# dbandstra/zang

Hardware: AMD Instinct MI355X
Metric: voice-samples/sec (higher is better)
Workload: dtype f32

## Files before the change

bindings/zang_hip.zig:

```

const std = @import("std");

pub const OK: c_int = 0;
pub const ERR_INVALID: c_int = -1;
pub const ERR_UNSUPPORTED: c_int = -2;
pub const ERR_NO_DEVICE: c_int = -3;
pub const ERR_COMM: c_int = -4;
pub const ERR_RCCL_BASE: c_int = -100;
pub const PAINT_ADD: u32 = 0;
pub const PAINT_ZERO_FIRST: u32 = 1;
pub const PAINT_PARAMS_UNCHANGED: u32 = 4;
pub const PAINT_TOLERANT: u32 = 8;
pub const COB_CONSTANT: u32 = 0;
pub const COB_BUFFER: u32 = 1;
pub const CURVE_INSTANTANEOUS: u32 = 0;
pub const CURVE_LINEAR: u32 = 1;
pub const CURVE_SQUARED: u32 = 2;
pub const CURVE_CUBED: u32 = 3;
pub const CAPTURE_COALESCE: u32 = 1;
pub const MIX_SEQUENTIAL: u32 = 2;
pub const COMM_ID_BYTES: u32 = 128;
pub const AUDIO_SIGNED8: u32 = 0;
pub const AUDIO_SIGNED16_LSB: u32 = 1;
pub const NOISE_WHITE: u32 = 0;
pub const NOISE_PINK: u32 = 1;
pub const ENV_IDLE: u32 = 0;
pub const ENV_ATTACK: u32 = 1;
pub const ENV_DECAY: u32 = 2;
pub const ENV_SUSTAIN: u32 = 3;
pub const ENV_RELEASE: u32 = 4;
pub const FILTER_BYPASS: u32 = 0;
pub const FILTER_LOW_PASS: u32 = 1;
pub const FILTER_BAND_PASS: u32 = 2;
pub const FILTER_HIGH_PASS: u32 = 3;
pub const FILTER_NOTCH: u32 = 4;
pub const FILTER_ALL_PASS: u32 = 5;
pub const SAMPLE_U8: u32 = 0;
pub const SAMPLE_S16_LSB: u32 = 1;
pub const SAMPLE_S24_LSB: u32 = 2;
pub const SAMPLE_S32_LSB: u32 = 3;
pub const DISTORTION_OVERDRIVE: u32 = 0;
pub const DISTORTION_CLIP: u32 = 1;
pub const CURVE_FN_LINEAR: u32 = 0;
pub const CURVE_FN_SMOOTHSTEP: u32 = 1;
pub const MIX_MAX_BATCH: u32 = 16;
pub const FM_MOD_FREQ_MUL: u32 = 0;
pub const FM_MOD_WAVEFORM: u32 = 1;
pub const FM_MOD_VOLUME: u32 = 2;
pub const FM_MOD_ATTACK: u32 = 3;
pub const FM_MOD_DECAY: u32 = 4;
pub const FM_MOD_SUSTAIN: u32 = 5;
pub const FM_MOD_RELEASE: u32 = 6;
pub const FM_MOD_TREMOLO: u32 = 7;
pub const FM_MOD_VIBRATO: u32 = 8;
pub const FM_MOD_FEEDBACK: u32 = 9;
pub const FM_CAR_FREQ_MUL: u32 = 10;
pub const FM_CAR_WAVEFORM: u32 = 11;
pub const FM_CAR_VOLUME: u32 = 12;
pub const FM_CAR_ATTACK: u32 = 13;
pub const FM_CAR_DECAY: u32 = 14;
pub const FM_CAR_SUSTAIN: u32 = 15;
pub const FM_CAR_RELEASE: u32 = 16;
pub const FM_CAR_TREMOLO: u32 = 17;
pub const FM_CAR_VIBRATO: u32 = 18;
pub const FM_TREMOLO_DEPTH: u32 = 19;
pub const FM_VIBRATO_DEPTH: u32 = 20;
pub const FM_ALGORITHM: u32 = 21;
pub const FM_PATCH_VALUES: u32 = 22;
pub const FM_SPLIT_OPERATORS: u32 = 16;
pub const SP_CONSTANT: u32 = 0;
pub const SP_BOOLEAN: u32 = 1;
pub const SP_COB: u32 = 2;
pub const SP_BUFFER: u32 = 3;
pub const SP_ENUM: u32 = 4;
pub const SP_CURVE: u32 = 5;
pub const SINEOSC_SPAN_FREQ: u32 = 0;
pub const SINEOSC_SPAN_PHASE: u32 = 1;
pub const SINEOSC_SPAN_FIELDS: u32 = 2;
pub const PULSEOSC_SPAN_FREQ: u32 = 0;
pub const PULSEOSC_SPAN_COLOR: u32 = 1;
pub const PULSEOSC_SPAN_FIELDS: u32 = 2;
pub const TRISAWOSC_SPAN_FREQ: u32 = 0;
pub const TRISAWOSC_SPAN_COLOR: u32 = 1;
pub const TRISAWOSC_SPAN_FIELDS: u32 = 2;
pub const NOISE_SPAN_COLOR: u32 = 0;
pub const NOISE_SPAN_FIELDS: u32 = 1;
pub const ENVELOPE_SPAN_ATTACK: u32 = 0;
pub const ENVELOPE_SPAN_DECAY: u32 = 1;
pub const ENVELOPE_SPAN_RELEASE: u32 = 2;
pub const ENVELOPE_SPAN_SUSTAIN_VOLUME: u32 = 3;
pub const ENVELOPE_SPAN_NOTE_ON: u32 = 4;
pub const ENVELOPE_SPAN_FIELDS: u32 = 5;
pub const GATE_SPAN_NOTE_ON: u32 = 0;
pub const GATE_SPAN_FIELDS: u32 = 1;
pub const FILTER_SPAN_TYPE: u32 = 0;
pub const FILTER_SPAN_CUTOFF: u32 = 1;
pub const FILTER_SPAN_RES: u32 = 2;
pub const FILTER_SPAN_FIELDS: u32 = 3;
pub const SAMPLER_SPAN_SAMPLE_RATE: u32 = 0;
pub const SAMPLER_SPAN_LOOP: u32 = 1;
pub const SAMPLER_SPAN_FIELDS: u32 = 2;
pub const DECIMATOR_SPAN_FAKE_SAMPLE_RATE: u32 = 0;
pub const DECIMATOR_SPAN_FIELDS: u32 = 1;
pub const DISTORTION_SPAN_TYPE: u32 = 0;
pub const DISTORTION_SPAN_INGAIN: u32 = 1;
pub const DISTORTION_SPAN_OUTGAIN: u32 = 2;
pub const DISTORTION_SPAN_OFFSET: u32 = 3;
pub const DISTORTION_SPAN_FIELDS: u32 = 4;
pub const SAMPLER_KIT_SPAN_SAMPLE_RATE: u32 = 0;
pub const SAMPLER_KIT_SPAN_LOOP: u32 = 1;
pub const SAMPLER_KIT_SPAN_SAMPLE: u32 = 2;
pub const SAMPLER_KIT_SPAN_CHANNEL: u32 = 3;
pub const SAMPLER_KIT_SPAN_FIELDS: u32 = 4;
pub const MAX_IMPULSES: u32 = 32;
pub const MAX_PARAMS_SIZE: u32 = 64;
pub const SCRIPT_MAX_PARAMS: u32 = 16;
pub const ZSCRIPT_FORM_SPANS: u32 = 8;
pub const ZSCRIPT_FORM_ROLES: u32 = 1;
pub const ZSCRIPT_FORM_ROLES_WORTH: u32 = 2;

pub const Ctx = opaque {};
pub const Graph = opaque {};
pub const Event = opaque {};
pub const Comm = opaque {};
pub const SineOscHandle = opaque {};
pub const PulseOscHandle = opaque {};
pub const TriSawOscHandle = opaque {};
pub const NoiseHandle = opaque {};
pub const EnvelopeHandle = opaque {};
pub const GateHandle = opaque {};
pub const FilterHandle = opaque {};
pub const SamplerHandle = opaque {};
pub const SampleKit = opaque {};
pub const DecimatorHandle = opaque {};
pub const DistortionHandle = opaque {};
pub const CurveModuleHandle = opaque {};
pub const CycleHandle = opaque {};
pub const PortamentoHandle = opaque {};
pub const NiceHandle = opaque {};
pub const DelayHandle = opaque {};
pub const FilteredEchoesHandle = opaque {};
pub const StereoEchoesHandle = opaque {};
pub const NoiseFilterHandle = opaque {};
pub const PMOscHandle = opaque {};
pub const Fm = opaque {};
pub const Script = opaque {};
pub const ScriptModule = opaque {};
pub const ZScript = opaque {};
pub const ImpulseQueue = opaque {};
pub const NoteTracker = opaque {};
pub const PolyphonyDispatcher = opaque {};
pub const Trigger = opaque {};
pub const PolyVoice = opaque {};
pub const VoiceBank = opaque {};

pub const Buf = extern struct {
    ptr: ?[*]f32 = null,
    voices: u32 = 0,
    frames: u32 = 0,
    stride: u32 = 0,
    reserved: u32 = 0,
};
pub const F32 = extern struct {
    value: f32 = 0,
    reserved: u32 = 0,
    per_voice: ?[*]const f32 = null,
};
pub const Bool = extern struct {
    value: u32 = 0,
    reserved: u32 = 0,
    per_voice: ?[*]const u8 = null,
};
pub const Cob = extern struct {
    tag: u32 = 0,
    reserved: u32 = 0,
    constant: F32 = std.mem.zeroes(F32),
    buffer: Buf = std.mem.zeroes(Buf),
};
pub const Curve = extern struct {
    tag: u32 = 0,
    reserved: u32 = 0,
    duration: F32 = std.mem.zeroes(F32),
};
pub const SineOscParams = extern struct {
    sample_rate: f32 = 0,
    reserved: u32 = 0,
    freq: Cob = std.mem.zeroes(Cob),
    phase: Cob = std.mem.zeroes(Cob),
};
pub const SineOscState = extern struct {
    t: f32 = 0,
};
pub const PulseOscParams = extern struct {
    sample_rate: f32 = 0,
    reserved: u32 = 0,
    freq: Cob = std.mem.zeroes(Cob),
    color: F32 = std.mem.zeroes(F32),
};
pub const PulseOscState = extern struct {
    cnt: u32 = 0,
};
pub const TriSawOscParams = extern struct {
    sample_rate: f32 = 0,
    reserved: u32 = 0,
    freq: Cob = std.mem.zeroes(Cob),
    color: F32 = std.mem.zeroes(F32),
};
pub const TriSawOscState = extern struct {
    cnt: u32 = 0,
    t: f32 = 0,
};
pub const NoiseParams = extern struct {
    color: u32 = 0,
};
pub const NoiseState = extern struct {
    r: [4]u64 = [_]u64{0} ** 4,
    b: [7]f32 = [_]f32{0} ** 7,
    reserved: u32 = 0,
};
pub const EnvelopeParams = extern struct {
    sample_rate: f32 = 0,
    reserved: u32 = 0,
    attack: Curve = std.mem.zeroes(Curve),
    decay: Curve = std.mem.zeroes(Curve),
    release: Curve = std.mem.zeroes(Curve),
    sustain_volume: F32 = std.mem.zeroes(F32),
    note_on: Bool = std.mem.zeroes(Bool),
};
pub const EnvelopeState = extern struct {
    state: u32 = 0,
    t: f32 = 0,
    last_value: f32 = 0,
    start: f32 = 0,
};
pub const GateParams = extern struct {
    note_on: Bool = std.mem.zeroes(Bool),
};
pub const FilterParams = extern struct {
    input: Buf = std.mem.zeroes(Buf),
    @"type": u32 = 0,
    reserved: u32 = 0,
    cutoff: Cob = std.mem.zeroes(Cob),
    res: Cob = std.mem.zeroes(Cob),
};
pub const FilterState = extern struct {
    l: f32 = 0,
    b: f32 = 0,
};
pub const Sample = extern struct {
    num_channels: u64 = 0,
    sample_rate: u64 = 0,
    format: u32 = 0,
    reserved: u32 = 0,
    data: ?[*]const u8 = null,
    data_len: u64 = 0,
};
pub const SamplerParams = extern struct {
    sample_rate: F32 = std.mem.zeroes(F32),
    sample: Sample = std.mem.zeroes(Sample),
    channel: u64 = 0,
    loop: u32 = 0,
    reserved: u32 = 0,
};
pub const SamplerState = extern struct {
    t: f32 = 0,
};
pub const DecimatorParams = extern struct {
    sample_rate: f32 = 0,
    reserved: u32 = 0,
    input: Buf = std.mem.zeroes(Buf),
    fake_sample_rate: F32 = std.mem.zeroes(F32),
};
// ... 1471 lines not shown
```

include/zang_hip.h:

```cpp
#ifndef ZANG_HIP_H
#define ZANG_HIP_H

#if !defined(__HIPCC_RTC__)
#include <stddef.h>
#include <stdint.h>
#endif

#ifdef __cplusplus
extern "C" {
#endif

#define ZH_API __attribute__((visibility("default")))

enum { ZH_OK = 0, ZH_ERR_INVALID = -1, ZH_ERR_UNSUPPORTED = -2, ZH_ERR_NO_DEVICE = -3,
       ZH_ERR_COMM = -4,
       ZH_ERR_RCCL_BASE = -100     };

enum { ZH_PAINT_ADD = 0,
       ZH_PAINT_ZERO_FIRST = 1,
       ZH_PAINT_PARAMS_UNCHANGED = 4,
       ZH_PAINT_TOLERANT = 8
        };

typedef struct zh_ctx zh_ctx;
// ... 388 lines not shown
typedef struct zh_fm_params { float sample_rate; uint32_t reserved; zh_buf tremolo_input, vibrato_input; zh_f32 freq; zh_bool note_on; } zh_fm_params;
typedef struct zh_fm_op_state { float t, feedback1, feedback2; uint32_t reserved; zh_envelope_state env; } zh_fm_op_state;
typedef struct zh_fm_state { zh_fm_op_state modulator, carrier; } zh_fm_state;
ZH_API int zh_fm_patch_default(zh_fm_patch *patch);
ZH_API int zh_fm_create(zh_ctx *ctx, uint32_t n_voices, uint32_t group, zh_fm **out);
ZH_API int zh_fm_destroy(zh_fm *m);
ZH_API int zh_fm_set_patches(zh_fm *m, const zh_fm_patch *patches, uint32_t n_patches);
ZH_API int zh_fm_get_state(zh_fm *m, zh_fm_state *host);
ZH_API int zh_fm_set_state(zh_fm *m, const zh_fm_state *host);
ZH_API int zh_fm_paint(zh_fm *m, uint32_t span_start, uint32_t span_end, const zh_buf *outputs,
                       const zh_buf *temps ,
                       zh_bool note_id_changed, const zh_fm_params *params, uint32_t flags);
ZH_API int zh_fm_paint_spans(zh_fm *m, uint32_t span_start, uint32_t span_end, const zh_buf *outputs,
                             const zh_buf *temps, float sample_rate, zh_buf tremolo_input, zh_buf vibrato_input,
                             const zh_span_table *table, uint32_t flags);

enum { ZH_SP_CONSTANT = 0,
       ZH_SP_BOOLEAN = 1,
       ZH_SP_COB = 2,
       ZH_SP_BUFFER = 3,
       ZH_SP_ENUM = 4,
       ZH_SP_CURVE = 5 };
typedef struct zh_script_param {
    uint32_t kind, u;
    float f;
    uint32_t is_buffer;
    const float *pf;
    const uint8_t *pb;
    uint32_t stride, reserved;
} zh_script_param;
#define ZH_SCRIPT_MAX_PARAMS 16

typedef struct zh_script zh_script;
typedef struct zh_script_module zh_script_module;
ZH_API int zh_script_compile(const char *hip_source, void **code_out, size_t *code_size_out, char *log, size_t log_cap);
ZH_API void zh_script_free_code(void *code);
ZH_API int zh_script_load(zh_ctx *ctx, const char *hip_source, zh_script **out, char *log, size_t log_cap);
ZH_API int zh_script_load_code(zh_ctx *ctx, const void *code, size_t code_size, zh_script **out);
ZH_API int zh_script_destroy(zh_script *s);
ZH_API int zh_script_module_create(zh_script *s, const char *name, uint32_t n_voices, uint32_t state_words,
                                   uint64_t first_seed, zh_script_module **out);
ZH_API int zh_script_module_destroy(zh_script_module *m);
ZH_API int zh_script_module_ranges_ok(zh_script_module *m);
ZH_API int zh_script_module_get_state(zh_script_module *m, uint32_t *host_words);
ZH_API int zh_script_module_set_state(zh_script_module *m, const uint32_t *host_words);
ZH_API int zh_script_module_paint(zh_script_module *m, uint32_t span_start, uint32_t span_end, const zh_buf *outputs,
                                  zh_bool note_id_changed, const zh_script_param *params, uint32_t n_params, uint32_t flags);
typedef struct zh_script_span_table {
    uint32_t max_spans, reserved;
    const uint32_t *count;
    const uint32_t *start, *end;
    const uint8_t  *note_id_changed;
} zh_script_span_table;
typedef struct zh_script_span_param {
    const float    *f;
    const uint32_t *u;
} zh_script_span_param;
#define ZH_ZSCRIPT_FORM_SPANS 8
ZH_API int zh_script_module_paint_spans(zh_script_module *m, uint32_t span_start, uint32_t span_end, const zh_buf *outputs,
                                        const zh_script_param *params, uint32_t n_params, const zh_script_span_param *span_params,
                                        const zh_script_span_table *table, uint32_t flags);

enum { ZH_SINEOSC_SPAN_FREQ = 0,
       ZH_SINEOSC_SPAN_PHASE,
       ZH_SINEOSC_SPAN_FIELDS };
enum { ZH_PULSEOSC_SPAN_FREQ = 0,
       ZH_PULSEOSC_SPAN_COLOR,
       ZH_PULSEOSC_SPAN_FIELDS };
enum { ZH_TRISAWOSC_SPAN_FREQ = 0,
       ZH_TRISAWOSC_SPAN_COLOR,
       ZH_TRISAWOSC_SPAN_FIELDS };
enum { ZH_NOISE_SPAN_COLOR = 0,
       ZH_NOISE_SPAN_FIELDS };
enum { ZH_ENVELOPE_SPAN_ATTACK = 0,
       ZH_ENVELOPE_SPAN_DECAY,
       ZH_ENVELOPE_SPAN_RELEASE,
       ZH_ENVELOPE_SPAN_SUSTAIN_VOLUME,
       ZH_ENVELOPE_SPAN_NOTE_ON,
       ZH_ENVELOPE_SPAN_FIELDS };
enum { ZH_GATE_SPAN_NOTE_ON = 0,
       ZH_GATE_SPAN_FIELDS };
enum { ZH_FILTER_SPAN_TYPE = 0,
       ZH_FILTER_SPAN_CUTOFF,
       ZH_FILTER_SPAN_RES,
       ZH_FILTER_SPAN_FIELDS };
enum { ZH_SAMPLER_SPAN_SAMPLE_RATE = 0,
       ZH_SAMPLER_SPAN_LOOP,
       ZH_SAMPLER_SPAN_FIELDS };
enum { ZH_DECIMATOR_SPAN_FAKE_SAMPLE_RATE = 0,
       ZH_DECIMATOR_SPAN_FIELDS };
enum { ZH_DISTORTION_SPAN_TYPE = 0,
       ZH_DISTORTION_SPAN_INGAIN,
       ZH_DISTORTION_SPAN_OUTGAIN,
       ZH_DISTORTION_SPAN_OFFSET,
       ZH_DISTORTION_SPAN_FIELDS };
ZH_API int zh_sineosc_paint_spans(zh_sineosc *m, uint32_t span_start, uint32_t span_end, const zh_buf *outputs, const zh_buf *temps,
                                  const zh_sineosc_params *params, const zh_script_span_param *span_params ,
                                  const zh_script_span_table *table, uint32_t flags);
ZH_API int zh_pulseosc_paint_spans(zh_pulseosc *m, uint32_t span_start, uint32_t span_end, const zh_buf *outputs, const zh_buf *temps,
                                   const zh_pulseosc_params *params, const zh_script_span_param *span_params ,
                                   const zh_script_span_table *table, uint32_t flags);
ZH_API int zh_trisawosc_paint_spans(zh_trisawosc *m, uint32_t span_start, uint32_t span_end, const zh_buf *outputs, const zh_buf *temps,
                                    const zh_trisawosc_params *params, const zh_script_span_param *span_params ,
                                    const zh_script_span_table *table, uint32_t flags);
ZH_API int zh_noise_paint_spans(zh_noise *m, uint32_t span_start, uint32_t span_end, const zh_buf *outputs, const zh_buf *temps,
                                const zh_noise_params *params, const zh_script_span_param *span_params ,
                                const zh_script_span_table *table, uint32_t flags);
ZH_API int zh_envelope_paint_spans(zh_envelope *m, uint32_t span_start, uint32_t span_end, const zh_buf *outputs, const zh_buf *temps,
                                   const zh_envelope_params *params, const zh_script_span_param *span_params ,
                                   const zh_script_span_table *table, uint32_t flags);
ZH_API int zh_gate_paint_spans(zh_gate *m, uint32_t span_start, uint32_t span_end, const zh_buf *outputs, const zh_buf *temps,
                               const zh_gate_params *params, const zh_script_span_param *span_params ,
                               const zh_script_span_table *table, uint32_t flags);
ZH_API int zh_filter_paint_spans(zh_filter *m, uint32_t span_start, uint32_t span_end, const zh_buf *outputs, const zh_buf *temps,
                                 const zh_filter_params *params, const zh_script_span_param *span_params ,
                                 const zh_script_span_table *table, uint32_t flags);
ZH_API int zh_sampler_paint_spans(zh_sampler *m, uint32_t span_start, uint32_t span_end, const zh_buf *outputs, const zh_buf *temps,
                                  const zh_sampler_params *params, const zh_script_span_param *span_params ,
                                  const zh_script_span_table *table, uint32_t flags);
ZH_API int zh_decimator_paint_spans(zh_decimator *m, uint32_t span_start, uint32_t span_end, const zh_buf *outputs, const zh_buf *temps,
                                    const zh_decimator_params *params, const zh_script_span_param *span_params ,
                                    const zh_script_span_table *table, uint32_t flags);
ZH_API int zh_distortion_paint_spans(zh_distortion *m, uint32_t span_start, uint32_t span_end, const zh_buf *outputs, const zh_buf *temps,
                                     const zh_distortion_params *params, const zh_script_span_param *span_params ,
                                     const zh_script_span_table *table, uint32_t flags);

typedef struct zh_u32 { uint32_t value; uint32_t reserved; const uint32_t *per_voice; } zh_u32;
typedef struct zh_sampler_kit_params {
    zh_f32 sample_rate;
    zh_bool loop;
    zh_u32 sample;
    zh_u32 channel;
    const zh_sample_kit *kit;
} zh_sampler_kit_params;
enum { ZH_SAMPLER_KIT_SPAN_SAMPLE_RATE = 0,
       ZH_SAMPLER_KIT_SPAN_LOOP,
       ZH_SAMPLER_KIT_SPAN_SAMPLE,
       ZH_SAMPLER_KIT_SPAN_CHANNEL,
       ZH_SAMPLER_KIT_SPAN_FIELDS };
ZH_API int zh_sampler_paint_kit_spans(zh_sampler *m, uint32_t span_start, uint32_t span_end, const zh_buf *outputs, const zh_buf *temps,
                                      const zh_sampler_kit_params *params, const zh_script_span_param *span_params ,
                                      const zh_script_span_table *table, uint32_t flags);
ZH_API int zh_sampler_paint_kit(zh_sampler *m, uint32_t span_start, uint32_t span_end, const zh_buf *outputs, const zh_buf *temps,
                                zh_bool note_id_changed, const zh_sampler_kit_params *params, uint32_t flags);

typedef struct zh_zscript zh_zscript;
ZH_API int zh_zscript_compile(const char *text, const char *filename, uint32_t packages, zh_zscript **out, char *err, size_t err_cap);
ZH_API int zh_zscript_destroy(zh_zscript *z);
ZH_API void zh_zscript_free_text(char *text);
ZH_API int zh_zscript_generate_zig(zh_zscript *z, char **text_out);
ZH_API int zh_zscript_generate_hip(zh_zscript *z, const char *only_csv, int unroll, char **text_out);
#define ZH_ZSCRIPT_FORM_ROLES 1
#define ZH_ZSCRIPT_FORM_ROLES_WORTH 2
ZH_API int zh_zscript_generate_hip_forms(zh_zscript *z, const char *only_csv, int unroll, uint32_t forms, char **text_out);
ZH_API uint32_t zh_zscript_module_count(zh_zscript *z);
ZH_API int zh_zscript_module_info(zh_zscript *z, uint32_t i, char *name, size_t name_cap, uint32_t *state_words, uint32_t *noise_fields,
                                  uint32_t *n_params, char *error , size_t error_cap);
ZH_API int zh_zscript_module_num_temps(zh_zscript *z, uint32_t i, uint32_t *num_temps);
ZH_API int zh_zscript_module_param(zh_zscript *z, uint32_t i, uint32_t p, char *name, size_t name_cap, char *kind, size_t kind_cap,
                                   char *enum_name, size_t enum_cap);

typedef struct zh_impulse { uint64_t frame, note_id, event_id; } zh_impulse;
typedef struct zh_iap { const zh_impulse *impulses; const void *paramses; uint64_t len; } zh_iap;
enum { ZH_MAX_IMPULSES = 32, ZH_MAX_PARAMS_SIZE = 64 };

typedef struct zh_impulse_queue zh_impulse_queue;
ZH_API int zh_impulse_queue_create(uint32_t params_size, zh_impulse_queue **out);
ZH_API int zh_impulse_queue_destroy(zh_impulse_queue *q);
ZH_API int zh_impulse_queue_push(zh_impulse_queue *q, uint64_t impulse_frame, uint64_t note_id, const void *params);
ZH_API int zh_impulse_queue_consume(zh_impulse_queue *q, zh_iap *out);

typedef struct zh_note_tracker zh_note_tracker;
ZH_API int zh_note_tracker_create(uint32_t params_size, uint64_t n_events, const void *paramses, const float *t,
                                  const uint64_t *note_ids, zh_note_tracker **out);
ZH_API int zh_note_tracker_destroy(zh_note_tracker *nt);
ZH_API int zh_note_tracker_reset(zh_note_tracker *nt);
ZH_API int zh_note_tracker_consume(zh_note_tracker *nt, float sample_rate, uint64_t span_start, uint64_t span_end, zh_iap *out);

typedef struct zh_polyphony_dispatcher zh_polyphony_dispatcher;
ZH_API int zh_polyphony_dispatcher_create(uint32_t polyphony, uint32_t params_size, uint32_t note_on_offset,
                                          zh_polyphony_dispatcher **out);
ZH_API int zh_polyphony_dispatcher_destroy(zh_polyphony_dispatcher *pd);
ZH_API int zh_polyphony_dispatcher_reset(zh_polyphony_dispatcher *pd);
ZH_API int zh_polyphony_dispatcher_dispatch(zh_polyphony_dispatcher *pd, zh_iap iap, zh_iap *out );

typedef struct zh_trigger zh_trigger;
typedef struct zh_paint_span {
    uint64_t start, end; uint32_t note_id_changed; uint32_t reserved; uint8_t params[64];
} zh_paint_span;
ZH_API int zh_trigger_create(uint32_t params_size, zh_trigger **out);
ZH_API int zh_trigger_destroy(zh_trigger *t);
ZH_API int zh_trigger_reset(zh_trigger *t);
ZH_API int zh_trigger_counter(zh_trigger *t, uint64_t span_start, uint64_t span_end, zh_iap iap);
ZH_API int zh_trigger_next(zh_trigger *t, zh_paint_span *out);

typedef struct zh_poly_voice zh_poly_voice;
ZH_API int zh_poly_voice_create(uint32_t polyphony, uint32_t params_size, uint32_t note_on_offset, uint64_t n_events,
                                const void *paramses, const float *t, const uint64_t *note_ids, zh_poly_voice **out);
ZH_API int zh_poly_voice_destroy(zh_poly_voice *pv);
ZH_API int zh_poly_voice_reset(zh_poly_voice *pv);
ZH_API int zh_poly_voice_schedule(zh_poly_voice *pv, float sample_rate, const uint32_t *frames, uint32_t n_buffers,
                                  uint32_t max_spans, uint32_t *counts, uint32_t *start, uint32_t *end, void *params,
                                  uint8_t *note_id_changed);

typedef struct zh_voice_bank zh_voice_bank;
typedef struct zh_voice_bank_instrument_state { uint64_t next_event; float t; uint32_t reserved; } zh_voice_bank_instrument_state;
typedef struct zh_voice_bank_voice_state {
    uint32_t used, note_on; uint64_t note_id, event_id;
    uint32_t has_note, reserved; uint64_t trigger_note_id;
    uint64_t trigger_event;
} zh_voice_bank_voice_state;
ZH_API int zh_voice_bank_create(zh_ctx *ctx, uint32_t n_instruments, uint32_t polyphony, uint32_t params_size, uint32_t note_on_offset,
                                const uint64_t *event_offsets, const void *paramses, const float *t, const uint64_t *note_ids,
                                zh_voice_bank **out);
ZH_API int zh_voice_bank_destroy(zh_voice_bank *bank);
ZH_API int zh_voice_bank_reset(zh_voice_bank *bank);
ZH_API int zh_voice_bank_reserve(zh_voice_bank *bank, uint32_t max_rows);
ZH_API int zh_voice_bank_schedule(zh_voice_bank *bank, float sample_rate, const uint32_t *frames, uint32_t n_buffers, uint32_t max_spans);
ZH_API int zh_voice_bank_script_table(const zh_voice_bank *bank, uint32_t max_spans, zh_script_span_table *out);
ZH_API int zh_voice_bank_span_param(const zh_voice_bank *bank, uint32_t word, zh_script_span_param *out);
ZH_API int zh_voice_bank_span_table(const zh_voice_bank *bank, uint32_t max_spans, uint32_t freq_word, zh_span_table *out);
ZH_API int zh_voice_bank_overflows(zh_voice_bank *bank, uint64_t *out);
ZH_API int zh_voice_bank_get_state(zh_voice_bank *bank, zh_voice_bank_instrument_state *instruments ,
                                   zh_voice_bank_voice_state *voices );
ZH_API int zh_voice_bank_set_state(zh_voice_bank *bank, const zh_voice_bank_instrument_state *instruments,
                                   const zh_voice_bank_voice_state *voices);

typedef struct zh_bank_impulses {
    uint32_t n; const uint32_t *instrument, *frame; const uint64_t *note_id; const void *paramses;
} zh_bank_impulses;
typedef struct zh_voice_bank_live_voice_state {
    uint32_t used, note_on; uint64_t note_id, event_id;
    uint32_t has_note, reserved; uint64_t trigger_note_id;
    uint32_t carried[16];
} zh_voice_bank_live_voice_state;
ZH_API int zh_voice_bank_create_live(zh_ctx *ctx, uint32_t n_instruments, uint32_t polyphony, uint32_t params_size, uint32_t note_on_offset,
                                     uint32_t max_impulses_per_call, zh_voice_bank **out);
ZH_API int zh_voice_bank_schedule_live(zh_voice_bank *bank, uint32_t out_len, uint32_t max_spans, const zh_bank_impulses *batch);
ZH_API int zh_voice_bank_live_get_state(zh_voice_bank *bank, uint64_t *next_event_id ,
                                        zh_voice_bank_live_voice_state *voices );
ZH_API int zh_voice_bank_live_set_state(zh_voice_bank *bank, const uint64_t *next_event_id, const zh_voice_bank_live_voice_state *voices);

typedef struct zh_hcob { uint32_t tag; float constant; const float *buffer; } zh_hcob;
typedef struct zh_hcurve { uint32_t tag; float duration; } zh_hcurve;

typedef struct zh_sineosc_host_params { float sample_rate; zh_hcob freq, phase; } zh_sineosc_host_params;
typedef struct zh_pulseosc_host_params { float sample_rate; zh_hcob freq; float color; } zh_pulseosc_host_params;
typedef zh_pulseosc_host_params zh_trisawosc_host_params;
typedef struct zh_noise_host_params { uint32_t color; } zh_noise_host_params;
typedef struct zh_envelope_host_params { float sample_rate; zh_hcurve attack, decay, release; float sustain_volume; uint32_t note_on; } zh_envelope_host_params;
typedef struct zh_gate_host_params { uint32_t note_on; } zh_gate_host_params;
typedef struct zh_filter_host_params { const float *input; uint32_t type; zh_hcob cutoff, res; } zh_filter_host_params;
typedef struct zh_sampler_host_params {
    float sample_rate; uint64_t num_channels, sample_rate_in; uint32_t format; const uint8_t *data; uint64_t data_len;
    uint64_t channel; uint32_t loop;
} zh_sampler_host_params;
typedef struct zh_decimator_host_params { float sample_rate; const float *input; float fake_sample_rate; } zh_decimator_host_params;
typedef struct zh_distortion_host_params { const float *input; uint32_t type; float ingain, outgain, offset; } zh_distortion_host_params;

ZH_API int zh_noise_state_init(zh_noise_state *state, uint64_t seed);
ZH_API int zh_decimator_state_init(zh_decimator_state *state);

ZH_API int zh_sineosc_paint_host(zh_ctx *ctx, zh_sineosc_state *state, uint32_t span_start, uint32_t span_end, float *const *outputs, float *const *temps, uint32_t note_id_changed, const zh_sineosc_host_params *params);
ZH_API int zh_pulseosc_paint_host(zh_ctx *ctx, zh_pulseosc_state *state, uint32_t span_start, uint32_t span_end, float *const *outputs, float *const *temps, uint32_t note_id_changed, const zh_pulseosc_host_params *params);
ZH_API int zh_trisawosc_paint_host(zh_ctx *ctx, zh_trisawosc_state *state, uint32_t span_start, uint32_t span_end, float *const *outputs, float *const *temps, uint32_t note_id_changed, const zh_trisawosc_host_params *params);
ZH_API int zh_noise_paint_host(zh_ctx *ctx, zh_noise_state *state, uint32_t span_start, uint32_t span_end, float *const *outputs, float *const *temps, uint32_t note_id_changed, const zh_noise_host_params *params);
ZH_API int zh_envelope_paint_host(zh_ctx *ctx, zh_envelope_state *state, uint32_t span_start, uint32_t span_end, float *const *outputs, float *const *temps, uint32_t note_id_changed, const zh_envelope_host_params *params);
ZH_API int zh_gate_paint_host(zh_ctx *ctx, void *state_unused, uint32_t span_start, uint32_t span_end, float *const *outputs, float *const *temps, uint32_t note_id_changed, const zh_gate_host_params *params);
ZH_API int zh_filter_paint_host(zh_ctx *ctx, zh_filter_state *state, uint32_t span_start, uint32_t span_end, float *const *outputs, float *const *temps, uint32_t note_id_changed, const zh_filter_host_params *params);
ZH_API int zh_sampler_paint_host(zh_ctx *ctx, zh_sampler_state *state, uint32_t span_start, uint32_t span_end, float *const *outputs, float *const *temps, uint32_t note_id_changed, const zh_sampler_host_params *params);
ZH_API int zh_decimator_paint_host(zh_ctx *ctx, zh_decimator_state *state, uint32_t span_start, uint32_t span_end, float *const *outputs, float *const *temps, uint32_t note_id_changed, const zh_decimator_host_params *params);
ZH_API int zh_distortion_paint_host(zh_ctx *ctx, void *state_unused, uint32_t span_start, uint32_t span_end, float *const *outputs, float *const *temps, uint32_t note_id_changed, const zh_distortion_host_params *params);

#ifdef __cplusplus
}
#endif
#endif
```

zang_amd/csrc/common.hip.h:

```cpp
#pragma once
#if defined(__HIPCC_RTC__)
#define ZH_DEVICE_ONLY 1
#endif
#include <hip/hip_runtime.h>
#if !defined(ZH_DEVICE_ONLY)
#include <stdint.h>
#include <stddef.h>
#include <new>
#endif
#include "rtc_types.hip.h"
#include "../../include/zang_hip.h"

#if !defined(ZH_DEVICE_ONLY)
#include <utility>
#include <vector>
#include <functional>
#include <memory>
#include <string>
struct zh_flipper {
    uint64_t id;
    zh_ctx *ctx;
    uint32_t n;
    uint32_t *cnt[2];
    int cur;
    uint32_t words = 1;
};
struct zh_flip_use {
    uint64_t id;
    zh_flipper *f;
    int first_cur;
    uint32_t flips;
};

struct zh_flipper;
struct zh_co_batch {
    bool active = false;
    const void *owner = nullptr;
    uint32_t start = 0, end = 0, stride = 0, key = 0, max = 0;
    bool flips = false;
    std::vector<float *> imgs;
    std::shared_ptr<void> items;
    std::function<void(hipStream_t, float *const *, uint32_t)> launch;
    const char *kernel = nullptr;
};
struct zh_direct_item {
    std::function<void(hipStream_t, float *const *, uint32_t)> launch;
    std::vector<float *> imgs;
    const char *kernel;
};

struct zh_ctx {
    int device;
    hipStream_t stream;
    bool own_stream;
    uint32_t capture_flags;
    bool epoch_open;
    zh_co_batch co;
    uint32_t co_paints, co_launches;
    std::string last_form;
    bool form_fresh;
    float *mix_partials;
    size_t mix_partials_floats;
    std::vector<float *> mix_retired;
    uint32_t graphs_live;
    std::vector<struct zh_graph *> graphs;
    bool capturing;
    uint32_t capture_serial;
    std::vector<zh_flip_use> capture_log;
    std::vector<std::pair<std::string, uint32_t>> capture_kernels;
    int deferred_error = 0;
    std::vector<zh_direct_item> co_plan;
    bool co_plan_ok = true;
    uint32_t capture_launches = 0, co_plan_launches = 0;
    void *noise_jump;
};

struct zh_graph {
    zh_ctx *ctx;
    hipGraph_t graph;
    hipGraphExec_t exec;
    std::vector<zh_flip_use> flips;
    uint32_t nodes = 0;
    uint32_t co_paints = 0, co_launches = 0;
    std::vector<std::pair<std::string, uint32_t>> kernels;
    std::vector<zh_direct_item> plan;
    std::vector<std::pair<std::string, uint32_t>> plan_kernels;
};

struct ZhDeviceGuard {
    int prev, want;
    explicit ZhDeviceGuard(int device) : prev(-1), want(device) {
        if (want < 0) return;
        if (hipGetDevice(&prev) != hipSuccess) { prev = -1; return; }
        if (prev != want) (void)hipSetDevice(want);
    }
    ~ZhDeviceGuard() { if (want >= 0 && prev >= 0 && prev != want) (void)hipSetDevice(prev); }
    ZhDeviceGuard(const ZhDeviceGuard &) = delete;
    ZhDeviceGuard &operator=(const ZhDeviceGuard &) = delete;
};
void zh_epoch_barrier(zh_ctx *ctx);
extern thread_local zh_ctx *zh_tls_ctx;
struct ZhFormScope {
    zh_ctx *prev;
    explicit ZhFormScope(const zh_ctx *c) : prev(zh_tls_ctx) {
        if (!prev) { zh_tls_ctx = const_cast<zh_ctx *>(c); if (zh_tls_ctx) zh_tls_ctx->form_fresh = true; }
    }
    ~ZhFormScope() { zh_tls_ctx = prev; }
};
#define ZH_GUARD_EPOCH(ctxptr) const zh_ctx *_zh_gctx = (ctxptr); ZhDeviceGuard _zh_guard(_zh_gctx ? _zh_gctx->device : -1); ZhFormScope _zh_fscope(_zh_gctx)
#define ZH_LAUNCH(kernel, ...) do { zh_note_launch(zh_tls_ctx, #kernel); hipLaunchKernelGGL(kernel, __VA_ARGS__); } while (0)
#define ZH_GUARD(ctxptr) ZH_GUARD_EPOCH(ctxptr); do { if (_zh_gctx && _zh_gctx->epoch_open) zh_epoch_barrier(const_cast<zh_ctx *>(_zh_gctx)); } while (0)
void zh_epoch_flush_batch(zh_ctx *ctx, bool last);

void zh_flipper_register(zh_flipper *f);
void zh_flipper_unregister(zh_flipper *f);
void zh_flipper_used(zh_flipper *f);
void zh_flipper_painted(zh_flipper *f);

enum { ZF_SINE_RANGES, ZF_NOISE_RANGES, ZF_ENVELOPE_RANGES, ZF_SAMPLER_RANGES, ZF_DECIMATOR_RANGES, ZF_CURVE_RANGES, ZF_CYCLE_RANGES,
       ZF_PORTAMENTO_RANGES, ZF_PULSE_CTRL_RANGES, ZF_PULSE_CTRL_SUMS, ZF_TRISAW_CTRL_RANGES, ZF_TRISAW_CTRL_QUOT, ZF_PMOSC_RANGES,
       ZF_SCRIPT_RANGES, ZF_SCRIPT_RANGES_MAXV, ZF_OSC_FC, ZF_NICE_PC_MAX, ZF_NICE_PC4_MAX, ZF_NICE_WAVE_MAX, ZF_PMOSC_WAVE_MAX,
       ZF_NICE_MIX_ROLL, ZF_NICE_MIX_WG_MIN, ZF_NF_PC_MAX, ZF_NF_RING_MAX, ZF_FILTER_PC_MAX, ZF_FILTER_PC16_MAX, ZF_FILTER_PC_CTL_MAX,
       ZF_PINK_PIPE_MAX, ZF_PINK_TAPS, ZF_ECHOES_PC_MAX, ZF_DELAY_FRAMES_MAX, ZF_FILTER_TP_MAX, ZF_NF_TP_MAX, ZF_NICE_TP_MAX,
       ZF_PINK_TP_MAX, ZF_ECHOES_TP_MAX, ZF_NICE_MIX_FMA, ZF_BASICS_ROWS_MIN, ZF_SCRIPT_PC, ZF_SCRIPT_PC_MAXV, ZF_NF_TP_PIPE_FRAMES, ZF_DISTORTION_ROWS_MIN, ZF_DISTORTION_RC, ZF_GRAPH_DIRECT,
       ZF_STEREO_ECHOES_PC_MAX, ZF_COUNT };
long zh_form(int id);
bool zh_form_is_set(int id);
uint32_t zh_range_frames(uint32_t V, uint32_t n, int form, uint32_t target_waves, uint32_t max_voices);
void zh_note_launch(zh_ctx *ctx, const char *kernel);
extern thread_local const char *zh_tls_launch_detail;

constexpr int kMixGroupFrames = 8;

struct zh_event {
    hipEvent_t ev;
};
#endif

#define ZH_INLINE_LAMBDA __attribute__((always_inline))

#if !defined(ZH_DEVICE_ONLY)
#define ZH_TRY(expr)                                   \
    do {                                               \
        hipError_t _e = (expr);                        \
        if (_e != hipSuccess) return (int)_e;          \
    } while (0)

static inline int zh_launch_status() {
    hipError_t e = hipGetLastError();
    return e == hipSuccess ? ZH_OK : (int)e;
}
#endif

struct Img {
    float *p;
    uint32_t stride;
    __device__ __forceinline__ float *at(uint32_t f, uint32_t v) const { return p + (size_t)f * stride + v; }
};
struct CImg {
    const float *p;
    uint32_t stride;
    __device__ __forceinline__ const float *at(uint32_t f, uint32_t v) const { return p + (size_t)f * stride + v; }
};
struct F32P {
    float value;
    const float *pv;
    __device__ __forceinline__ float get(uint32_t v) const { return pv ? pv[v] : value; }
};
struct BoolP {
    uint32_t value;
    const uint8_t *pv;
    __device__ __forceinline__ bool get(uint32_t v) const { return pv ? pv[v] != 0 : value != 0; }
};
struct CobP {
    uint32_t is_buffer;
    F32P c;
    CImg b;
};

#if !defined(ZH_DEVICE_ONLY)
static inline Img mk_img(const zh_buf &b) { return Img{b.ptr, b.stride}; }
static inline CImg mk_cimg(const zh_buf &b) { return CImg{b.ptr, b.stride}; }
static inline F32P mk_f32(const zh_f32 &f) { return F32P{f.value, f.per_voice}; }
static inline BoolP mk_bool(const zh_bool &b) { return BoolP{b.value, b.per_voice}; }
static inline CobP mk_cob(const zh_cob &c) {
    return CobP{c.tag == ZH_COB_BUFFER ? 1u : 0u, mk_f32(c.constant), mk_cimg(c.buffer)};
}

constexpr uint32_t kMaxRowStride = 1u << 26;
static inline bool buf_covers(const zh_buf &b, uint32_t n_voices, uint32_t span_end) {
    return b.ptr != nullptr && b.voices >= n_voices && b.frames >= span_end && b.stride >= n_voices && b.stride <= kMaxRowStride;
}
static inline bool bufs_alias(const zh_buf &a, const zh_buf &b) {
    if (!a.ptr || !b.ptr) return false;
    const float *ae = a.ptr + (size_t)a.frames * a.stride, *be = b.ptr + (size_t)b.frames * b.stride;
    return a.ptr < be && b.ptr < ae;
}
static inline bool cob_aliases(const zh_cob &c, const zh_buf &b) { return c.tag == ZH_COB_BUFFER && bufs_alias(c.buffer, b); }
static inline int zh_zero_first_aliased(zh_ctx *ctx, uint32_t start, uint32_t end, const zh_buf &out, uint32_t n_voices, bool aliased, uint32_t &flags) {
    if (!aliased || !(flags & ZH_PAINT_ZERO_FIRST)) return ZH_OK;
    flags &= ~(uint32_t)ZH_PAINT_ZERO_FIRST;
    zh_buf o = out;
    o.voices = n_voices;
    return end > start ? zh_zero(ctx, start, end, o) : ZH_OK;
}
static inline bool cob_ok(const zh_cob &c, uint32_t n_voices, uint32_t span_end) {
    if (c.tag == ZH_COB_CONSTANT) return true;
    if (c.tag == ZH_COB_BUFFER) return buf_covers(c.buffer, n_voices, span_end);
    return false;
}

#ifndef ZH_SEQ_BLOCK
#define ZH_SEQ_BLOCK 64
#endif
constexpr int kSeqBlock = ZH_SEQ_BLOCK;
static inline dim3 seq_grid(uint32_t n) { return dim3((n + kSeqBlock - 1) / kSeqBlock); }

template <typename T> static inline int dev_alloc(T **p, size_t count) {
    *p = nullptr;
    if (count == 0) return ZH_OK;
    hipError_t e = hipMalloc((void **)p, count * sizeof(T));
    return e == hipSuccess ? ZH_OK : (int)e;
}

#endif

enum StoreMode { ST_PLAIN = 0, ST_NT = 1, ST_SC1 = 2, ST_SC0SC1 = 3 };

typedef float zv4f __attribute__((ext_vector_type(4)));
typedef unsigned int zv4u __attribute__((ext_vector_type(4)));

#if defined(__HIP_DEVICE_COMPILE__)
typedef __amdgpu_buffer_rsrc_t zh_rsrc_t;
__device__ __forceinline__ zh_rsrc_t make_rsrc(const void *base, uint32_t bytes) {
    return __builtin_amdgcn_make_buffer_rsrc(const_cast<void *>(base), 0, bytes, 0x00020000);
}
template <int SM>
__device__ __forceinline__ void store4(float *p, zh_rsrc_t rsrc, uint32_t byte_off, zv4f v) {
    if constexpr (SM == ST_PLAIN) *reinterpret_cast<zv4f *>(p) = v;
    else if constexpr (SM == ST_NT) __builtin_nontemporal_store(v, reinterpret_cast<zv4f *>(p));
    else if constexpr (SM == ST_SC1) __builtin_amdgcn_raw_buffer_store_b128(__builtin_bit_cast(zv4u, v), rsrc, byte_off, 0, 16);
    else __builtin_amdgcn_raw_buffer_store_b128(__builtin_bit_cast(zv4u, v), rsrc, byte_off, 0, 17);
}
template <int SM>
__device__ __forceinline__ void store1(float *p, zh_rsrc_t rsrc, uint32_t byte_off, float v) {
    if constexpr (SM == ST_PLAIN) *p = v;
    else if constexpr (SM == ST_NT) __builtin_nontemporal_store(v, p);
    else if constexpr (SM == ST_SC1) __builtin_amdgcn_raw_buffer_store_b32(__builtin_bit_cast(unsigned int, v), rsrc, byte_off, 0, 16);
    else __builtin_amdgcn_raw_buffer_store_b32(__builtin_bit_cast(unsigned int, v), rsrc, byte_off, 0, 17);
}
__device__ __forceinline__ void store_row(float *p, float v) { __builtin_nontemporal_store(v, p); }
__device__ __forceinline__ void store4_sc1(float *p, zv4f v) { asm volatile("global_store_dwordx4 %0, %1, off sc1\n\ts_nop 1" ::"v"(p), "v"(v) : "memory"); }
#else
typedef int zh_rsrc_t;
__device__ inline void store4_sc1(float *, zv4f) {}
__device__ inline void store_row(float *, float) {}
__device__ inline zh_rsrc_t make_rsrc(const void *, uint32_t) { return 0; }
template <int SM> __device__ inline void store4(float *, zh_rsrc_t, uint32_t, zv4f) {}
template <int SM> __device__ inline void store1(float *, zh_rsrc_t, uint32_t, float) {}
#endif

#if !defined(ZH_DEVICE_ONLY)
int zh_store_mode();
int zh_store_mode_env();
constexpr uint32_t kRowPadVoices = 1024;
#endif
```

zang_amd/csrc/dispatch.hip:

```cpp
#include "common.hip.h"
#include <mutex>
#include <stdlib.h>
#include <string.h>
#include <string>

namespace {
struct FormRow { const char *name; long def; const char *doc; };
const FormRow kForms[ZF_COUNT] = {
     {"sine_ranges", -1, "SineOsc: frame ranges of the span at once, each replaying the phase walk before it (k_sineosc_ranges); auto: ~4,096 waves up to 1 Mi voices, ~2,048 up to 65,536 with a control image"},
     {"noise_ranges", -1, "Noise: frame ranges from jumped generator states (noise_jump.hip); auto: by voice count up to 65,536"},
     {"envelope_ranges", -1, "Envelope: frame ranges, each replaying the clock (k_envelope_ranges); auto: ~2,048 waves up to 40,960 voices"},
     {"sampler_ranges", -1, "Sampler: frame ranges (positions are a product, no replay); auto: ~16,384 waves up to 1 Mi voices"},
     {"decimator_ranges", -1, "Decimator: frame ranges replaying the hold counter; auto: ~1,024-2,048 waves up to 65,536 voices"},
     {"curve_ranges", -1, "Curve: frame ranges; auto: ~2,048 waves up to 40,960 voices"},
     {"cycle_ranges", -1, "Cycle: frame ranges (constant speed); auto: ~1,024 waves up to 16,384 voices"},
     {"portamento_ranges", -1, "Portamento: frame ranges; auto: ~2,048 waves up to 32,768 voices"},
     {"pulse_ctrl_ranges", -1, "PulseOsc with a frequency image: frame ranges over the summed phase advances; auto: ~2,048 waves up to 40,960 voices"},
     {"pulse_ctrl_sums", 1, "... 1: a first kernel sums each range's own advances (k_pulseosc_ctrl_sums), 0: every range replays the frames before it"},
     {"trisaw_ctrl_ranges", -1, "TriSawOsc with a frequency image: frame ranges; auto: ~1,024 waves up to 16,384 voices"},
     {"trisaw_ctrl_quot", 1, "... 1: freq / sample_rate painted once into a module-owned image first (k_div_image), 0: divided in every replay"},
     {"pmosc_ranges", -1, "PMOscInstrument: frame ranges (k_pmosc_ranges); auto: ~2,048-4,096 waves up to 131,072 voices"},
     {"script_ranges", -1, "generated script kernels: frame ranges for modules without a delay ring; auto: by voice count"},
     {"script_ranges_maxv", 131072, "... the largest voice count that takes them"},
     {"osc_fc", 0, "constant-frequency PulseOsc / TriSawOsc: frames per lane of the chunked kernel; 0 = PulseOsc 4, from 16,384 voices 3 with non-temporal stores (profiles/r05/osc_large_voice_counts.txt); TriSawOsc 8-64 by voice count (tools/sweep_osc_fc.sh), PulseOsc's when the paint is a sawtooth for every voice (one color <= 0)"},
     {"nice_pc_max", 65536, "NiceInstrument: up to here the oscillator, envelope and filter chains run in three waves side by side (k_nice_pc: 72 vs 146 us at 4,096 voices, 107 vs 168 at 65,536; slower at 131,072)"},
     {"nice_pc4_max", 32768, "... and up to here in four (k_nice_pc4: 44 / 47 / 53.5 us at 4,096 / 16,384 / 32,768 voices against 60.5 / 62.5 / 63)"},
     {"nice_wave_max", 64, "zh_nice_paint_spans: up to here one WAVE per voice, lanes = frames (k_nice_spans_wave)"},
     {"pmosc_wave_max", 64, "zh_pmosc_paint_spans: the same (k_pmosc_spans_wave)"},
     {"nice_mix_roll", 1, "fused mixdown: the oscillator's half-period bit carried as a lane mask (1) or recomputed (0): 148.2 vs 149.6 us at 131,072 voices"},
     {"nice_mix_wg_min", 65536, "fused mixdown: from here one partial row per 256-voice workgroup instead of per wave (a quarter of the partial traffic; 4,096 voices: 99 -> 105 us with it, 131,072: level)"},
     {"nf_pc_max", 65536, "Noise -> Filter voice: up to here noise and filter in two waves side by side (k_noise_filter_pc: 75 vs 110 us at 4,096 voices, 111 vs 133 at 65,536)"},
     {"nf_ring_max", 16384, "... white noise: up to here three producer waves, a filter wave and a writer wave per 64 voices (k_noise_filter_ring)"},
     {"filter_pc_max", 32768, "Filter, constant cutoff / resonance: up to here the three-wave pipeline over 32-frame tiles (k_filter_pc: 41-51 us against 54-76 in one wave); 0 = never (the 16-frame form too unless filter_pc16_max is given), 1 = the 16-frame form only"},
     {"filter_pc16_max", 65536, "... 16-frame tiles above filter_pc_max up to here (36,864 / 65,536 voices: 72 / 104 us against 97 / 116)"},
     {"filter_pc_ctl_max", 32768, "... with control images (k_filter_pc_ctl: 47-98 us against 96-140 up to 32,768 voices)"},
     {"pink_pipe_max", 32768, "pink Noise: up to here white frame ranges + the taps as a second kernel (k_pink_taps / k_pink_pipe) instead of one loop"},
     {"pink_taps", 1, "... 1: four-wave tap kernel (32-frame tiles up to 16,384 voices, 16 above), 16: the 16-frame tiles always, 0: the seven-stage chain k_pink_pipe"},
     {"echoes_pc_max", 65536, "FilteredEchoes: up to here ring reader / filter / writer as waves side by side (k_filtered_echoes_pc)"},
     {"delay_frames_max", 4294967295, "Delay: up to here the frames of a delay length at once instead of the walk (57 -> 13 us at 4,096 voices, 423 -> 271 at 131,072: every voice count)"},
     {"filter_tp_max", 16384, "ZH_PAINT_TOLERANT Filter: the largest voice count painted as chunks at once (filter_tp.hip.h)"},
     {"nf_tp_max", 16384, "... Noise -> Filter voice"},
     {"nice_tp_max", 16384, "... NiceInstrument and its fused mixdown"},
     {"pink_tp_max", 16384, "... pink Noise"},
     {"echoes_tp_max", 6144, "... FilteredEchoes (six image streams: level with the exact form at 8,192 voices)"},
     {"nice_mix_fma", 1, "ZH_PAINT_TOLERANT fused mixdown above nice_tp_max voices: 1 = the kernel compiled with multiply-adds fused (nice_mix_fma.hip), 0 = the exact kernel"},
     {"basics_rows_min", 32768, "basics.zig operations (zero, set, copy, add ..., multiply ...): from here three consecutive rows of a 256-voice column per wave (k_elementwise_chunks) instead of the row-striding loop: 131,072 voices 12-23 % faster"},
     {"script_pc", -1, "generated script kernels: the role-wave form (zs_paint_pc_<name>: the body's builtin calls as producer / recurrence / writer waves over LDS tiles); auto: where the emitter found the lane form unable to take frame ranges and the longest role well below the whole body; 0 = never, 1 = every module that has the form"},
     {"script_pc_maxv", 65536, "... the largest voice count that takes it -- half of it for a module whose role form does more than 1.25 x the body's work or needs more than 9 waves (FilteredSawtooth: 53 / 57 / 66 / 110 us at 4,096 / 16,384 / 32,768 / 65,536 voices against 172-181 in one wave per 64 voices; slower at 131,072)"},
     {"nf_tp_pipe_frames", 0, "ZH_PAINT_TOLERANT Noise -> Filter voice recorded pipelined (ZH_CAPTURE_COALESCE, k_nf_tp_ba): frames per chunk, a multiple of 32; 0 = as outside a pipeline (32 at 4,096 voices)"},
     {"distortion_rows_min", 32768, "Distortion clip: from here four voices per lane, three consecutive rows of a 256-voice column per wave, the per-voice constants once per workgroup through LDS (k_distortion_chunks: 224 -> 178 us at 131,072 voices); the overdrive too when this row is set by hand (no faster: 239 against 244-250 us)"},
     {"distortion_rc", 0, "... rows per wave of that form: 3 (0), 6 or 8"},
     {"graph_direct", 1, "zh_graph_launch of a ZH_CAPTURE_COALESCE capture that recorded nothing but held-back oscillator batches: 1 = their launches enqueued directly, one per batch of up to 32 buffers (20 paints: one launch of 20), 0 = the recorded hipGraph (20 paints: two launches of 10)"},
     {"stereo_echoes_pc_max", 32768, "StereoEchoes: up to here loader / filter / writer waves (k_stereo_echoes_pc); StereoEchoes(15000), 1,024 frames, role waves against the walk: 253 / 318 us at 32,768 voices, 518 / 454 at 65,536 (profiles/r10)"},
};

struct Overrides { bool set[ZF_COUNT]; long val[ZF_COUNT]; };
Overrides parse_forms() {
    Overrides o;
    memset(&o, 0, sizeof o);
    const char *e = getenv("ZH_FORMS");
    if (!e) return o;
    std::string s(e);
    size_t i = 0;
    while (i < s.size()) {
        size_t j = s.find(',', i);
        if (j == std::string::npos) j = s.size();
        const std::string item = s.substr(i, j - i);
        const size_t eq = item.find('=');
        if (eq != std::string::npos) {
            const std::string name = item.substr(0, eq);
            for (int k = 0; k < ZF_COUNT; k++)
                if (name == kForms[k].name) { o.set[k] = true; o.val[k] = strtol(item.c_str() + eq + 1, nullptr, 10); }
        }
        i = j + 1;
    }
    return o;
}
}

bool zh_form_is_set(int id) {
    if (id < 0 || id >= ZF_COUNT) return false;
    return parse_forms().set[id];
}

long zh_form(int id) {
    if (id < 0 || id >= ZF_COUNT) return 0;
    static const bool live = [] { const char *e = getenv("ZH_ENV_LIVE"); return e && e[0] == '1'; }();
    if (live) {
        const Overrides o = parse_forms();
        return o.set[id] ? o.val[id] : kForms[id].def;
    }
    static const Overrides once = parse_forms();
    return once.set[id] ? once.val[id] : kForms[id].def;
}

uint32_t zh_range_frames(uint32_t V, uint32_t n, int form, uint32_t target_waves, uint32_t max_voices) {
    const long forced = zh_form(form);
    if (forced == 0 || V == 0 || n < 128 || V > max_voices) return 0;
    const uint32_t waves = (V + 63) / 64;
    uint32_t want = forced > 0 ? (uint32_t)forced : target_waves / waves;
    if (want < 2) return 0;
    if (want > 64) want = 64;
    const uint32_t ch = ((n + want - 1) / want + 7) / 8 * 8;
    return (n + ch - 1) / ch >= 2 ? ch : 0;
}

thread_local const char *zh_tls_launch_detail = nullptr;

void zh_note_launch(zh_ctx *ctx, const char *kernel) {
    const char *detail = zh_tls_launch_detail;
    zh_tls_launch_detail = nullptr;
    if (!ctx) return;
    if (ctx->capturing) {
        ctx->capture_launches++;
        const char *b0 = kernel;
        while (*b0 == '(' || *b0 == ' ') b0++;
        size_t n0 = 0;
        while (b0[n0] && b0[n0] != '<' && b0[n0] != ')' && b0[n0] != ' ') n0++;
        std::string key(b0, n0);
        if (detail) { key += '['; key += detail; key += ']'; }
        bool found = false;
        for (auto &kv : ctx->capture_kernels) if (kv.first == key) { kv.second++; found = true; break; }
        if (!found && ctx->capture_kernels.size() < 64) ctx->capture_kernels.emplace_back(key, 1u);
    }
    std::string &f = ctx->last_form;
    if (ctx->form_fresh) { f.clear(); ctx->form_fresh = false; }
    if (f.size() > 480) return;
    const char *b = kernel;
    while (*b == '(' || *b == ' ') b++;
    size_t n = 0;
    while (b[n] && b[n] != '<' && b[n] != ')' && b[n] != ' ') n++;
    if (!f.empty()) {
        const size_t last = f.rfind(',');
        const std::string prev = last == std::string::npos ? f : f.substr(last + 1);
        if (prev.compare(0, std::string::npos, b, n) == 0) return;
        f += ',';
    }
    f.append(b, n);
}

extern "C" {

int zh_form_count(void) { return ZF_COUNT; }

int zh_form_info(int index, const char **name, long *default_value, long *current_value, const char **doc) {
    if (index < 0 || index >= ZF_COUNT) return ZH_ERR_INVALID;
    if (name) *name = kForms[index].name;
    if (default_value) *default_value = kForms[index].def;
    if (current_value) *current_value = zh_form(index);
    if (doc) *doc = kForms[index].doc;
    return ZH_OK;
}

int zh_last_form(zh_ctx *ctx, char *out, size_t n) {
    if (!ctx || !out || n == 0) return ZH_ERR_INVALID;
    const std::string &f = ctx->last_form;
    const size_t k = f.size() < n - 1 ? f.size() : n - 1;
    memcpy(out, f.data(), k);
    out[k] = 0;
    return ZH_OK;
}

}
```

zang_amd/csrc/voices.hip.h:

```cpp
#pragma once
#include "common.hip.h"
#include "zmath.hip.h"
#include "dsp.hip.h"
#include "envelope.hip.h"

template <int SINMODE = 1>
__device__ __forceinline__ float sine_osc_sin(float t) {
    const float x = t * 3.14159265358979323846f * 2.0f;
    if constexpr (SINMODE == 2) return zsinf_tol(x);
    else return zsinf<SINMODE != 0>(x);
}
constexpr float kSineOscSmallT = 6.0e7f;

struct SineOscLane {
    float t;
    float t_step, inv_sr;
    __device__ __forceinline__ void begin(float sample_rate, float freq_const) {
        t_step = freq_const / sample_rate;
        inv_sr = 1.0f / sample_rate;
    }
    template <bool FB, int SINMODE = 1, bool SELF = false> __device__ __forceinline__ float frame(float freq_i, float phase_i) {
        const float val = sine_osc_sin<SINMODE>(t + phase_i);
        if (FB) t += (SELF ? freq_i + val : freq_i) * inv_sr; else t += t_step;
        return val;
// ... 21 lines not shown
    __device__ __forceinline__ bool frame_const(float &val) {
        if (bad) return false;
        val = pulse_sample(k, cnt);
        cnt += k.ifreq;
        return true;
    }
    __device__ __forceinline__ void begin_ctrl(float sample_rate, float color) {
        srf = 4294967296.0f / sample_rate;
        sr8 = sample_rate / 8.0f;
        pulse_setup_color(k, color);
    }
    __device__ __forceinline__ bool frame_ctrl(float s_freq, float &val) {
        if (s_freq < 0 || s_freq > sr8) return false;
        pulse_setup_freq(k, srf, s_freq);
        val = pulse_sample(k, cnt);
        cnt += k.ifreq;
        return true;
    }
};

struct TriSawK {
    uint32_t ifreq, brpt;
    float f, omf, rcpf, col, c1, c2;
};

__device__ __forceinline__ void trisaw_setup(TriSawK &k, float srf, float freq, float color) {
    const float gain = 0.7f;
    k.ifreq = zf32_to_u32(srf * freq);
    k.brpt = zftou32(zclamp01(color));
    k.f = zutof23(k.ifreq);
    k.omf = 1.0f - k.f;
    k.rcpf = 1.0f / k.f;
    k.col = zutof23(k.brpt);
    k.c1 = gain / k.col;
    k.c2 = -gain / (1.0f - k.col);
}
__device__ __forceinline__ float trisaw_sample(const TriSawK &k, uint32_t cnt) {
    const float gain = 0.7f;
    const float p = zutof23(cnt) - k.col;
    const bool b0 = cnt < k.brpt;
    const bool b1 = (uint32_t)(cnt - k.ifreq) < k.brpt;
    const bool b2 = cnt < k.ifreq;
    const float cx = b0 ? k.c1 : k.c2;
    const float flat_nowrap = cx * (p + p - k.f);
    const float flat_wrap = -k.rcpf * (gain + cx * k.omf * (p + p + k.omf));
    const float ramp2 = k.rcpf * (k.c2 * (p * p) - k.c1 * ((p - k.f) * (p - k.f)));
    const float ramp5 = -k.rcpf * (gain + k.c2 * ((p + k.omf) * (p + k.omf)) - k.c1 * (p * p));
    const float flat = b2 ? flat_wrap : flat_nowrap;
    const float ramp = b2 ? ramp5 : ramp2;
    const float v = (b0 == b1) ? flat : ramp;
    return gain + v;
}
__device__ __forceinline__ bool trisaw_all_saw(const TriSawK &k) { return __builtin_amdgcn_ballot_w64(k.brpt != 0u) == 0; }
__device__ __forceinline__ float trisaw_sample_saw(const TriSawK &k, uint32_t cnt) {
    const float gain = 0.7f;
    const float p = zutof23(cnt) - k.col;
    const bool b2 = cnt < k.ifreq;
    const float flat_nowrap = k.c2 * (p + p - k.f);
    const float flat_wrap = -k.rcpf * (gain + k.c2 * k.omf * (p + p + k.omf));
    return gain + (b2 ? flat_wrap : flat_nowrap);
}
__device__ __forceinline__ float trisaw_naive(float t, bool saw) {
    const float fr = t - floorf(t);
    const float sawv = fr * 2.0f - 1.0f;
    const float up = fr * 4.0f;
    const float down = 1.0f - (fr - 0.25f) * 4.0f;
    const float up2 = (fr - 0.75f) * 4.0f - 1.0f;
    const float tri = zsel_hard(fr < 0.25f, up, zsel_hard(fr < 0.75f, down, up2));
    return 0.7f * zsel_hard(saw, sawv, tri);
}

struct TriSawOscLane {
    uint32_t cnt;
    float t;
    TriSawK k;
    float sample_rate;
    bool bad, saw;
    bool all_saw;
    __device__ __forceinline__ void begin_const(float sr, float freq, float color) {
        bad = freq < 0 || freq > sr / 8.0f;
        trisaw_setup(k, 4294967296.0f / sr, freq, color);
        all_saw = trisaw_all_saw(k);
    }
    __device__ __forceinline__ bool frame_const(float &val) {
        if (bad) return false;
        val = all_saw ? trisaw_sample_saw(k, cnt) : trisaw_sample(k, cnt);
        cnt += k.ifreq;
        return true;
    }
    __device__ __forceinline__ void begin_ctrl(float sr, float color) {
        sample_rate = sr;
        saw = color < 0.25f || color > 0.75f;
    }
    template <bool SELF = false> __device__ __forceinline__ float frame_ctrl(float s_freq) {
        const float val = trisaw_naive(t, saw);
        t += (SELF ? s_freq + val : s_freq) / sample_rate;
        return val;
    }
    __device__ __forceinline__ float frame_ctrl_q(float q) {
        const float val = trisaw_naive(t, saw);
        t += q;
        return val;
    }
    __device__ __forceinline__ void end_ctrl() { t = t - truncf(t); }
};

struct NoiseLane {
    ZXoshiro r;
    float b[7];
    __device__ __forceinline__ void begin() {
#pragma unroll
        for (int j = 0; j < 7; j++) b[j] = 0.0f;
    }
    template <bool PINK> __device__ __forceinline__ float frame() {
        const float white = zrandom_float32(r) * 2.0f - 1.0f;
        return PINK ? pink_step(b, white) : white;
    }
    __device__ __forceinline__ float frame_sel(bool pink) {
        const float white = zrandom_float32(r) * 2.0f - 1.0f;
        const float p = pink_step(b, white);
        return pink ? p : white;
    }
};

struct FilterLane {
    float l, b;
    float cut, res, l_mul, b_mul, h_mul;
    bool bypass;
    __device__ __forceinline__ void begin(uint32_t type, float cutoff_const, float res_const) {
        bypass = type == ZH_FILTER_BYPASS;
        l_mul = (type == ZH_FILTER_LOW_PASS || type == ZH_FILTER_NOTCH || type == ZH_FILTER_ALL_PASS) ? 1.0f : 0.0f;
        b_mul = (type == ZH_FILTER_BAND_PASS || type == ZH_FILTER_ALL_PASS) ? 1.0f : 0.0f;
        h_mul = (type == ZH_FILTER_HIGH_PASS || type == ZH_FILTER_NOTCH || type == ZH_FILTER_ALL_PASS) ? 1.0f : 0.0f;
        cut = zclampf(cutoff_const, 0.0f, 1.0f);
        res = 1.0f - zclampf(res_const, 0.0f, 1.0f);
    }
    template <bool CB, bool RB> __device__ __forceinline__ float frame(float x, float cutoff_i, float res_i) {
        if (bypass) return x;
        if (CB) cut = zclampf(cutoff_i, 0.0f, 1.0f);
        if (RB) res = 1.0f - zclampf(res_i, 0.0f, 1.0f);
        const SvfOut s = svf_step(l, b, x, cut, res);
        return s.l * l_mul + s.b * b_mul + s.h * h_mul;
    }
    __device__ __forceinline__ float pre(float x) const { return x + kSvfDcOffset; }
    template <bool CB, bool RB> __device__ __forceinline__ SvfOut core(float in, float cutoff_i, float res_i) {
        if (bypass) return SvfOut{0.0f, 0.0f, 0.0f};
        if (CB) cut = zclampf(cutoff_i, 0.0f, 1.0f);
        if (RB) res = 1.0f - zclampf(res_i, 0.0f, 1.0f);
        return svf_core(l, b, in, cut, res);
    }
    __device__ __forceinline__ float mix(float sl, float sb, float sh) const { return sl * l_mul + sb * b_mul + sh * h_mul; }
    __device__ __forceinline__ float post(float x, float sl, float sb, float sh) const { return bypass ? x : mix(sl, sb, sh); }

};

struct DecimatorLane {
    float dval, dcount;
    int mode;
    float ratio;
    __device__ __forceinline__ void begin(float sample_rate, float fake) {
        mode = fake >= sample_rate ? 0 : (fake > 0.0f ? 1 : 2);
        ratio = fake / sample_rate;
    }
    __device__ __forceinline__ bool frame(float x, float &val) {
        const float dc = dcount + ratio;
        const bool trig = dc >= 1.0f;
        const float dcn = trig ? dc - 1.0f : dc;
        const bool run = mode == 1;
        dval = (run && trig) ? x : dval;
        dcount = run ? dcn : dcount;
        val = mode == 0 ? x : dval;
        return mode != 2;
    }
    __device__ __forceinline__ void step(uint32_t i, uint32_t &last) {
        const float dc = dcount + ratio;
        const bool trig = dc >= 1.0f;
        dcount = trig ? dc - 1.0f : dc;
        last = trig ? i : last;
    }
    __device__ __forceinline__ bool walk_is_plain() const { return mode != 1 || (dcount >= 0.0f && dcount <= 1.0f && ratio > 0.0f && ratio < 1.0f); }
    __device__ __forceinline__ void step_plain(uint32_t &idx, uint32_t &last) {
        const float dc = dcount + ratio;
        last = dc >= 1.0f ? idx : last;
        dcount = __builtin_amdgcn_fractf(dc);
        idx += 1;
    }
    __device__ __forceinline__ void end() {
        if (mode == 0) { dval = 0.0f; dcount = 1.0f; }
    }
};

struct DistortionLane {
    float gain1, offs, gain2;
    bool overdrive;
    __device__ __forceinline__ void begin(uint32_t type, float ingain, float outgain, float offset) {
        overdrive = type == ZH_DISTORTION_OVERDRIVE;
        gain1 = zpowf_pos(2.0f, ingain * 8.0f - 2.0f);
        offs = gain1 * offset;
        gain2 = overdrive ? outgain / zatanf(gain1) : outgain;
    }
    __device__ __forceinline__ float frame(float x) {
        const float a0 = x * gain1 + offs;
        if (overdrive) return gain2 * zatanf(a0);
        return gain2 * (a0 < -1.0f ? -1.0f : (a0 > 1.0f ? 1.0f : a0));
    }
};

struct SampleP {
    const uint8_t *data;
    uint64_t data_len;
    uint32_t num_channels, sample_rate_in, format, channel, loop, whole;
    int32_t num_samples;
    double inv_num_samples;
};

template <int N> struct zint { static constexpr int value = N; };
constexpr int kSampleEmpty = -1;
template <int FMT>
__device__ __forceinline__ float sampler_decode(const uint8_t *data, size_t i, bool whole) {
    if constexpr (FMT == kSampleEmpty) return 0.0f;
    else if constexpr (FMT == ZH_SAMPLE_U8) return ((float)data[i] - 127.5f) / 127.5f;
    else {
        constexpr int byte_count = FMT + 1;
        const uint8_t *p = data + i * byte_count;
        int32_t sval;
        if constexpr (byte_count == 2) sval = whole ? (int16_t)*reinterpret_cast<const uint16_t *>(p) : (int16_t)((uint16_t)p[0] | ((uint16_t)p[1] << 8));
        else if constexpr (byte_count == 3) {
            const uint32_t u = (uint32_t)p[0] | ((uint32_t)p[1] << 8) | ((uint32_t)p[2] << 16);
            sval = (int32_t)(u << 8) >> 8;
        } else sval = whole ? (int32_t)*reinterpret_cast<const uint32_t *>(p)
                            : (int32_t)((uint32_t)p[0] | ((uint32_t)p[1] << 8) | ((uint32_t)p[2] << 16) | ((uint32_t)p[3] << 24));
        const float inv_max = 1.0f / (float)(1u << (byte_count * 8 - 1));
        return (float)sval * inv_max;
    }
}

__device__ __forceinline__ int32_t sampler_mod(int32_t index, int32_t n, double inv_n) {
    const int32_t q = (int32_t)floor((double)index * inv_n);
    int32_t r = (int32_t)((uint32_t)index - (uint32_t)q * (uint32_t)n);
    r = r < 0 ? r + n : r;
    r = r >= n ? r - n : r;
    return r;
}

template <int FMT>
__device__ __forceinline__ float sampler_at(const SampleP &s, int32_t index) {
    if constexpr (FMT == kSampleEmpty) return 0.0f;
    const bool in = index >= 0 && index < s.num_samples;
    const size_t i = (size_t)(in ? index : 0) * s.num_channels + s.channel;
    const float val = sampler_decode<FMT>(s.data, i, s.whole != 0);
    return in ? val : 0.0f;
}
template <int FMT, bool LOOP>
__device__ __forceinline__ float sampler_get_sample(const SampleP &s, int32_t index1) {
    if constexpr (FMT == kSampleEmpty) return 0.0f;
    return sampler_at<FMT>(s, LOOP ? sampler_mod(index1, s.num_samples, s.inv_num_samples) : index1);
}

struct SamplerLane {
    float t;
    float ratio;
    int32_t t0;
    uint32_t n;
    bool loop, silent, plain;
    __device__ __forceinline__ void begin(const SampleP &s, float out_rate, bool loop_, bool note_id_changed) {
        if (note_id_changed) t = 0.0f;
        loop = loop_;
        ratio = (float)s.sample_rate_in / out_rate;
        silent = ratio < 0.0f && !loop;
        plain = ratio > 0.9999f && ratio < 1.0001f;
        t0 = zf32_to_i32(roundf(t));
        n = 0;
    }
    template <int FMT> __device__ __forceinline__ float at(const SampleP &s, int32_t index1) const {
        if constexpr (FMT == kSampleEmpty) return 0.0f;
        else return sampler_at<FMT>(s, loop ? sampler_mod(index1, s.num_samples, s.inv_num_samples) : index1);
    }
    template <int FMT> __device__ __forceinline__ bool frame(const SampleP &s, float &val) {
        if (silent) return false;
        if (plain) {
            val = at<FMT>(s, (int32_t)((uint32_t)t0 + n));
            n++;
            return true;
        }
        const int32_t i0 = zf32_to_i32(floorf(t));
        const int32_t i1 = (int32_t)((uint32_t)i0 + 1u);
        const float tfrac = (float)i1 - t;
        const float s0 = at<FMT>(s, i0);
        const float s1 = at<FMT>(s, i1);
        val = s0 * (1.0f - tfrac) + s1 * tfrac;
        t += ratio;
        return true;
    }
    __device__ __forceinline__ void end(const SampleP &s) {
        if (silent) return;
        if (plain) t += (float)n;
        if (t >= (float)s.data_len && loop) t -= (float)s.data_len;
    }
};

struct CycleLane {
    float t;
    float step, isr;
    __device__ __forceinline__ void begin(float sample_rate, float speed_const) {
        step = speed_const / sample_rate;
        isr = 1.0f / sample_rate;
// ... 228 lines not shown
```

zang_amd/csrc/zscript_emit.hip:

```cpp
#include <math.h>
#include <stdarg.h>
#include <stdio.h>
#include <stdlib.h>
#include <string.h>

#include "../../include/zang_hip.h"
#include "zscript.hpp"
#include <algorithm>
#include <regex>

namespace zs {
namespace {

std::string strf(const char *fmt, ...) {
    va_list ap, ap2;
    va_start(ap, fmt);
    va_copy(ap2, ap);
    const int n = vsnprintf(nullptr, 0, fmt, ap);
    va_end(ap);
    std::string s((size_t)n + 1, '\0');
    vsnprintf(&s[0], s.size(), fmt, ap2);
    va_end(ap2);
    s.resize((size_t)n);
    return s;
// ... 253 lines not shown
            o.p(strf("pub const num_outputs = %zu;\n", mr.num_outputs));
            o.p(strf("pub const num_temps = %zu;\n", mr.num_temps));
            o.p("pub const Params = struct {\n");
            param_decls(module->params, false);
            o.p("};\n");
            o.p("pub const NoteParams = struct {\n");
            param_decls(module->params, true);
            o.p("};\n");
            o.p("\n");
            for (size_t j = 0; j < mr.fields.size(); j++) o.p(strf("field%zu: ", j) + module_name(mr.fields[j]) + ",\n");
            for (size_t j = 0; j < mr.delays.size(); j++) o.p(strf("delay%zu: zang.Delay(%zu),\n", j, mr.delays[j]));
            for (size_t j = 0; j < mr.note_trackers.size(); j++) o.p(strf("tracker%zu: zang.Notes(_track%zu.Params).NoteTracker,\n", j, mr.note_trackers[j]));
            for (size_t j = 0; j < mr.triggers.size(); j++) o.p(strf("trigger%zu: zang.Trigger(_track%zu.Params),\n", j, mr.triggers[j]));
            o.p("\n");
            o.p(strf("pub fn init() _module%zu {\n", mi));
            o.p("return .{\n");
            for (size_t j = 0; j < mr.fields.size(); j++) o.p(strf(".field%zu = ", j) + module_name(mr.fields[j]) + ".init(),\n");
            for (size_t j = 0; j < mr.delays.size(); j++) o.p(strf(".delay%zu = zang.Delay(%zu).init(),\n", j, mr.delays[j]));
            for (size_t j = 0; j < mr.note_trackers.size(); j++)
                o.p(strf(".tracker%zu = zang.Notes(_track%zu.Params).NoteTracker.init(&_track%zu.notes),\n", j, mr.note_trackers[j], mr.note_trackers[j]));
            for (size_t j = 0; j < mr.triggers.size(); j++) o.p(strf(".trigger%zu = zang.Trigger(_track%zu.Params).init(),\n", j, mr.triggers[j]));
            o.p("};\n");
            o.p("}\n");
            o.p("\n");
            o.p(strf("pub fn paint(self: *_module%zu, span: zang.Span, outputs: [num_outputs][]f32, temps: [num_temps][]f32, note_id_changed: bool, params: Params) void {\n", mi));
            for (const Instr &ins : mr.instructions) instruction(mr, ins, "span", "note_id_changed");
            o.p("}\n");
            o.p("};\n");
        }
        return o.text;
    }
};

struct HipBackendError { std::string message; };

std::string f32_literal(float xf) {
    const double x = (double)xf;
    if (x != x) return "__builtin_nanf(\"\")";
    if (isinf(x)) return x < 0 ? "-__builtin_inff()" : "__builtin_inff()";
    const char *sign = signbit(x) ? "-" : "";
    if (x == 0.0) return std::string(sign) + "0x0.0p+0f";
    int e;
    const double m = frexp(fabs(x), &e);
    const uint64_t frac = (uint64_t)ldexp(m * 2.0 - 1.0, 52);
    return strf("%s0x1.%013llxp%+df", sign, (unsigned long long)frac, e - 1);
}

struct Val {
    enum Kind { buf, flt, boolean, en, curve } kind = flt;
    std::string expr;
    std::string tag;
    bool tag_literal = false;
    std::shared_ptr<Val> payload;
    std::string count;
    bool computed = false;
    std::string cob_b, cob_c;
    uint64_t sines = 0;
};

const uint64_t kAllSines = ~0ull;
const size_t kMaxSines = 63;
static bool linear_input(const std::string &module, const std::string &param) {
    return (module == "Filter" || module == "Decimator") && param == "input";
}

size_t state_words(const std::string &name) {
    static const std::map<std::string, size_t> w = {{"SineOsc", 1}, {"PulseOsc", 1}, {"TriSawOsc", 2}, {"Noise", 8}, {"Envelope", 4}, {"Gate", 0},
                                                    {"Filter", 2}, {"Decimator", 2}, {"Distortion", 0}, {"Cycle", 1}, {"Portamento", 3}, {"Curve", 4}};
    auto it = w.find(name);
    if (it == w.end()) throw HipBackendError{"builtin module " + name + " is not supported by the HIP backend"};
    return it->second;
}
const size_t kTrackWords = 3;

struct InitItem { bool noise; size_t word; size_t k; float value; };

struct Part {
    Lines lines;
    int cost = 1, walk = 0;
    bool stateful = false;
    bool owner = false;
};
struct Unit {
    Lines text;
    std::vector<Part> parts;
    std::vector<std::string> ztemps;
    bool opaque = false;
    bool stateful = false;
    int cost = 1;
    int walk = 0;
    std::vector<size_t> ends, stores, quiets;
};
struct Mark { size_t ends, stores, quiets, units, frame; };

struct Kernel {
    std::string name;
    std::vector<HipParam> params;
    Lines pro, frame, epi_ends, epi_stores;
    std::set<size_t> pro_begin;
    std::map<size_t, std::pair<std::string, std::string>> pro_split;
    std::vector<Unit> units;
    Mark mark() const { return Mark{epi_ends.size(), epi_stores.size(), quiet_terms.size(), units.size(), frame.size()}; }
    void unit_done(const Mark &m, Unit u) {
        for (size_t i = m.ends; i < epi_ends.size(); i++) u.ends.push_back(i);
        for (size_t i = m.stores; i < epi_stores.size(); i++) u.stores.push_back(i);
        for (size_t i = m.quiets; i < quiet_terms.size(); i++) u.quiets.push_back(i);
        units.push_back(std::move(u));
    }
    void collapse(const Mark &m) {
        Unit u;
        u.opaque = u.stateful = true;
        u.cost = 4;
        for (size_t i = m.units; i < units.size(); i++) u.cost += units[i].cost;
        u.walk = u.cost;
        units.resize(m.units);
        u.text.assign(frame.begin() + (long)m.frame, frame.end());
        unit_done(m, std::move(u));
    }
    std::vector<InitItem> init;
    std::set<size_t> tracks;
    Lines temps;
    std::vector<size_t> rows;
    size_t words = 0, noise_fields = 0, uid = 0;
    bool rings = false;
    bool walk_reads_computed = false;
    Lines quiet_terms;
    size_t nsines = 0;
    uint64_t exact_sines = 0;
    std::string fresh(const std::string &stem) { uid++; return stem + std::to_string(uid); }
    size_t zuid = 0;
    std::string zfresh(const std::string &stem) { zuid++; return stem + std::to_string(zuid); }
    size_t alloc(size_t n) { const size_t w = words; words += n; return w; }
    long sine_source(uint64_t &bit) {
        if (nsines >= kMaxSines) { bit = 0; return -1; }
        bit = 1ull << nsines;
        return (long)nsines++;
    }
    void sink(const Val &v) { if (v.kind == Val::buf) exact_sines |= v.sines; }
};

struct ModuleCtx {
    Kernel &k;
    size_t module_index;
    std::vector<Val> env;
    std::string outvar, nic, prefix;
    std::map<size_t, std::string> tnames;
    std::map<size_t, bool> heavy;
    std::map<size_t, std::pair<std::string, std::string>> cobsrc;
    std::map<size_t, uint64_t> srcs;
    uint64_t outsines = 0;
    Lines *begin_sink, *end_sink;
    std::string rel = "(i - L.start)", length = "SPAN_LEN";
    const std::map<size_t, Val> *track = nullptr;
    ModuleCtx(Kernel &k_, size_t mi, std::vector<Val> env_, std::string outvar_, std::string nic_, std::string prefix_, const ModuleCtx *parent)
        : k(k_), module_index(mi), env(std::move(env_)), outvar(std::move(outvar_)), nic(std::move(nic_)), prefix(std::move(prefix_)) {
        begin_sink = parent ? parent->begin_sink : &k.pro;
        end_sink = parent ? parent->end_sink : &k.epi_ends;
        if (parent) { rel = parent->rel; length = parent->length; }
    }
    std::string tname(size_t i) {
        auto it = tnames.find(i);
        if (it != tnames.end()) return it->second;
        const std::string n = prefix + "t" + std::to_string(i);
        tnames[i] = n;
        k.temps.push_back(n);
        return n;
    }
    std::string fname(size_t i) const { return prefix + "f" + std::to_string(i); }
};

struct BeginSink {
    ModuleCtx &mc;
    void push_back(const std::string &l) const {
        if (mc.begin_sink == &mc.k.pro) mc.k.pro_begin.insert(mc.k.pro.size());
        mc.begin_sink->push_back(l);
    }
};

static std::string resolve_sines(const std::string &line, uint64_t tolerant) {
    std::string out;
    size_t at = 0;
    for (;;) {
        const size_t b = line.find('\x01', at);
        if (b == std::string::npos) { out += line.substr(at); return out; }
        const size_t bar = line.find('|', b), e = line.find('\x02', b);
        out += line.substr(at, b - at);
        const char kind = line[b + 1];
        const unsigned long sid = strtoul(line.substr(b + 2, bar - b - 2).c_str(), nullptr, 10);
        const std::string payload = line.substr(bar + 1, e - bar - 1);
        const bool tol = (tolerant >> sid) & 1;
        if (kind == 'O') {
            if (payload == "1") out += tol ? ", (ZS_T ? 2 : 1)" : "";
            else out += tol ? ", (ZS_T ? 2 : (int)!ZS_Q)" : ", !ZS_Q";
        } else {
            out += tol ? "(ZS_T ? zsinf_tol(" + payload + ") : zsinf(" + payload + "))" : "zsinf(" + payload + ")";
        }
        at = e + 1;
    }
}

class HipEmitter {
public:
    const CompiledScript &s;
    explicit HipEmitter(const CompiledScript &cs) : s(cs) {}

    Val val(ModuleCtx &mc, const Res &r) {
        Val v;
        switch (r.kind) {
        case RK::temp_buffer: {
            v.kind = Val::buf; v.expr = mc.tname(r.index);
            auto it = mc.heavy.find(r.index);
            v.computed = it == mc.heavy.end() ? true : it->second;
            auto ss = mc.srcs.find(r.index);
            v.sines = ss == mc.srcs.end() ? kAllSines : ss->second;
            auto cs = mc.cobsrc.find(r.index);
            if (cs != mc.cobsrc.end()) { v.cob_b = cs->second.first; v.cob_c = cs->second.second; }
            return v;
        }
        case RK::temp_float: v.kind = Val::flt; v.expr = mc.fname(r.index); return v;
        case RK::literal_number: v.kind = Val::flt; v.expr = f32_literal(r.num.value); return v;
        case RK::literal_boolean: v.kind = Val::boolean; v.expr = r.bval ? "true" : "false"; return v;
        case RK::literal_enum_value:
            v.kind = Val::en; v.tag = r.label; v.tag_literal = true;
            if (r.payload) v.payload = std::make_shared<Val>(val(mc, *r.payload));
            return v;
        case RK::literal_curve: v.kind = Val::curve; v.expr = strf("zs_curve%zu", r.index); v.count = std::to_string(s.pr.curves[r.index].points.size()); return v;
        case RK::self_param: return mc.env[r.index];
        case RK::track_param: return mc.track->at(r.index);
        default: throw HipBackendError{"internal: value kind"};
        }
    }
    static std::string enum_tag(const Val &v, const BuiltinEnum &en) {
        if (v.tag_literal) {
            for (size_t i = 0; i < en.values.size(); i++) if (en.values[i].label == v.tag) return std::to_string(i);
            throw HipBackendError{"internal: enum label"};
        }
        return v.tag;
    }
    static std::string enum_payload(const Val &v) { return v.payload ? v.payload->expr : "0.0f"; }
    static Lines put_lines(ModuleCtx &mc, const Dest &d, const std::string &expr, bool zero_first, bool heavy, uint64_t sines) {
        if (!d.output) {
            mc.heavy[d.index] = heavy;
            mc.srcs[d.index] = sines;
            mc.cobsrc.erase(d.index);
            const std::string t = mc.tname(d.index);
            if (zero_first) return {t + " = 0.0f;", t + " = " + t + " + (" + expr + ");"};
            return {t + " = " + expr + ";"};
        }
        mc.outsines |= sines;
        return {mc.outvar + " = " + mc.outvar + " + (" + expr + ");"};
    }
    static void put(ModuleCtx &mc, const Dest &d, const std::string &expr, bool zero_first, bool heavy = false, uint64_t sines = 0, int cost = 1) {
        Kernel &k = mc.k;
        const Mark mk = k.mark();
        Unit u;
        u.text = put_lines(mc, d, expr, zero_first, heavy, sines);
        u.cost = cost + (zero_first ? 1 : 0);
        if (d.output && mc.outvar == "o") {
            const std::string zo = k.zfresh("zo");
            u.ztemps.push_back(zo);
            Part a, w;
            a.lines = {zo + " = " + expr + ";"};
            a.cost = u.cost; a.owner = true;
            w.lines = {"o = o + (" + zo + ");"};
            u.parts = {a, w};
        }
        append(k.frame, u.text);
        k.unit_done(mk, std::move(u));
    }
    static int op_cost(const std::string &op) {
        if (op == "sin" || op == "cos") return 36;
        if (op == "pow") return 90;
        if (op == "div") return 10;
        if (op == "sqrt") return 8;
        if (op == "max" || op == "min") return 2;
        return 1;
    }
    static std::string un(const std::string &op, const std::string &a) {
        if (op == "abs") return "fabsf(" + a + ")";
        if (op == "cos") return "zcosf(" + a + ")";
        if (op == "neg") return "-(" + a + ")";
        if (op == "sin") return "zsinf(" + a + ")";
        return "sqrtf(" + a + ")";
    }
    static std::string bin(const std::string &op, const std::string &a, const std::string &b) {
        if (op == "add") return "(" + a + ") + (" + b + ")";
        if (op == "sub") return "(" + a + ") - (" + b + ")";
        if (op == "mul") return "(" + a + ") * (" + b + ")";
        if (op == "div") return "(" + a + ") / (" + b + ")";
        if (op == "pow") return "zpowf(" + a + ", " + b + ")";
        if (op == "max") return "zs_max(" + a + ", " + b + ")";
        return "zs_min(" + a + ", " + b + ")";
    }

    void call_builtin(ModuleCtx &mc, const Instr &ins, const Module &callee, const std::vector<Res> &args) {
        Kernel &k = mc.k;
        const Mark mk = k.mark();
        const std::string &name = callee.builtin_name;
        std::map<std::string, Val> a;
        for (size_t i = 0; i < callee.params.size(); i++) a[callee.params[i].name] = val(mc, args[i]);
        {
            static const std::map<std::string, std::vector<std::string>> state_inputs = {
                {"SineOsc", {"freq"}}, {"PulseOsc", {"freq"}}, {"TriSawOsc", {"freq"}}, {"Cycle", {"speed"}},
                {"Filter", {"input", "cutoff", "res"}}, {"Decimator", {"input"}}};
            auto si = state_inputs.find(name);
            if (si != state_inputs.end())
                for (const std::string &pn : si->second) {
                    auto it = a.find(pn);
                    if (it != a.end() && it->second.kind == Val::buf && it->second.computed) k.walk_reads_computed = true;
                }
        }
        uint64_t out_sines = 0;
        for (const auto &pv : a) {
            if (linear_input(name, pv.first)) out_sines |= pv.second.kind == Val::buf ? pv.second.sines : 0;
            else k.sink(pv.second);
        }
        const std::string o = k.fresh("m");
        const size_t w = k.alloc(state_words(name));
        Lines &decl = k.pro, &ends = *mc.end_sink, &epi = k.epi_stores;
        const BeginSink pro{mc};
        Lines frame;
        std::string painted, value;
        const char *oc = o.c_str();
        auto ld_f = [&](const char *field, size_t word) {
            decl.push_back(strf("%s.%s = zs_ld_f(L.state, %zu, V, v);", oc, field, word));
            epi.push_back(strf("zs_st_f(L.state, %zu, V, v, %s.%s);", word, oc, field));
        };
        auto ld_u = [&](const char *field, size_t word, const char *cast) {
            decl.push_back(strf("%s.%s = %szs_ld_u(L.state, %zu, V, v);", oc, field, cast, word));
            epi.push_back(strf("zs_st_u(L.state, %zu, V, v, (uint32_t)%s.%s);", word, oc, field));
        };
        struct Cob { bool is_buf; std::string c, i; };
        auto cob = [](const Val &v) { return v.kind == Val::buf ? Cob{true, "0.0f", v.expr} : Cob{false, v.expr, v.expr}; };
        auto tf = [](bool b) { return b ? "true" : "false"; };
        auto painted_pair = [&]() {
            const std::string cv = k.fresh("cv"), cp = k.fresh("cp");
            return std::make_pair(cv, cp);
        };
        const std::string sr = a.count("sample_rate") ? a["sample_rate"].expr : "";

        if (name == "SineOsc") {
            const Cob f = cob(a["freq"]), ph = cob(a["phase"]);
            decl.push_back("SineOscLane " + o + ";");
            ld_f("t", w);
            pro.push_back(o + ".begin(" + sr + ", " + f.c + ");");
            const Val &fv = a["freq"];
            const bool quiet = !ph.is_buf && mc.begin_sink == &k.pro && (!f.is_buf || !fv.cob_b.empty());
            if (quiet && !f.is_buf) k.quiet_terms.push_back(o + ".small_args(" + ph.c + ", (float)zs_n)");
            if (quiet && f.is_buf) k.quiet_terms.push_back("(!" + fv.cob_b + " && " + o + ".small_args_step(" + fv.cob_c + " * " + o + ".inv_sr, " + ph.c + ", (float)zs_n))");
            uint64_t bit = 0;
            const long sid = k.sine_source(bit);
            out_sines |= bit;
            const std::string mode = sid < 0 ? std::string(quiet ? ", !ZS_Q" : "") : strf("\x01" "O%ld|%s\x02", sid, quiet ? "!ZS_Q" : "1");
            value = o + ".frame<" + tf(f.is_buf) + mode + ">(" + (f.is_buf ? f.i : "0.0f") + ", " + ph.i + ")";
            ends.push_back(o + ".end();");
        } else if (name == "Cycle") {
            const Cob sp = cob(a["speed"]);
            decl.push_back("CycleLane " + o + ";");
            ld_f("t", w);
            pro.push_back(o + ".begin(" + sr + ", " + sp.c + ");");
            value = o + ".frame<" + tf(sp.is_buf) + ">(" + (sp.is_buf ? sp.i : "0.0f") + ")";
        } else if (name == "PulseOsc" || name == "TriSawOsc") {
            const Cob f = cob(a["freq"]);
            decl.push_back(name + "Lane " + o + ";");
            ld_u("cnt", w, "");
            if (name == "TriSawOsc") ld_f("t", w + 1);
            if (f.is_buf) {
                pro.push_back(o + ".begin_ctrl(" + sr + ", " + a["color"].expr + ");");
                if (name == "PulseOsc") {
                    auto pp = painted_pair();
                    frame.push_back("float " + pp.first + " = 0.0f;");
                    frame.push_back("const bool " + pp.second + " = " + o + ".frame_ctrl(" + f.i + ", " + pp.first + ");");
                    painted = pp.second; value = pp.first;
                } else {
                    value = o + ".frame_ctrl(" + f.i + ")";
                    ends.push_back(o + ".end_ctrl();");
                }
            } else {
                pro.push_back(o + ".begin_const(" + sr + ", " + f.c + ", " + a["color"].expr + ");");
                auto pp = painted_pair();
                frame.push_back("float " + pp.first + " = 0.0f;");
                frame.push_back("const bool " + pp.second + " = " + o + ".frame_const(" + pp.first + ");");
                painted = pp.second; value = pp.first;
            }
        } else if (name == "Noise") {
            decl.push_back("NoiseLane " + o + ";");
            for (size_t j = 0; j < 4; j++) {
                decl.push_back(strf("%s.r.s%zu = zs_ld_u64(L.state, %zu, V, v);", oc, j, w + 2 * j));
                epi.push_back(strf("zs_st_u64(L.state, %zu, V, v, %s.r.s%zu);", w + 2 * j, oc, j));
            }
            pro.push_back(o + ".begin();");
            k.init.push_back(InitItem{true, w, k.noise_fields, 0.0f});
            k.noise_fields++;
            const std::string tag = enum_tag(a["color"], *callee.params[0].type.en);
            if (tag == "0" || tag == "1") value = o + ".frame<" + tf(tag == "1") + ">()";
            else value = "((" + tag + ") == 1u ? " + o + ".frame<true>() : " + o + ".frame<false>())";
        } else if (name == "Envelope") {
            const std::string t0 = enum_tag(a["attack"], *callee.params[1].type.en), t1 = enum_tag(a["decay"], *callee.params[2].type.en),
                              t2 = enum_tag(a["release"], *callee.params[3].type.en);
            const bool one_tag = a["attack"].tag_literal && a["decay"].tag_literal && a["release"].tag_literal && t0 == t1 && t1 == t2 && t0 != "0";
            decl.push_back(one_tag ? "EnvLaneT<1, " + t0 + "> " + o + ";" : "EnvLane " + o + ";");
            ld_u("state", w, "");
            ld_f("t", w + 1);
            ld_f("last_value", w + 2);
            ld_f("start", w + 3);
            pro.push_back(o + ".sample_rate = " + sr + "; " + o + ".sustain_volume = " + a["sustain_volume"].expr + "; " + o + ".note_on = " + a["note_on"].expr + ";");
            const char *stages[3] = {"attack", "decay", "release"};
            for (int i = 0; i < 3; i++)
                pro.push_back(o + "." + stages[i] + " = CurveP{(uint32_t)(" + enum_tag(a[stages[i]], *callee.params[1 + i].type.en) + "), " + enum_payload(a[stages[i]]) + "};");
            pro.push_back(o + ".begin(" + mc.nic + ");");
            auto pp = painted_pair();
            frame.push_back("float " + pp.first + " = 0.0f;");
            const std::string step = mc.begin_sink == &k.pro ? "frame_sq<ZS_Q>(" + pp.first + ", zs_walk)" : "frame(" + pp.first + ")";
            if (mc.begin_sink == &k.pro) k.quiet_terms.push_back(o + ".quiet(zs_n)");
            frame.push_back("const bool " + pp.second + " = " + o + "." + step + ";");
            painted = pp.second; value = pp.first;
        } else if (name == "Gate") {
            painted = a["note_on"].expr; value = "1.0f";
        } else if (name == "Filter") {
            const Cob c = cob(a["cutoff"]), r = cob(a["res"]);
            decl.push_back("FilterLane " + o + ";");
            ld_f("l", w);
            ld_f("b", w + 1);
            pro.push_back(o + ".begin((uint32_t)(" + enum_tag(a["type"], *callee.params[1].type.en) + "), " + c.c + ", " + r.c + ");");
            value = o + ".frame<" + tf(c.is_buf) + ", " + tf(r.is_buf) + ">(" + a["input"].expr + ", " + (c.is_buf ? c.i : "0.0f") + ", " + (r.is_buf ? r.i : "0.0f") + ")";
        } else if (name == "Decimator") {
            decl.push_back("DecimatorLane " + o + ";");
            ld_f("dval", w);
            ld_f("dcount", w + 1);
            k.init.push_back(InitItem{false, w + 1, 0, 1.0f});
            pro.push_back(o + ".begin(" + sr + ", " + a["fake_sample_rate"].expr + ");");
            auto pp = painted_pair();
            frame.push_back("float " + pp.first + " = 0.0f;");
            frame.push_back("const bool " + pp.second + " = " + o + ".frame(" + a["input"].expr + ", " + pp.first + ");");
            painted = pp.second; value = pp.first;
            ends.push_back(o + ".end();");
        } else if (name == "Distortion") {
            decl.push_back("DistortionLane " + o + ";");
            pro.push_back(o + ".begin((uint32_t)(" + enum_tag(a["type"], *callee.params[1].type.en) + "), " + a["ingain"].expr + ", " + a["outgain"].expr + ", " + a["offset"].expr + ");");
            value = o + ".frame(" + a["input"].expr + ")";
        } else if (name == "Portamento") {
            decl.push_back("PortamentoLane " + o + ";");
            ld_f("t", w);
            ld_f("last", w + 1);
            ld_f("st", w + 2);
            pro.push_back(o + ".begin(" + sr + ", (uint32_t)(" + enum_tag(a["curve"], *callee.params[1].type.en) + "), " + enum_payload(a["curve"]) + ", " + a["goal"].expr + ", " +
                          a["note_on"].expr + ", " + a["prev_note_on"].expr + ", " + mc.nic + ");");
            value = o + ".frame()";
        } else if (name == "Curve") {
            decl.push_back("CurveLane " + o + ";");
            decl.push_back("CurveTable " + o + "_tb;");
            ld_f("t", w);
            ld_u("cur", w + 1, "");
            ld_u("off", w + 2, "(int32_t)");
            ld_u("next", w + 3, "");
            pro.push_back(o + ".begin(" + o + "_tb, " + sr + ", (uint32_t)(" + enum_tag(a["function"], *callee.params[1].type.en) + "), " + a["curve"].expr + ", " + a["curve"].count + ", " +
                          mc.length + ", " + mc.nic + ");");
            auto pp = painted_pair();
            frame.push_back("float " + pp.first + " = 0.0f;");
            frame.push_back("const bool " + pp.second + " = " + o + ".frame(" + o + "_tb, " + mc.rel + ", " + pp.first + ");");
            painted = pp.second; value = pp.first;
        } else {
            throw HipBackendError{"builtin module " + name + " is not supported by the HIP backend"};
        }
        std::string target;
        if (!ins.out.output) {
            mc.heavy[ins.out.index] = true;
            mc.srcs[ins.out.index] = out_sines;
            mc.cobsrc.erase(ins.out.index);
            target = mc.tname(ins.out.index);
            frame.insert(frame.begin(), target + " = 0.0f;");
        } else {
            mc.outsines |= out_sines;
            target = mc.outvar;
        }
        const std::string addl = target + " = " + target + " + (" + value + ");";
        Unit u;
        u.stateful = state_words(name) > 0;
        u.cost = builtin_cost(name, a, u.walk);
        auto writer_add = [&](const std::string &val, const std::string &flag) {
            const std::string zo = k.zfresh("zo");
            u.ztemps.push_back(zo);
            Lines give = {zo + " = " + val + ";"};
            Part w;
            w.lines = {"o = o + (" + zo + ");"};
            if (!flag.empty()) {
                const std::string zp = k.zfresh("zp");
                u.ztemps.push_back(zp);
                give.push_back(zp + " = (" + flag + ") ? 1.0f : 0.0f;");
                w.lines = {"if (" + zp + " != 0.0f) o = o + (" + zo + ");"};
            }
            return std::make_pair(give, w);
        };
        if (name == "Filter") {
            const Cob c = cob(a["cutoff"]), r = cob(a["res"]);
            const std::string fi = k.zfresh("zfi"), fl = k.zfresh("zfl"), fb = k.zfresh("zfb"), fh = k.zfresh("zfh");
            for (const std::string &t : {fi, fl, fb, fh}) u.ztemps.push_back(t);
            Part pa, pb, pc;
            pa.lines = {fi + " = " + o + ".pre(" + a["input"].expr + ");"};
            pa.cost = 1;
            pb.lines = {"{", "    const SvfOut zs_s = " + o + ".core<" + tf(c.is_buf) + ", " + tf(r.is_buf) + ">(" + fi + ", " + (c.is_buf ? c.i : "0.0f") + ", " + (r.is_buf ? r.i : "0.0f") + ");",
                        "    " + fl + " = zs_s.l;", "    " + fb + " = zs_s.b;", "    " + fh + " = zs_s.h;", "}"};
            pb.cost = pb.walk = u.cost - 6; pb.stateful = pb.owner = true;
            const bool never_bypass = a["type"].tag_literal && a["type"].tag != "bypass";
            const std::string mix = never_bypass ? o + ".mix(" + fl + ", " + fb + ", " + fh + ")" : o + ".post(" + a["input"].expr + ", " + fl + ", " + fb + ", " + fh + ")";
            pc.cost = 5;
            if (target == "o") {
                auto gw = writer_add(mix, "");
                pc.lines = gw.first;
                u.parts = {pa, pb, pc, gw.second};
            } else {
                if (!ins.out.output) pc.lines.push_back(target + " = 0.0f;");
                pc.lines.push_back(target + " = " + target + " + (" + mix + ");");
                u.parts = {pa, pb, pc};
            }
        } else if (target == "o") {
            auto gw = writer_add(value, painted);
            Lines body = frame;
            append(body, gw.first);
            Part pa;
            pa.lines.push_back("{");
            append(pa.lines, indent(body));
            pa.lines.push_back("}");
            pa.cost = u.cost; pa.walk = u.walk; pa.stateful = u.stateful; pa.owner = true;
            u.parts = {pa, gw.second};
        }
        frame.push_back(painted.empty() ? addl : "if (" + painted + ") " + addl);
        u.text.push_back("{");
        append(u.text, indent(frame));
        u.text.push_back("}");
        append(k.frame, u.text);
        k.unit_done(mk, std::move(u));
    }
    static int builtin_cost(const std::string &name, std::map<std::string, Val> &a, int &walk) {
        auto is_buf = [&](const char *p) { auto it = a.find(p); return it != a.end() && it->second.kind == Val::buf; };
        auto ret = [&](int cost, int w) { walk = w; return cost; };
        if (name == "SineOsc") return is_buf("freq") ? ret(42, 3) : ret(40, 2);
        if (name == "PulseOsc") return is_buf("freq") ? ret(34, 34) : ret(16, 2);
        if (name == "TriSawOsc") {
            if (is_buf("freq")) return ret(24, 12);
            const std::string &c = a["color"].expr;
            return c == "0x0.0p+0f" || c == "-0x0.0p+0f" ? ret(17, 2) : ret(42, 2);
        }
        if (name == "Noise") return a["color"].tag_literal && a["color"].tag == "white" ? ret(24, 20) : ret(44, 20);
        if (name == "Envelope") return ret(16, 5);
        if (name == "Filter") { const int c = 21 + (is_buf("cutoff") ? 3 : 0) + (is_buf("res") ? 4 : 0); return ret(c, c); }
        if (name == "Decimator") return ret(8, 8);
        if (name == "Distortion") return a["type"].tag_literal && a["type"].tag == "clip" ? ret(6, 0) : ret(40, 0);
        if (name == "Portamento") return ret(14, 9);
        if (name == "Curve") return ret(10, 4);
        if (name == "Cycle") return ret(5, 5);
        return ret(2, 0);
    }

    void instruction(ModuleCtx &mc, const ModuleResult &mr, const Instr &ins) {
        Kernel &k = mc.k;
        switch (ins.kind) {
        case IK::copy_buffer: {
            const Val src = val(mc, ins.src);
            put(mc, ins.out, src.expr, false, src.computed, src.sines);
            if (!ins.out.output && !src.cob_b.empty()) mc.cobsrc[ins.out.index] = {src.cob_b, src.cob_c};
            break;
        }
        case IK::float_to_buffer: put(mc, ins.out, val(mc, ins.src).expr, false); break;
        case IK::cob_to_buffer: {
            const Val &src = mc.env[ins.in_self_param];
            put(mc, ins.out, src.expr, false, src.computed, src.sines);
            if (!ins.out.output && !src.cob_b.empty()) mc.cobsrc[ins.out.index] = {src.cob_b, src.cob_c};
            break;
        }
        case IK::arith_float: case IK::arith_float_float: {
            const std::string expr = ins.kind == IK::arith_float ? un(ins.op, val(mc, ins.a).expr) : bin(ins.op, val(mc, ins.a).expr, val(mc, ins.b).expr);
            if (mc.begin_sink == &k.pro) {
                k.pro_split[k.pro.size()] = {"float " + mc.fname(ins.out_float) + " = 0.0f;", mc.fname(ins.out_float) + " = " + expr + ";"};
                k.pro.push_back("const float " + mc.fname(ins.out_float) + " = " + expr + ";");
            } else {
                k.pro.push_back("float " + mc.fname(ins.out_float) + " = 0.0f;");
                mc.begin_sink->push_back(mc.fname(ins.out_float) + " = " + expr + ";");
            }
            break;
        }
        case IK::arith_buffer: {
            const Val va = val(mc, ins.a);
            std::string expr = un(ins.op, va.expr);
            uint64_t sines = va.sines;
            if (ins.op == "sin" || ins.op == "cos" || ins.op == "sqrt") {
                k.sink(va);
                sines = 0;
                if (ins.op == "sin") {
                    const long sid = k.sine_source(sines);
                    if (sid >= 0) expr = strf("\x01" "F%ld|", sid) + va.expr + "\x02";
                }
            }
            put(mc, ins.out, expr, false, va.computed || ins.op == "sin" || ins.op == "cos", sines, op_cost(ins.op));
            break;
        }
        case IK::arith_float_buffer: case IK::arith_buffer_float: case IK::arith_buffer_buffer: {
            const Val va = val(mc, ins.a), vb = val(mc, ins.b);
            std::string a = va.expr, b = vb.expr;
            const bool heavy = va.computed || vb.computed || ins.op == "pow";
            const uint64_t sa = va.kind == Val::buf ? va.sines : 0, sb = vb.kind == Val::buf ? vb.sines : 0;
            uint64_t sines = sa | sb;
            if (ins.op == "pow") { k.sink(va); k.sink(vb); sines = 0; }
            else if (ins.op == "div") { k.sink(vb); sines = sa; }
            if (ins.op == "add" || ins.op == "mul") {
                if (ins.kind == IK::arith_float_buffer) std::swap(a, b);
                put(mc, ins.out, bin(ins.op, a, b), true, heavy, sines, op_cost(ins.op));
            } else {
                put(mc, ins.out, bin(ins.op, a, b), false, heavy, sines, op_cost(ins.op));
            }
            break;
        }
        case IK::call: {
            const size_t callee_index = mr.fields[ins.field_index];
            const Module &callee = s.pr.modules[callee_index];
            if (callee.builtin) { call_builtin(mc, ins, callee, ins.args); break; }
            std::vector<Val> env;
            for (const Res &r : ins.args) env.push_back(val(mc, r));
            std::string outvar;
            if (!ins.out.output) {
                mc.heavy[ins.out.index] = true; mc.cobsrc.erase(ins.out.index); outvar = mc.tname(ins.out.index);
                const Mark mk = k.mark();
                Unit u;
                u.text = {outvar + " = 0.0f;"};
                append(k.frame, u.text);
                k.unit_done(mk, std::move(u));
            } else outvar = mc.outvar;
            ModuleCtx sub(k, callee_index, env, outvar, mc.nic, k.fresh(mc.prefix + "c") + "_", &mc);
            module_body(sub);
            if (!ins.out.output) mc.srcs[ins.out.index] = sub.outsines;
            else mc.outsines |= sub.outsines;
            break;
        }
        case IK::track_call: track_call(mc, mr, ins); break;
        case IK::delay: delay(mc, mr, ins); break;
        }
    }

    void delay(ModuleCtx &mc, const ModuleResult &mr, const Instr &ins) {
        Kernel &k = mc.k;
        const Mark mk = k.mark();
        const size_t n = mr.delays[ins.delay_index];
        if (n < 1) throw HipBackendError{"delay of 0 samples"};
        const size_t w_idx = k.alloc(1), w_ring = k.alloc(n);
        const std::string d = k.fresh("d");
        k.pro.push_back(strf("uint32_t %s_idx = zs_ld_u(L.state, %zu, V, v);", d.c_str(), w_idx));
        k.epi_stores.push_back(strf("zs_st_u(L.state, %zu, V, v, %s_idx);", w_idx, d.c_str()));
        if (!ins.out.output) k.frame.push_back(mc.tname(ins.out.index) + " = 0.0f;");
        const std::string fb = mc.tname(ins.feedback_temp), fbout = mc.tname(ins.feedback_out_temp);
        mc.srcs[ins.feedback_temp] = kAllSines;
        Lines begins, ends, body;
        Lines *sb = mc.begin_sink, *se = mc.end_sink;
        const std::string srel = mc.rel, slen = mc.length;
        const std::string rel = d + "_rel", length = d + "_len";
        const Lines head = {"const uint32_t " + rel + " = " + srel + strf(" %% %zuu;", n),
                            "const uint32_t " + length + strf(" = min(%zuu, ", n) + slen + " - (" + srel + " - " + rel + "));"};
        Lines saved_frame;
        saved_frame.swap(k.frame);
        mc.begin_sink = &begins; mc.end_sink = &ends; mc.rel = rel; mc.length = length;
        try {
            for (const Instr &sub : ins.instructions) instruction(mc, mr, sub);
        } catch (...) {
            mc.begin_sink = sb; mc.end_sink = se; mc.rel = srel; mc.length = slen;
            throw;
        }
        body.swap(k.frame);
        k.frame.swap(saved_frame);
        mc.begin_sink = sb; mc.end_sink = se; mc.rel = srel; mc.length = slen;
        k.rings = true;
        const std::string slot = strf("L.state[(size_t)(%zuu + %s_idx) * V + v]", w_ring, d.c_str());
        append(k.frame, head);
        if (!begins.empty()) { k.frame.push_back("if (" + rel + " == 0u) {"); append(k.frame, indent(begins)); k.frame.push_back("}"); }
        k.frame.push_back(fbout + " = 0.0f;");
        k.frame.push_back(fb + " = 0.0f;");
        if (n >= 2) {
            const char *dc = d.c_str();
            k.pro.push_back(strf("float %s_pre = zu2f(L.state[(size_t)(%zuu + %s_idx) * V + v]);", dc, w_ring, dc));
            k.frame.push_back(strf("const float %s_cur = %s_pre;", dc, dc));
            k.frame.push_back(strf("%s_pre = zu2f(L.state[(size_t)(%zuu + (%s_idx + 1u == %zuu ? 0u : %s_idx + 1u)) * V + v]);", dc, w_ring, dc, n, dc));
            k.frame.push_back(fb + " = " + fb + " + " + d + "_cur;");
        } else {
            k.frame.push_back(fb + " = " + fb + " + zu2f(" + slot + ");");
        }
        append(k.frame, body);
        k.frame.push_back(slot + " = zf2u(" + fbout + ");");
        k.frame.push_back(strf("%s_idx = %s_idx + 1u == %zuu ? 0u : %s_idx + 1u;", d.c_str(), d.c_str(), n, d.c_str()));
        if (!ends.empty()) { k.frame.push_back("if (" + rel + " + 1u == " + length + ") {"); append(k.frame, indent(ends)); k.frame.push_back("}"); }
        k.collapse(mk);
    }

    void track_call(ModuleCtx &mc, const ModuleResult &mr, const Instr &ins) {
        Kernel &k = mc.k;
        const Mark mk = k.mark();
        const size_t ti = ins.track_index;
        const Track &track = s.pr.tracks[ti];
        const Module &module = s.pr.modules[mc.module_index];
        const size_t w = k.alloc(kTrackWords);
        const std::string t = k.fresh("trk");
        const char *tc = t.c_str();
        k.tracks.insert(ti);
        std::map<size_t, Val> env;
        Lines loads;
        for (size_t pi = 0; pi < track.params.size(); pi++) {
            const ModuleParam &p = track.params[pi];
            Val v;
            if (p.type.kind == PK::constant) {
                k.pro.push_back(strf("float %s_p%zu = 0.0f;", tc, pi));
                loads.push_back(strf("%s_p%zu = zs_track%zu_p%zu[%s_note];", tc, pi, ti, pi, tc));
                v.kind = Val::flt; v.expr = strf("%s_p%zu", tc, pi);
            } else if (p.type.kind == PK::boolean) {
                k.pro.push_back(strf("bool %s_p%zu = false;", tc, pi));
                loads.push_back(strf("%s_p%zu = zs_track%zu_p%zu[%s_note] != 0;", tc, pi, ti, pi, tc));
                v.kind = Val::boolean; v.expr = strf("%s_p%zu", tc, pi);
            } else if (p.type.kind == PK::one_of) {
                k.pro.push_back(strf("uint32_t %s_p%zu = 0u; float %s_q%zu = 0.0f;", tc, pi, tc, pi));
                loads.push_back(strf("%s_p%zu = zs_track%zu_p%zu[%s_note]; %s_q%zu = zs_track%zu_q%zu[%s_note];", tc, pi, ti, pi, tc, tc, pi, ti, pi, tc));
                v.kind = Val::en; v.tag = strf("%s_p%zu", tc, pi);
                v.payload = std::make_shared<Val>();
                v.payload->kind = Val::flt; v.payload->expr = strf("%s_q%zu", tc, pi);
            } else if (p.type.kind == PK::curve) {
                k.pro.push_back(strf("const zh_curve_node *%s_p%zu = nullptr; uint32_t %s_q%zu = 0u;", tc, pi, tc, pi));
                loads.push_back(strf("%s_p%zu = zs_track%zu_p%zu[%s_note]; %s_q%zu = zs_track%zu_q%zu[%s_note];", tc, pi, ti, pi, tc, tc, pi, ti, pi, tc));
                v.kind = Val::curve; v.expr = strf("%s_p%zu", tc, pi); v.count = strf("%s_q%zu", tc, pi);
            } else {
                const char *kn = p.type.kind == PK::buffer ? "buffer" : "constant_or_buffer";
                throw HipBackendError{"track param `" + p.name + "`: type " + kn + " is not supported by the HIP backend"};
            }
            env[pi] = v;
        }
        std::string reset = mc.nic;
        for (size_t i = 0; i < module.params.size(); i++)
            if (module.params[i].name == "note_on") { reset = "(" + mc.env[i].expr + " && " + mc.nic + ")"; break; }
        k.pro.push_back("TrackLane " + t + ";");
        k.pro.push_back(strf("%s.next = zs_ld_u(L.state, %zu, V, v); %s.t = zs_ld_f(L.state, %zu, V, v); %s.cur = zs_ld_u(L.state, %zu, V, v);", tc, w, tc, w + 1, tc, w + 2));
        k.pro.push_back(strf("uint32_t %s_k = 0u, %s_note = 0u; bool %s_new = false;", tc, tc, tc));
        k.epi_stores.push_back(strf("zs_st_u(L.state, %zu, V, v, %s.next); zs_st_f(L.state, %zu, V, v, %s.t); zs_st_u(L.state, %zu, V, v, %s.cur);", w, tc, w + 1, tc, w + 2, tc));
        BeginSink{mc}.push_back(t + strf(".begin(zs_track%zu_t, %zuu, (", ti, track.notes.size()) + mc.env[0].expr + ") / (" + val(mc, ins.speed).expr + "), " + mc.length + ", " + reset + ");");
        BeginSink{mc}.push_back(t + "_k = 0u;");
        Lines begins, ends, body;
        Lines *sb = mc.begin_sink, *se = mc.end_sink;
        const std::string srel = mc.rel, slen = mc.length, snic = mc.nic;
        const std::map<size_t, Val> *strack = mc.track;
        Lines saved_frame;
        saved_frame.swap(k.frame);
        mc.begin_sink = &begins; mc.end_sink = &ends;
        mc.rel = strf("(%s_rel - %s.s_start[%s_k])", tc, tc, tc);
        mc.length = strf("(%s.s_end[%s_k] - %s.s_start[%s_k])", tc, tc, tc, tc);
        mc.nic = t + "_new"; mc.track = &env;
        auto restore = [&]() { mc.begin_sink = sb; mc.end_sink = se; mc.rel = srel; mc.length = slen; mc.nic = snic; mc.track = strack; };
        try {
            for (const Instr &sub : ins.instructions) instruction(mc, mr, sub);
        } catch (...) { restore(); throw; }
        body.swap(k.frame);
        k.frame.swap(saved_frame);
        restore();
        const std::string I = "    ";
        k.frame.push_back(strf("const uint32_t %s_rel = ", tc) + srel + ";");
        k.frame.push_back(strf("if (%s_k < %s.n && %s_rel == %s.s_start[%s_k]) {", tc, tc, tc, tc, tc));
        k.frame.push_back(I + strf("%s_note = %s.s_note[%s_k];", tc, tc, tc));
        k.frame.push_back(I + t + "_new = " + reset + strf(" || %s.s_new[%s_k];", tc, tc));
        append(k.frame, indent(loads));
        append(k.frame, indent(begins));
        k.frame.push_back("}");
        k.frame.push_back(strf("const bool %s_on = %s_k < %s.n && %s_rel >= %s.s_start[%s_k];", tc, tc, tc, tc, tc, tc));
        k.frame.push_back(strf("if (%s_on) {", tc));
        append(k.frame, indent(body));
        k.frame.push_back("}");
        k.frame.push_back(strf("if (%s_on && %s_rel + 1u == %s.s_end[%s_k]) {", tc, tc, tc, tc));
        append(k.frame, indent(ends));
        k.frame.push_back(I + t + "_k++;");
        k.frame.push_back("}");
        k.collapse(mk);
    }

    Lines track_tables(size_t ti) {
        const Track &track = s.pr.tracks[ti];
        const auto &notes = s.track_results[ti];
        const size_t n = track.notes.empty() ? 1 : track.notes.size();
        auto join = [](const Lines &parts, const char *empty) {
            std::string o;
            for (size_t i = 0; i < parts.size(); i++) o += (i ? ", " : "") + parts[i];
            return o.empty() ? std::string(empty) : o;
        };
        Lines out, parts;
        for (const TrackNote &x : track.notes) parts.push_back(f32_literal(x.t.value));
        out.push_back(strf("__device__ const float zs_track%zu_t[%zu] = {", ti, n) + join(parts, "0.0f") + "};");
        for (size_t pi = 0; pi < track.params.size(); pi++) {
            const ModuleParam &p = track.params[pi];
            Lines a, b;
            if (p.type.kind == PK::constant) {
                for (size_t ni = 0; ni < track.notes.size(); ni++) a.push_back(f32_literal(notes[ni][pi].num.value));
                out.push_back(strf("__device__ const float zs_track%zu_p%zu[%zu] = {", ti, pi, n) + join(a, "0.0f") + "};");
            } else if (p.type.kind == PK::boolean) {
                for (size_t ni = 0; ni < track.notes.size(); ni++) a.push_back(notes[ni][pi].bval ? "1" : "0");
                out.push_back(strf("__device__ const unsigned char zs_track%zu_p%zu[%zu] = {", ti, pi, n) + join(a, "0") + "};");
            } else if (p.type.kind == PK::one_of) {
                for (size_t ni = 0; ni < track.notes.size(); ni++) {
                    const Res &r = notes[ni][pi];
                    size_t idx = 0;
                    while (p.type.en->values[idx].label != r.label) idx++;
                    a.push_back(std::to_string(idx));
                    b.push_back(r.payload ? f32_literal(r.payload->num.value) : "0.0f");
                }
                out.push_back(strf("__device__ const unsigned int zs_track%zu_p%zu[%zu] = {", ti, pi, n) + join(a, "0") + "};");
                out.push_back(strf("__device__ const float zs_track%zu_q%zu[%zu] = {", ti, pi, n) + join(b, "0.0f") + "};");
            } else if (p.type.kind == PK::curve) {
                for (size_t ni = 0; ni < track.notes.size(); ni++) {
                    a.push_back(strf("zs_curve%zu", notes[ni][pi].index));
                    b.push_back(std::to_string(s.pr.curves[notes[ni][pi].index].points.size()));
                }
                out.push_back(strf("__device__ const zh_curve_node *const zs_track%zu_p%zu[%zu] = {", ti, pi, n) + join(a, "nullptr") + "};");
                out.push_back(strf("__device__ const unsigned int zs_track%zu_q%zu[%zu] = {", ti, pi, n) + join(b, "0") + "};");
            }
        }
        return out;
    }

    void module_body(ModuleCtx &mc) {
        const ModuleResult &mr = s.module_results[mc.module_index];
        for (const Instr &ins : mr.instructions) instruction(mc, mr, ins);
    }

    void kernel(Kernel &k, size_t module_index) {
        const Module &module = s.pr.modules[module_index];
        if (module.params.size() > ZH_SCRIPT_MAX_PARAMS)
            throw HipBackendError{strf("module has %zu params; the loader passes at most 16", module.params.size())};
        std::vector<Val> env;
        for (size_t i = 0; i < module.params.size(); i++) {
            const ModuleParam &p = module.params[i];
            Val v;
            const char *kind = "";
            switch (p.type.kind) {
            case PK::constant:
                kind = "constant";
                k.pro_split[k.pro.size()] = {strf("float P%zu = 0.0f;", i), strf("P%zu = zs_span_f(L.p[%zu], S.p[%zu], zs_kv, v);", i, i, i)};
                k.pro.push_back(strf("const float P%zu = zs_const(L.p[%zu], v);", i, i));
                v.kind = Val::flt; v.expr = strf("P%zu", i);
                break;
            case PK::boolean:
                kind = "boolean";
                k.pro_split[k.pro.size()] = {strf("bool P%zu = false;", i), strf("P%zu = zs_span_b(L.p[%zu], S.p[%zu], zs_kv, v);", i, i, i)};
                k.pro.push_back(strf("const bool P%zu = zs_bool(L.p[%zu], v);", i, i));
                v.kind = Val::boolean; v.expr = strf("P%zu", i);
                break;
            case PK::buffer: {
                kind = "buffer";
                const size_t j = k.rows.size();
                k.rows.push_back(i);
                v.kind = Val::buf; v.expr = strf("x[%zu]", j);
                break;
            }
            case PK::constant_or_buffer: {
                kind = "constant_or_buffer";
                const size_t j = k.rows.size();
                k.rows.push_back(i);
                k.pro_split[k.pro.size()] = {strf("const bool P%zu_b = L.p[%zu].is_buffer != 0; float P%zu_c = 0.0f;", i, i, i),
                                             strf("P%zu_c = zs_span_f(L.p[%zu], S.p[%zu], zs_kv, v);", i, i, i)};
                k.pro.push_back(strf("const bool P%zu_b = L.p[%zu].is_buffer != 0; const float P%zu_c = zs_const(L.p[%zu], v);", i, i, i, i));
                v.kind = Val::buf; v.expr = strf("(P%zu_b ? x[%zu] : P%zu_c)", i, j, i);
                v.cob_b = strf("P%zu_b", i); v.cob_c = strf("P%zu_c", i);
                break;
            }
            case PK::curve:
                kind = "curve";
                v.kind = Val::curve; v.expr = strf("reinterpret_cast<const zh_curve_node *>(L.p[%zu].pf)", i); v.count = strf("L.p[%zu].u", i);
                break;
            case PK::one_of:
                kind = "one_of";
                k.pro_split[k.pro.size()] = {strf("uint32_t P%zu_tag = 0u; float P%zu_f = 0.0f;", i, i),
                                             strf("P%zu_tag = zs_span_tag(L.p[%zu], S.p[%zu], zs_kv); P%zu_f = zs_span_payload(L.p[%zu], S.p[%zu], zs_kv);", i, i, i, i, i, i)};
                k.pro.push_back(strf("const uint32_t P%zu_tag = L.p[%zu].u; const float P%zu_f = L.p[%zu].f;", i, i, i, i));
                v.kind = Val::en; v.tag = strf("P%zu_tag", i);
                v.payload = std::make_shared<Val>();
                v.payload->kind = Val::flt; v.payload->expr = strf("P%zu_f", i);
                break;
            }
            env.push_back(v);
            k.params.push_back(HipParam{p.name, kind, p.type.en ? p.type.en->name : ""});
        }
        ModuleCtx mc(k, module_index, env, "o", "NIC", "", nullptr);
        module_body(mc);
    }

    struct RUnit {
        Lines lines;
        std::set<std::string> reads, writes;
        std::set<size_t> rows;
        bool touches_o = false, stateful = false, opaque = false, floating = false;
        int cost = 1, walk = 0, role = -1;
        std::vector<size_t> ends, stores, quiets;
    };
    struct Role {
        std::vector<size_t> items;
        std::set<int> preds;
        int cost = 0, lag = 0;
        int walk = 0, rep = 1;
        int walk_sum = 0;
        std::vector<size_t> tin, tout;
    };
    struct Transfer {
        long def;
        std::string var;
        int from = 0;
        std::set<int> to;
        int depth = 2, src_lag = 0;
        size_t off = 0;
    };
    static constexpr long kOIn = -1000000;
    static constexpr int kMaxProducers = 5;

    template <class CB> static void scan_idents(const std::string &l, size_t from, size_t to, CB &&cb) {
        size_t i = from;
        while (i < to) {
            const char c = l[i];
            if ((c >= '0' && c <= '9')) {
                size_t j = i + 1;
                while (j < to && (isalnum((unsigned char)l[j]) || l[j] == '.' || ((l[j] == '+' || l[j] == '-') && (l[j - 1] == 'p' || l[j - 1] == 'P' || l[j - 1] == 'e' || l[j - 1] == 'E')))) j++;
                i = j;
            } else if (isalpha((unsigned char)c) || c == '_') {
                size_t j = i + 1;
                while (j < to && (isalnum((unsigned char)l[j]) || l[j] == '_')) j++;
                const bool member = i > 0 && l[i - 1] == '.';
                if (!member) cb(l.substr(i, j - i), i, j);
                i = j;
            } else {
                i++;
            }
        }
    }
    static void analyze(RUnit &u, const std::set<std::string> &temps) {
        std::set<std::string> written;
        auto read = [&](const std::string &id, size_t, size_t e, const std::string &l) {
            if (id == "o") { u.touches_o = true; return; }
            if (id == "x" && e < l.size() && l[e] == '[') { u.rows.insert((size_t)strtoul(l.c_str() + e + 1, nullptr, 10)); return; }
            if (!temps.count(id)) return;
            if (u.opaque) { u.reads.insert(id); u.writes.insert(id); return; }
            if (!written.count(id)) u.reads.insert(id);
        };
        for (const std::string &l : u.lines) {
            size_t p = l.find_first_not_of(' ');
            if (p == std::string::npos) continue;
            size_t cond0 = 0, cond1 = 0;
            bool conditional = false;
            if (!u.opaque && l.compare(p, 4, "if (") == 0) {
                int depth = 0;
                size_t q = p + 3;
                for (; q < l.size(); q++) { if (l[q] == '(') depth++; else if (l[q] == ')' && --depth == 0) break; }
                cond0 = p + 4; cond1 = q; conditional = true;
                p = l.find_first_not_of(' ', q + 1);
                if (p == std::string::npos) p = l.size();
            }
            std::string target;
            size_t rhs = p;
            if (!u.opaque) {
                size_t j = p;
                while (j < l.size() && (isalnum((unsigned char)l[j]) || l[j] == '_')) j++;
                const std::string id = l.substr(p, j - p);
                if (l.compare(j, 3, " = ") == 0 && (temps.count(id) || id == "o")) { target = id; rhs = j + 3; }
            }
            scan_idents(l, cond0, cond1, [&](const std::string &id, size_t b, size_t e) { read(id, b, e, l); });
            scan_idents(l, rhs, l.size(), [&](const std::string &id, size_t b, size_t e) { read(id, b, e, l); });
            if (target == "o") u.touches_o = true;
            else if (!target.empty()) {
                if (conditional && !written.count(target)) u.reads.insert(target);
                written.insert(target);
                u.writes.insert(target);
            }
        }
    }

    Lines role_kernel(const Kernel &k, size_t nin, size_t ni, const Lines &preamble, size_t lds_budget, bool &worth) {
        std::set<std::string> temps(k.temps.begin(), k.temps.end());
        std::vector<RUnit> us;
        for (const Unit &u : k.units) {
            temps.insert(u.ztemps.begin(), u.ztemps.end());
            if (u.parts.empty()) {
                RUnit r;
                r.stateful = u.stateful; r.opaque = u.opaque; r.cost = u.cost; r.walk = u.walk;
                r.ends = u.ends; r.stores = u.stores; r.quiets = u.quiets;
                r.lines = u.text;
                us.push_back(std::move(r));
                continue;
            }
            for (const Part &p : u.parts) {
                RUnit r;
                r.stateful = p.stateful; r.cost = p.cost; r.walk = p.walk;
                if (p.owner) { r.ends = u.ends; r.stores = u.stores; r.quiets = u.quiets; }
                r.lines = p.lines;
                us.push_back(std::move(r));
            }
        }
        for (RUnit &u : us) analyze(u, temps);
        const size_t n = us.size();
        std::vector<std::vector<std::pair<size_t, std::string>>> deps(n);
        {
            std::map<std::string, size_t> last;
            for (size_t i = 0; i < n; i++) {
                for (const std::string &t : us[i].reads) { auto it = last.find(t); if (it != last.end()) deps[i].push_back({it->second, t}); }
                for (const std::string &t : us[i].writes) last[t] = i;
            }
        }
        std::vector<Role> roles(1);
        auto reaches = [&](int a, int b) {
            std::vector<int> stack = {b};
            std::set<int> seen;
            while (!stack.empty()) {
                const int r = stack.back(); stack.pop_back();
                if (r == a) return true;
                if (!seen.insert(r).second) continue;
                for (int p : roles[(size_t)r].preds) stack.push_back(p);
            }
            return false;
        };
        for (size_t i = 0; i < n; i++) {
            RUnit &u = us[i];
            std::set<int> P;
            {
                std::vector<size_t> stack = {i};
                std::set<size_t> seen;
                while (!stack.empty()) {
                    const size_t x = stack.back(); stack.pop_back();
                    for (const auto &d : deps[x]) {
                        if (!us[d.first].floating) P.insert(us[d.first].role);
                        else if (seen.insert(d.first).second) stack.push_back(d.first);
                    }
                }
            }
            auto recurrence = [&](int r) { return r > 0 && roles[(size_t)r].cost > 0 && roles[(size_t)r].walk_sum == roles[(size_t)r].cost; };
            bool floats = !u.stateful && !u.opaque && !u.touches_o && u.cost < 8 && !P.count(0);
            if (floats && !P.empty()) {
                floats = false;
                std::vector<int> sinks;
                for (int r : P) {
// ... 64 lines not shown
                if (state[(size_t)r]) continue;
                state[(size_t)r] = 1;
                stack.push_back({r, true});
                for (int p : roles[(size_t)r].preds) if (!state[(size_t)p]) stack.push_back({p, false});
            }
            for (int r : order) {
                int lag = (!role_rows[(size_t)r].empty() || r == 0) ? 1 : 0;
                for (int p : roles[(size_t)r].preds) lag = std::max(lag, roles[(size_t)p].lag + 1);
                roles[(size_t)r].lag = lag;
            }
            for (auto it = order.rbegin(); it != order.rend(); ++it) {
                const int r = *it;
                int latest = -1;
                for (int s = 0; s < NR; s++) if (roles[(size_t)s].preds.count(r)) latest = latest < 0 ? roles[(size_t)s].lag - 1 : std::min(latest, roles[(size_t)s].lag - 1);
                if (latest > roles[(size_t)r].lag) roles[(size_t)r].lag = latest;
            }
        }
        const int max_lag = roles[0].lag;
        std::vector<Transfer> tr;
        auto transfer = [&](long def, const std::string &var, int from, int to) -> size_t {
            for (size_t t = 0; t < tr.size(); t++) if (tr[t].def == def && tr[t].var == var) { tr[t].to.insert(to); return t; }
            Transfer x; x.def = def; x.var = var; x.from = from; x.to.insert(to);
            tr.push_back(x);
            return tr.size() - 1;
        };
        for (int r = 0; r < NR; r++) {
            for (size_t j : role_rows[(size_t)r]) transfer(-1 - (long)j, strf("x[%zu]", j), -1, r);
            for (size_t i : roles[(size_t)r].items)
                for (const auto &d : deps[i])
                    if (!us[d.first].floating && us[d.first].role != r) transfer((long)d.first, d.second, us[d.first].role, r);
        }
        const size_t oin = transfer(kOIn, "o", -1, 0);
        size_t bufs_no_oin = 0, bufs = 0;
        for (size_t t = 0; t < tr.size(); t++) {
            Transfer &x = tr[t];
            int first = 1 << 30, last = 0;
            for (int r : x.to) { first = std::min(first, roles[(size_t)r].lag); last = std::max(last, roles[(size_t)r].lag); }
            x.src_lag = x.from < 0 ? first - 1 : roles[(size_t)x.from].lag;
            x.depth = last - x.src_lag + 1;
            x.off = bufs;
            bufs += (size_t)x.depth;
            if (t != oin) bufs_no_oin = bufs;
        }
        int ch = 32;
        while (ch > 4 && bufs * (size_t)ch * 256 > lds_budget) ch /= 2;
        if (bufs * (size_t)ch * 256 > lds_budget) return {};
        const size_t tile = (size_t)ch / 4 * 64;
        for (int r = 0; r < NR; r++) {
            Role &R = roles[(size_t)r];
            for (size_t t = 0; t < tr.size(); t++) {
                if (t != oin && tr[t].to.count(r)) R.tin.push_back(t);
                if (tr[t].from == r) R.tout.push_back(t);
            }
            if (r == 0) R.tin.push_back(oin);
        }
        std::vector<std::vector<size_t>> loaders;
        for (size_t t = 0; t < tr.size(); t++) {
            if (tr[t].from >= 0) continue;
            if (loaders.empty() || loaders.back().size() == 4) loaders.emplace_back();
            loaders.back().push_back(t);
        }
        size_t nwaves = loaders.size() + (size_t)NR;
        {
            int pace = 14;
            std::vector<bool> can((size_t)NR, false);
            for (int r = 0; r < NR; r++) {
                Role &R = roles[(size_t)r];
                bool ok = r != 0;
                for (size_t i : R.items) { R.walk += us[i].walk; if (us[i].opaque) ok = false; }
                can[(size_t)r] = ok && R.walk * 2 <= R.cost;
                pace = std::max(pace, can[(size_t)r] ? R.walk : R.cost);
            }
            for (int r = 1; r < NR; r++) {
                Role &R = roles[(size_t)r];
                if (!can[(size_t)r]) continue;
                while (R.rep < 4 && R.rep * 2 <= ch / 4 && nwaves + (size_t)R.rep <= 16 && R.walk + (R.cost - R.walk) / R.rep > pace + pace / 8) { nwaves += (size_t)R.rep; R.rep *= 2; }
            }
        }
        int total = 0, longest = 0;
        for (int r = 0; r < NR; r++) { total += roles[(size_t)r].cost; longest = std::max(longest, roles[(size_t)r].walk + (roles[(size_t)r].cost - roles[(size_t)r].walk) / roles[(size_t)r].rep); }
        const bool hint = (k.rings || k.walk_reads_computed) && longest * 10 <= total * 7;
        worth = hint;
        int work = 0;
        for (int r = 0; r < NR; r++) work += roles[(size_t)r].rep * roles[(size_t)r].walk + (roles[(size_t)r].cost - roles[(size_t)r].walk);
        const bool hint_many = hint && work * 4 <= total * 5 && nwaves <= 9 && longest * 7 <= total * 2;

        const std::string I = "    ";
        const char *nc = k.name.c_str();
        Lines out;
        out.push_back(strf("// role-wave form: %zu waves (%zu loader, %d roles, the last the writer), %d frames per tile, %zu tile buffers", nwaves, loaders.size(), NR, ch, bufs));
        out.push_back(strf("extern \"C\" __device__ const uint32_t zs_pc_info_%s[4] = {%zuu, %zuu, %zuu, %uu};", nc, nwaves * 64, bufs * (size_t)ch * 256,
                           bufs_no_oin * (size_t)ch * 256, (hint ? 1u : 0u) | (hint_many ? 2u : 0u)));
        out.push_back(strf("extern \"C\" __global__ void __launch_bounds__(%zu) zs_paint_pc_%s(const ZsLaunch L) {", nwaves * 64, nc));
        out.push_back(I + "extern __shared__ float4 zs_lds[];");
        out.push_back(I + "const uint32_t zs_lane = threadIdx.x & 63u, zs_role = (uint32_t)__builtin_amdgcn_readfirstlane((int)(threadIdx.x >> 6));");
        out.push_back(I + "const uint32_t V = L.V;");
        out.push_back(I + "const uint32_t zs_v0 = blockIdx.x * 64 + zs_lane;");
        out.push_back(I + "const bool zs_live = zs_v0 < V;");
        out.push_back(I + "const uint32_t v = zs_live ? zs_v0 : V - 1;      // a lane past the last voice runs voice V - 1 again");
        append(out, preamble);
        out.push_back(I + "const bool zs_walk = false; (void)zs_walk;");
        out.push_back(I + "const uint32_t zs_nfr = L.end - L.start;");
        out.push_back(I + strf("const uint32_t zs_steps = (zs_nfr + %du) / %du + %du;", ch - 1, ch, max_lag));
        out.push_back(I + "const bool zs_zf = (L.flags & ZH_PAINT_ZERO_FIRST) != 0;");
        auto tile_list = [&](const std::vector<size_t> &ts) {
            std::string s;
            for (size_t t : ts) s += (s.empty() ? "" : ", ") + strf("{%zuu, %du}", tr[t].off * tile, tr[t].depth);
            return s.empty() ? std::string("{0u, 1u}") : s;
        };
        size_t wave = 0;
        for (const auto &ld : loaders) {
            out.push_back(I + (wave ? "} else if" : "if") + strf(" (zs_role == %zuu) {", wave));
            std::string src, str, vof, lag;
            for (size_t t : ld) {
                const bool o = tr[t].def == kOIn;
                const size_t j = o ? 0 : (size_t)(-1 - tr[t].def);
                src += (src.empty() ? "" : ", ") + (o ? std::string("L.out") : strf("ins[%zu]", j));
                str += (str.empty() ? "" : ", ") + (o ? std::string("zs_zf ? (size_t)0 : (size_t)L.ostride") : strf("istr[%zu]", j));
                vof += (vof.empty() ? "" : ", ") + (o ? std::string("v * 4u") : strf("ivo[%zu]", j));
                lag += (lag.empty() ? "" : ", ") + strf("%du", tr[t].src_lag);
            }
            out.push_back(I + I + strf("const ZsTileRef zs_to[%zu] = {", ld.size()) + tile_list(ld) + "};");
            out.push_back(I + I + strf("const float *zs_src[%zu] = {", ld.size()) + src + "};");
            out.push_back(I + I + strf("const size_t zs_str[%zu] = {", ld.size()) + str + "};");
            out.push_back(I + I + strf("const uint32_t zs_vof[%zu] = {", ld.size()) + vof + "};");
            out.push_back(I + I + strf("const uint32_t zs_lag[%zu] = {", ld.size()) + lag + "};");
            out.push_back(I + I + strf("zs_loader_run<%d, %zu>(zs_lds, zs_lane, zs_steps, L.start, zs_nfr, zs_to, zs_src, zs_str, zs_vof, zs_lag);", ch, ld.size()));
            wave++;
        }
        std::vector<int> seq;
        for (int r = 1; r < NR; r++) seq.push_back(r);
        seq.push_back(0);
        for (int r : seq) {
            const Role &R = roles[(size_t)r];
            if (R.rep == 1) out.push_back(I + (wave ? "} else if" : "if") + strf(" (zs_role == %zuu) {", wave) + strf("      // lag %d, ~%d instructions per frame", R.lag, R.cost));
            else out.push_back(I + (wave ? "} else if" : "if") + strf(" (zs_role >= %zuu && zs_role < %zuu) {", wave, wave + (size_t)R.rep) +
                               strf("      // lag %d, ~%d instructions per frame, ~%d of them state: %d waves, each computes every %s group of four frames", R.lag, R.cost, R.walk, R.rep,
                                    R.rep == 2 ? "second" : R.rep == 3 ? "third" : "fourth"));
            out.push_back(I + I + strf("const uint32_t zs_rep = zs_role - %zuu; (void)zs_rep;", wave));
            wave += (size_t)R.rep;
            const size_t NIN = R.tin.size(), NOUT = R.tout.size();
            out.push_back(I + I + strf("const ZsTileRef zs_ti[%zu] = {", NIN ? NIN : 1) + tile_list(R.tin) + "};");
            out.push_back(I + I + strf("const ZsTileRef zs_to[%zu] = {", NOUT ? NOUT : 1) + tile_list(R.tout) + "};");
            Lines quiet;
            for (size_t i : R.items) for (size_t q : us[i].quiets) quiet.push_back(k.quiet_terms[q]);
            std::string all;
            for (const std::string &t : quiet) all += (all.empty() ? "" : " && ") + t;
            const bool two = !quiet.empty();
            if (two) out.push_back(I + I + "auto zs_quiet = [&](int zs_n) ZH_INLINE_LAMBDA -> bool { return " + all + "; };");
            else out.push_back(I + I + "auto zs_quiet = [](int) ZH_INLINE_LAMBDA -> bool { return false; };");
            out.push_back(I + I + strf("auto zs_body = [&](auto zs_q, uint32_t i, const float (&zs_in)[%zu], float (&zs_out)[%zu], float &o) ZH_INLINE_LAMBDA {", NIN ? NIN : 1, NOUT ? NOUT : 1));
            const std::string B = I + I + I;
            out.push_back(B + "constexpr bool ZS_Q = decltype(zs_q)::value; (void)ZS_Q;");
            out.push_back(B + "(void)i; (void)zs_in; (void)zs_out; (void)o;");
            out.push_back(B + strf("float x[%zu]; (void)x;", ni));
            {
                std::string decl;
                for (const std::string &t : temps) decl += (decl.empty() ? "float " : ", ") + t + " = 0.0f";
                if (!decl.empty()) out.push_back(B + decl + ";");
                std::string use;
                for (const std::string &t : temps) use += "(void)" + t + "; ";
                if (!use.empty()) out.push_back(B + use);
            }
            std::set<size_t> loaded;
            for (size_t a = 0; a < NIN; a++) if (tr[R.tin[a]].def < 0 && tr[R.tin[a]].def != kOIn) { out.push_back(B + tr[R.tin[a]].var + strf(" = zs_in[%zu];", a)); loaded.insert(R.tin[a]); }
            for (size_t i : R.items) {
                for (const auto &d : deps[i]) {
                    if (us[d.first].floating || us[d.first].role == r) continue;
                    for (size_t a = 0; a < NIN; a++) {
                        const Transfer &x = tr[R.tin[a]];
                        if (x.def == (long)d.first && x.var == d.second && loaded.insert(R.tin[a]).second) out.push_back(B + x.var + strf(" = zs_in[%zu];", a));
                    }
                }
                for (const std::string &l : us[i].lines) out.push_back(B + resolve_sines(l, 0));
                for (size_t b = 0; b < NOUT; b++) if (tr[R.tout[b]].def == (long)i) out.push_back(B + strf("zs_out[%zu] = ", b) + tr[R.tout[b]].var + ";");
            }
            out.push_back(I + I + "};");
            size_t body_lines = 0;
            for (size_t i : R.items) body_lines += us[i].lines.size();
            const int uq = body_lines <= 12 ? ch / 4 : body_lines <= 40 ? 2 : 1;
            const std::string lam = strf("[&](uint32_t i, const float (&a)[%zu], float (&b)[%zu], float &o) ZH_INLINE_LAMBDA ", NIN ? NIN : 1, NOUT ? NOUT : 1);
            out.push_back(I + I + strf("zs_role_run<%d, %zu, %zu, %d, %s, %d>(zs_lds, zs_lane, %du, zs_rep, zs_steps, L.start, zs_nfr, zs_ti, zs_to, L.out, L.ostride, v * 4u, zs_zf,", ch, NIN, NOUT,
                                       R.rep > 1 ? std::max(uq / R.rep * R.rep, R.rep) : uq, r == 0 ? "true" : "false", R.rep, R.lag));
            out.push_back(I + I + I + lam + "{ zs_body(zs_tag<false>{}, i, a, b, o); }, zs_quiet,");
            out.push_back(I + I + I + lam + strf("{ zs_body(zs_tag<%s>{}, i, a, b, o); });", two ? "true" : "false"));
            Lines fin;
            for (size_t i : R.items) for (size_t e : us[i].ends) fin.push_back(k.epi_ends[e]);
            for (size_t i : R.items) for (size_t e : us[i].stores) fin.push_back(k.epi_stores[e]);
            if (!fin.empty()) {
                out.push_back(I + I + (R.rep > 1 ? "if (zs_live && zs_rep == 0u) {" : "if (zs_live) {"));
                for (const std::string &l : fin) out.push_back(I + I + I + l);
                out.push_back(I + I + "}");
            }
        }
        out.push_back(I + "}");
        out.push_back("}");
        return out;
    }

    Lines spans_kernel(const Kernel &k, size_t nin, size_t ni, int unroll) {
        const std::string I = "    ", II = I + I;
        auto rel = [](std::string l) {
            const std::string from = "(i - L.start)", to = "(i - zs_s0)";
            for (size_t at = l.find(from); at != std::string::npos; at = l.find(from, at + to.size())) l.replace(at, from.size(), to);
            return l;
        };
        Lines out, once, begin, ends, frame;
        for (size_t j = 0; j < k.pro.size(); j++) {
            auto sp = k.pro_split.find(j);
            if (sp != k.pro_split.end()) { once.push_back(sp->second.first); begin.push_back(sp->second.second); }
            else if (k.pro_begin.count(j)) begin.push_back(rel(k.pro[j]));
            else once.push_back(k.pro[j]);
        }
        for (const std::string &l : k.epi_ends) ends.push_back(rel(l));
        for (const std::string &l : k.frame) frame.push_back(rel(resolve_sines(l, 0)));
        out.push_back(strf("extern \"C\" __global__ void __launch_bounds__(64) zs_paint_spans_%s(const ZsLaunch L, const ZsSpans S) {", k.name.c_str()));
        out.push_back(I + "const uint32_t V = L.V;");
        out.push_back(I + "const bool zs_live = blockIdx.x * 64 + threadIdx.x < V;");
        out.push_back(I + "const uint32_t v = zs_live ? blockIdx.x * 64 + threadIdx.x : V - 1;   // (past the last voice: its loads, no sub-spans, no stores)");
        out.push_back(I + "bool NIC = false;");
        out.push_back(I + "uint32_t SPAN_LEN = 0u, zs_s0 = 0u;");
        out.push_back(I + "(void)NIC; (void)SPAN_LEN; (void)zs_s0;");
        std::string nulls, zeros;
        for (size_t j = 0; j < ni; j++) { nulls += j ? ", nullptr" : "nullptr"; zeros += j ? ", 0" : "0"; }
        out.push_back(I + strf("const float *ins[%zu] = {", ni) + nulls + "};");
        out.push_back(I + strf("size_t istr[%zu] = {", ni) + zeros + "};");
        out.push_back(I + strf("uint32_t ivo[%zu] = {", ni) + zeros + "};");
        for (size_t j = 0; j < k.rows.size(); j++) out.push_back(I + strf("ins[%zu] = zs_row(L.p[%zu], v, istr[%zu], ivo[%zu]);", j, k.rows[j], j, j));
        append(out, indent(once));
        out.push_back(I + "bool zs_walk = false;");
        out.push_back(I + "auto zs_begin = [&](const size_t zs_kv) ZH_INLINE_LAMBDA {");
        out.push_back(II + "NIC = S.t.note_id_changed[zs_kv] != 0;");
        out.push_back(II + "zs_s0 = S.t.start[zs_kv];");
        out.push_back(II + "SPAN_LEN = S.t.end[zs_kv] - zs_s0;");
        append(out, indent(indent(begin)));
        out.push_back(I + "};");
        out.push_back(I + "auto zs_end = [&]() ZH_INLINE_LAMBDA {");
        append(out, indent(indent(ends)));
        out.push_back(I + "};");
        std::string all;
        for (const std::string &t : k.quiet_terms) all += (all.empty() ? "" : " && ") + t;
        out.push_back(I + strf("auto zs_body = [&](auto zs_q, uint32_t i, const float (&x)[%zu], float &o) ZH_INLINE_LAMBDA {", ni));
        out.push_back(II + "constexpr bool ZS_Q = decltype(zs_q)::value; (void)ZS_Q;");
        out.push_back(II + "(void)i; (void)x;");
        if (!k.temps.empty()) {
            std::string decl = "float ";
            for (size_t j = 0; j < k.temps.size(); j++) decl += (j ? ", " : "") + k.temps[j] + " = 0.0f";
            out.push_back(II + decl + ";");
        }
        append(out, indent(indent(frame)));
        out.push_back(I + "};");
        out.push_back(I + strf("auto zs_f = [&](uint32_t i, const float (&x)[%zu], float &o) ZH_INLINE_LAMBDA { zs_body(zs_tag<false>{}, i, x, o); };", ni));
        if (all.empty()) {
            out.push_back(I + strf("zs_span_walk<%d, %zu>(L, S, v, zs_live, ins, istr, ivo, zs_walk, zs_begin, zs_end, zs_f, [](int) { return false; }, zs_f);", unroll, nin));
        } else {
            out.push_back(I + "auto zs_quiet = [&](int zs_n) ZH_INLINE_LAMBDA -> bool { return " + all + "; };");
            out.push_back(I + strf("auto zs_fq = [&](uint32_t i, const float (&x)[%zu], float &o) ZH_INLINE_LAMBDA { zs_body(zs_tag<true>{}, i, x, o); };", ni));
            out.push_back(I + strf("zs_span_walk<%d, %zu>(L, S, v, zs_live, ins, istr, ivo, zs_walk, zs_begin, zs_end, zs_f, zs_quiet, zs_fq);", unroll, nin));
        }
        out.push_back(I + "if (!zs_live) return;");
        append(out, indent(k.epi_stores));
        out.push_back("}");
        return out;
    }

    std::string generate(const std::set<std::string> *only, std::vector<HipModuleMeta> &meta, int unroll_override, unsigned forms) {
        Lines out = {"// generated by zang_amd.zangscript (HIP backend) -- compile with zh_script_load / zh_script_compile",
                     "#include \"script_rt.hip.h\"", ""};
        for (size_t ci = 0; ci < s.pr.curves.size(); ci++) {
            std::string pts;
            for (size_t i = 0; i < s.pr.curves[ci].points.size(); i++) {
                const auto &p = s.pr.curves[ci].points[i];
                pts += (i ? ", " : "") + ("{" + f32_literal(p.second.value) + ", " + f32_literal(p.first.value) + "}");
            }
            out.push_back(strf("__device__ const zh_curve_node zs_curve%zu[] = {", ci) + (pts.empty() ? "{0.0f, 0.0f}" : pts) + "};");
        }
        std::set<size_t> used_tracks;
        const size_t table_at = out.size();
        for (const auto &em : s.exported_modules) {
            const std::string &name = em.first;
            if (only && !only->count(name)) continue;
            Kernel k;
            k.name = name;
            HipModuleMeta m;
            m.name = name;
            m.num_temps = s.module_results[em.second].num_temps;
            try {
                kernel(k, em.second);
            } catch (const HipBackendError &e) {
                m.error = e.message;
                meta.push_back(m);
                out.push_back("");
                out.push_back("// " + name + ": " + e.message);
                continue;
            }
            m.state_words = k.words; m.noise_fields = k.noise_fields; m.params = k.params;
            meta.push_back(m);
            used_tracks.insert(k.tracks.begin(), k.tracks.end());
            const size_t nin = k.rows.size(), ni = nin ? nin : 1;
            const int unroll = unroll_override ? unroll_override : (k.frame.size() <= 40 ? 8 : k.frame.size() <= 100 ? 4 : 2);
            const std::string I = "    ";
            const char *nc = name.c_str();
            out.push_back("");
            out.push_back(strf("extern \"C\" __device__ const uint32_t zs_ranges_ok_%s = %uu;", nc, (k.rings || k.walk_reads_computed) ? 0u : 1u));
            {
                std::vector<bool> stored(k.words, false);
                static const std::regex re("zs_st_(f|u|u64)\\(L\\.state, ([0-9]+), V, v,");
                auto scan = [&](const Lines &ls) {
                    for (const std::string &ln : ls)
                        for (std::sregex_iterator it(ln.begin(), ln.end(), re), end; it != end; ++it) {
                            const size_t w = (size_t)std::stoul((*it)[2].str());
                            if (w < stored.size()) stored[w] = true;
                            if ((*it)[1].str() == "u64" && w + 1 < stored.size()) stored[w + 1] = true;
                        }
                };
                scan(k.epi_ends); scan(k.epi_stores);
                size_t n_stored = 0;
                for (bool b : stored) n_stored += b ? 1 : 0;
                out.push_back(strf("extern \"C\" __device__ const uint32_t zs_state_words_stored_%s = %zuu;", nc, n_stored));
            }
            out.push_back(strf("extern \"C\" __global__ void zs_init_%s(uint32_t *__restrict__ st, uint32_t V, uint64_t first_seed) {", nc));
            out.push_back(I + "const uint32_t v = blockIdx.x * 64 + threadIdx.x;");
            out.push_back(I + "if (v >= V) return;");
            out.push_back(I + strf("for (uint32_t w = 0; w < %zuu; w++) st[(size_t)w * V + v] = 0u;", k.words));
            for (const InitItem &it : k.init) {
                if (!it.noise) {
                    out.push_back(I + strf("zs_st_f(st, %zu, V, v, ", it.word) + f32_literal(it.value) + ");");
                } else {
                    out.push_back(I + strf("{ ZXoshiro r; zxoshiro_seed(r, first_seed + (uint64_t)v * %zuu + %zuu);", k.noise_fields, it.k));
                    out.push_back(I + strf("  zs_st_u64(st, %zu, V, v, r.s0); zs_st_u64(st, %zu, V, v, r.s1); zs_st_u64(st, %zu, V, v, r.s2); zs_st_u64(st, %zu, V, v, r.s3); }",
                                           it.word, it.word + 2, it.word + 4, it.word + 6));
                }
            }
            out.push_back("}");
            out.push_back("");
            out.push_back(strf("extern \"C\" __global__ void __launch_bounds__(64) zs_paint_%s(const ZsLaunch L) {", nc));
            out.push_back(I + "const uint32_t v = blockIdx.x * 64 + threadIdx.x;");
            out.push_back(I + "const uint32_t V = L.V;");
            out.push_back(I + "if (v >= V) return;");
            Lines preamble;
            preamble.push_back(I + "const bool NIC = L.nic.get(v);");
            preamble.push_back(I + "const uint32_t SPAN_LEN = L.end - L.start;");
            preamble.push_back(I + "(void)NIC; (void)SPAN_LEN;");
            std::string nulls, zeros;
            for (size_t j = 0; j < ni; j++) { nulls += j ? ", nullptr" : "nullptr"; zeros += j ? ", 0" : "0"; }
            preamble.push_back(I + strf("const float *ins[%zu] = {", ni) + nulls + "};");
            preamble.push_back(I + strf("size_t istr[%zu] = {", ni) + zeros + "};");
            preamble.push_back(I + strf("uint32_t ivo[%zu] = {", ni) + zeros + "};");
            for (size_t j = 0; j < k.rows.size(); j++) preamble.push_back(I + strf("ins[%zu] = zs_row(L.p[%zu], v, istr[%zu], ivo[%zu]);", j, k.rows[j], j, j));
            append(preamble, indent(k.pro));
            append(out, preamble);
            out.push_back(I + "bool zs_walk = false; (void)zs_walk;");
            const bool two_bodies = !k.quiet_terms.empty();
            const std::string loop_call = I +
                strf("zs_frame_loop<%d, %zu>(L.out, v, L.ostride, ins, istr, ivo, L.start, L.end, (L.flags & ZH_PAINT_ZERO_FIRST) != 0, zs_walk,", unroll, nin);
            uint64_t tolerant = 0;
            for (size_t i = 0; i < k.nsines; i++) if (!((k.exact_sines >> i) & 1)) tolerant |= 1ull << i;
            Lines frame_lines;
            for (const std::string &l : k.frame) frame_lines.push_back(resolve_sines(l, tolerant));
            const std::string lam = I + strf("                     [&](uint32_t i, const float (&x)[%zu], float &o) ZH_INLINE_LAMBDA ", ni);
            std::string all;
            for (const std::string &t : k.quiet_terms) all += (all.empty() ? "" : " && ") + t;
            if (tolerant) {
                if (two_bodies) out.push_back(I + "auto zs_quiet = [&](int zs_n) ZH_INLINE_LAMBDA -> bool { return " + all + "; };");
                out.push_back(I + strf("auto zs_body = [&](auto zs_q, auto zs_t, uint32_t i, const float (&x)[%zu], float &o) ZH_INLINE_LAMBDA {", ni));
                out.push_back(I + I + "constexpr bool ZS_Q = decltype(zs_q)::value; (void)ZS_Q;");
                out.push_back(I + I + "constexpr bool ZS_T = decltype(zs_t)::value; (void)ZS_T;");
            } else if (two_bodies) {
                out.push_back(I + "auto zs_quiet = [&](int zs_n) ZH_INLINE_LAMBDA -> bool { return " + all + "; };");
                out.push_back(I + strf("auto zs_body = [&](auto zs_q, uint32_t i, const float (&x)[%zu], float &o) ZH_INLINE_LAMBDA {", ni));
                out.push_back(I + I + "constexpr bool ZS_Q = decltype(zs_q)::value; (void)ZS_Q;");
            } else {
                out.push_back(loop_call);
                out.push_back(lam + "{");
            }
            out.push_back(I + I + "(void)i; (void)x;");
            if (!k.temps.empty()) {
                std::string decl = "float ";
                for (size_t j = 0; j < k.temps.size(); j++) decl += (j ? ", " : "") + k.temps[j] + " = 0.0f";
                out.push_back(I + I + decl + ";");
            }
            append(out, indent(indent(frame_lines)));
            if (tolerant) {
                out.push_back(I + "};");
                for (const char *t : {"true", "false"}) {
                    out.push_back(I + (std::string(t) == "true" ? "if (L.flags & ZH_PAINT_TOLERANT) {" : "} else {"));
                    out.push_back(loop_call);
                    if (two_bodies) {
                        out.push_back(lam + strf("{ zs_body(zs_tag<false>{}, zs_tag<%s>{}, i, x, o); }, zs_quiet,", t));
                        out.push_back(lam + strf("{ zs_body(zs_tag<true>{}, zs_tag<%s>{}, i, x, o); });", t));
                    } else {
                        out.push_back(lam + strf("{ zs_body(zs_tag<false>{}, zs_tag<%s>{}, i, x, o); });", t));
                    }
                }
                out.push_back(I + "}");
            } else if (two_bodies) {
                out.push_back(I + "};");
                out.push_back(loop_call);
                out.push_back(lam + "{ zs_body(zs_tag<false>{}, i, x, o); }, zs_quiet,");
                out.push_back(lam + "{ zs_body(zs_tag<true>{}, i, x, o); });");
            } else {
                out.push_back(I + "});");
            }
            append(out, indent(k.epi_ends));
            append(out, indent(k.epi_stores));
            out.push_back("}");
            if (forms & ZH_ZSCRIPT_FORM_SPANS) { out.push_back(""); append(out, spans_kernel(k, nin, ni, unroll)); }
            if (forms & (ZH_ZSCRIPT_FORM_ROLES | ZH_ZSCRIPT_FORM_ROLES_WORTH)) {
                bool worth = false;
                const Lines pc = role_kernel(k, nin, ni, preamble, (forms & 4u) ? 131072 : 65536, worth);
                if (!pc.empty() && ((forms & ZH_ZSCRIPT_FORM_ROLES) || worth)) { out.push_back(""); append(out, pc); }
            }
        }
        Lines tables;
        for (size_t ti : used_tracks) append(tables, track_tables(ti));
        out.insert(out.begin() + (long)table_at, tables.begin(), tables.end());
        std::string text;
        for (const std::string &l : out) text += l + "\n";
        return text;
    }
};

}

std::string generate_zig(const CompiledScript &cs) { return ZigEmitter(cs).generate(); }
std::string generate_hip(const CompiledScript &cs, const std::set<std::string> *only, std::vector<HipModuleMeta> &meta, int unroll_override, unsigned forms) {
    return HipEmitter(cs).generate(only, meta, unroll_override, forms);
}

}

struct zh_zscript {
    std::unique_ptr<zs::CompiledScript> cs;
    std::vector<zs::HipModuleMeta> meta;
};

static void put_text(char *dst, size_t cap, const std::string &text) {
    if (!dst || cap == 0) return;
    const size_t n = text.size() < cap - 1 ? text.size() : cap - 1;
    memcpy(dst, text.data(), n);
    dst[n] = 0;
}
static char *dup_text(const std::string &s) {
    char *p = (char *)malloc(s.size() + 1);
    if (p) memcpy(p, s.c_str(), s.size() + 1);
    return p;
}

extern "C" {

int zh_zscript_compile(const char *text, const char *filename, uint32_t packages, zh_zscript **out, char *err, size_t err_cap) {
    if (!text || !out) return ZH_ERR_INVALID;
    *out = nullptr;
    std::vector<const zs::Package *> pk;
    if (packages & 1u) pk.push_back(&zs::zang_builtin_package());
    if (packages & 2u) pk.push_back(&zs::modules_builtin_package());
    try {
        zh_zscript *z = new zh_zscript();
        try {
            z->cs = zs::compile(text, filename ? filename : "script.txt", pk);
        } catch (...) { delete z; throw; }
        *out = z;
        return ZH_OK;
    } catch (const zs::ScriptError &e) {
        put_text(err, err_cap, e.rendered);
        return ZH_ERR_INVALID;
    } catch (const std::exception &e) {
        put_text(err, err_cap, e.what());
        return ZH_ERR_INVALID;
    }
}
int zh_zscript_destroy(zh_zscript *z) { delete z; return ZH_OK; }
void zh_zscript_free_text(char *text) { free(text); }

int zh_zscript_generate_zig(zh_zscript *z, char **text_out) {
    if (!z || !text_out) return ZH_ERR_INVALID;
    *text_out = dup_text(zs::generate_zig(*z->cs));
    return *text_out ? ZH_OK : ZH_ERR_INVALID;
}
int zh_zscript_generate_hip(zh_zscript *z, const char *only_csv, int unroll, char **text_out) {
    return zh_zscript_generate_hip_forms(z, only_csv, unroll, 0u, text_out);
}
int zh_zscript_generate_hip_forms(zh_zscript *z, const char *only_csv, int unroll, uint32_t forms, char **text_out) {
    if (!z || !text_out) return ZH_ERR_INVALID;
    std::set<std::string> only;
    if (only_csv) {
        std::string cur;
        for (const char *p = only_csv;; p++) {
            if (*p == ',' || *p == 0) { if (!cur.empty()) only.insert(cur); cur.clear(); if (!*p) break; }
            else cur += *p;
        }
    }
    z->meta.clear();
    *text_out = dup_text(zs::generate_hip(*z->cs, only_csv ? &only : nullptr, z->meta, unroll, forms));
    return *text_out ? ZH_OK : ZH_ERR_INVALID;
}
uint32_t zh_zscript_module_count(zh_zscript *z) { return z ? (uint32_t)z->meta.size() : 0; }
int zh_zscript_module_info(zh_zscript *z, uint32_t i, char *name, size_t name_cap, uint32_t *state_words, uint32_t *noise_fields,
                           uint32_t *n_params, char *error, size_t error_cap) {
    if (!z || i >= z->meta.size()) return ZH_ERR_INVALID;
    const zs::HipModuleMeta &m = z->meta[i];
    put_text(name, name_cap, m.name);
    put_text(error, error_cap, m.error);
    if (state_words) *state_words = (uint32_t)m.state_words;
    if (noise_fields) *noise_fields = (uint32_t)m.noise_fields;
    if (n_params) *n_params = (uint32_t)m.params.size();
    return ZH_OK;
}
int zh_zscript_module_num_temps(zh_zscript *z, uint32_t i, uint32_t *num_temps) {
    if (!z || i >= z->meta.size() || !num_temps) return ZH_ERR_INVALID;
    *num_temps = (uint32_t)z->meta[i].num_temps;
    return ZH_OK;
}
int zh_zscript_module_param(zh_zscript *z, uint32_t i, uint32_t p, char *name, size_t name_cap, char *kind, size_t kind_cap, char *enum_name, size_t enum_cap) {
    if (!z || i >= z->meta.size() || p >= z->meta[i].params.size()) return ZH_ERR_INVALID;
    const zs::HipParam &hp = z->meta[i].params[p];
    put_text(name, name_cap, hp.name);
    put_text(kind, kind_cap, hp.kind);
    put_text(enum_name, enum_cap, hp.enum_name);
    return ZH_OK;
}

}
```

zang_amd/script.py:

```python
import ctypes as C
import os

import numpy as np
import torch

from . import abi, zscript_native as native
from .runtime import as_bool, as_buf, default_context


class ScriptCompileError(Exception):
    pass


class HipBackendError(Exception):
    """The script compiled, but this module uses something the HIP backend does not generate (the message says what)."""


def compile_hip(hip_source):
    lib = abi.load()
    code, n = C.c_void_p(), C.c_size_t()
    log = C.create_string_buffer(1 << 16)
    rc = lib.zh_script_compile(hip_source.encode(), C.byref(code), C.byref(n), log, len(log))
    if rc != 0:
        raise ScriptCompileError("hiprtc failed (%d):\n%s" % (rc, log.value.decode(errors="replace")))
    lib.zh_script_free_code(code)
    return n.value


class ScriptProgram:

    def __init__(self, text, ctx=None, filename="script.txt", only=None, forms=native.FORM_ROLES_WORTH, hip_patch=None, code_cache=None, spans=False):
        self.ctx = ctx or default_context()
        self.lib = self.ctx.lib
        self.text, self.filename = text, filename
        try:
            compiled = native.NativeScript(text, filename)
        except native.NativeScriptError as e:
            raise ScriptCompileError(str(e))
        forms = int(os.environ.get("ZH_SCRIPT_FORMS", forms))
        if spans:
            forms |= native.FORM_SPANS
        self.hip_source, self.meta = compiled.generate_hip(only=only, unroll=int(os.environ.get("ZH_SCRIPT_UNROLL", "0")), forms=forms)
        if hip_patch is not None:
            self.hip_source = hip_patch(self.hip_source)
        h = C.c_void_p()
        log = C.create_string_buffer(1 << 16)
        self.loaded_from_cache = False
        cache_file = None
        if code_cache is not None and hip_patch is None:
            import hashlib
            key = hashlib.sha256(self.hip_source.encode() + b"\0" + self.lib.zh_version()).hexdigest()[:32]
            cache_file = os.path.join(code_cache, "zs_%s.hsaco" % key)
            if os.path.exists(cache_file):
                blob = open(cache_file, "rb").read()
                if self.lib.zh_script_load_code(self.ctx.handle, blob, len(blob), C.byref(h)) == 0:
                    compiled.close()
                    self.handle, self._modules, self.loaded_from_cache = h, [], True
                    self.ctx._children.add(self)
                    return
        if cache_file is not None:
            code, n = C.c_void_p(), C.c_size_t()
            if self.lib.zh_script_compile(self.hip_source.encode(), C.byref(code), C.byref(n), log, len(log)) == 0:
                blob = C.string_at(code, n.value)
                self.lib.zh_script_free_code(code)
                os.makedirs(code_cache, exist_ok=True)
                tmp = cache_file + ".%d.tmp" % os.getpid()
                open(tmp, "wb").write(blob)
                os.replace(tmp, cache_file)
                if self.lib.zh_script_load_code(self.ctx.handle, blob, len(blob), C.byref(h)) == 0:
                    compiled.close()
                    self.handle, self._modules = h, []
                    self.ctx._children.add(self)
                    return
        rc = self.lib.zh_script_load(self.ctx.handle, self.hip_source.encode(), C.byref(h), log, len(log))
        if rc != 0 and forms and hip_patch is None:
            self.role_form_error = log.value.decode(errors="replace")
            self.hip_source, self.meta = compiled.generate_hip(only=only, unroll=int(os.environ.get("ZH_SCRIPT_UNROLL", "0")), forms=forms & native.FORM_SPANS)
            rc = self.lib.zh_script_load(self.ctx.handle, self.hip_source.encode(), C.byref(h), log, len(log))
        compiled.close()
        if rc != 0:
            raise ScriptCompileError("zh_script_load failed (%d):\n%s" % (rc, log.value.decode(errors="replace")))
        self.handle = h
        self._modules = []
        self.ctx._children.add(self)

    def module(self, name, n_voices, first_seed=0):
        m = self.meta.get(name)
        if m is None:
            raise KeyError("script exports no module named %r" % name)
        if "error" in m:
            raise HipBackendError("%s: %s" % (name, m["error"]))
        return ScriptModule(self, name, n_voices, first_seed)

    def close(self):
        if self.handle:
            for m in list(self._modules):
                m.close()
            self.lib.zh_script_destroy(self.handle)
            self.handle = None

    def __del__(self):
        try:
            self.close()
        except Exception:
            pass


_ENUM_LABELS = native.ENUM_LABELS


class ScriptModule:
    num_outputs = 1

    def __init__(self, program, name, n_voices, first_seed=0):
        self.program, self.name, self.n = program, name, n_voices
        self.meta = program.meta[name]
        self.params = self.meta["params"]
        self.lib = program.lib
        h = C.c_void_p()
        abi.check(self.lib.zh_script_module_create(program.handle, name.encode(), n_voices, self.meta["state_words"],
                                                   first_seed, C.byref(h)), "zh_script_module_create")
        self.handle = h
        program._modules.append(self)

    @property
    def num_temps(self):
        return self.meta["num_temps"]

    def _param(self, kind, enum, value, keep):
        p = abi.ScriptParam()
        dev = self.program.ctx.device
        if kind == "constant":
            p.kind = abi.SP_CONSTANT
            if torch.is_tensor(value):
                assert value.dtype == torch.float32 and value.numel() == self.n and value.is_contiguous()
                p.pf = value.data_ptr(); keep.append(value)
            else:
                p.f = float(value)
        elif kind == "boolean":
            p.kind = abi.SP_BOOLEAN
            if torch.is_tensor(value):
                assert value.dtype == torch.uint8 and value.numel() == self.n and value.is_contiguous()
                p.pb = value.data_ptr(); keep.append(value)
            else:
                p.u = 1 if value else 0
        elif kind in ("constant_or_buffer", "buffer"):
            p.kind = abi.SP_COB if kind == "constant_or_buffer" else abi.SP_BUFFER
            if isinstance(value, abi.Cob):
                keep.append(value)
                if value.tag == abi.COB_BUFFER:
                    p.is_buffer, p.pf, p.stride = 1, value.buffer.ptr, value.buffer.stride
                else:
                    p.f, p.pf = value.constant.value, value.constant.per_voice
            elif torch.is_tensor(value) and value.dim() == 2:
                b = as_buf(value); keep.append(value)
                p.is_buffer, p.pf, p.stride = 1, b.ptr, b.stride
            elif torch.is_tensor(value):
                assert kind == "constant_or_buffer" and value.dtype == torch.float32 and value.numel() == self.n
                p.pf = value.data_ptr(); keep.append(value)
            else:
                assert kind == "constant_or_buffer", "a waveform param needs a [frames, voices] image"
                p.f = float(value)
        elif kind == "curve":
            p.kind = abi.SP_CURVE
            if torch.is_tensor(value):
                p.pf, p.u = value.data_ptr(), value.numel() // 2; keep.append(value)
            else:
                nodes = np.array([(v, t) for t, v in value], np.float32).reshape(-1)
                tns = torch.from_numpy(nodes).to(dev)
                p.pf, p.u = tns.data_ptr(), len(value); keep.append(tns)
        else:
            p.kind = abi.SP_ENUM
            if isinstance(value, abi.Curve):
                if enum != "PaintCurve":
                    raise TypeError("a PaintCurve value for a %s param" % enum)
                if value.duration.per_voice:
                    raise ValueError("a script module takes one PaintCurve duration for all voices, not a per-voice array")
                p.u, p.f = value.tag, value.duration.value
            else:
                label, payload = (value, None) if isinstance(value, str) else value
                p.u = _ENUM_LABELS[enum].index(label.lstrip("."))
                p.f = float(payload) if payload is not None else 0.0
        return p

    def _params(self, params, keep, defaults=()):
        arr = (abi.ScriptParam * abi.SCRIPT_MAX_PARAMS)()
        for i, (name, kind, enum) in enumerate(self.params):
            if name in params:
                arr[i] = self._param(kind, enum, params[name], keep)
            elif name in defaults:
                arr[i] = self._param(kind, enum, _default_value(kind, enum), keep)
            else:
                raise KeyError("missing param %r" % name)
        extra = set(params) - {n for n, _, _ in self.params}
# ... 238 lines not shown
```

zang_amd/zscript_native.py:

```python
import ctypes as C

from . import abi

PACKAGE_ZANG, PACKAGE_MODULES = 1, 2
DEFAULT_PACKAGES = PACKAGE_ZANG | PACKAGE_MODULES

ENUM_LABELS = {
    "PaintCurve": ["instantaneous", "linear", "squared", "cubed"],
    "InterpolationFunction": ["linear", "smoothstep"],
    "DistortionType": ["overdrive", "clip"],
    "FilterType": ["bypass", "low_pass", "band_pass", "high_pass", "notch", "all_pass"],
    "NoiseColor": ["white", "pink"],
}


class NativeScriptError(Exception):
    """A compile error with the reference's rendering (file:line:col: message, source line, carets)."""


def _package_bits(packages):
    if isinstance(packages, int):
        return packages
    bits = 0
    for p in packages:
        name = getattr(p, "zig_package_name", p)
        if name == "zang":
            bits |= PACKAGE_ZANG
        elif name == "mod":
            bits |= PACKAGE_MODULES
        else:
            raise ValueError("the native compiler knows the two builtin packages only")
    return bits


FORM_ROLES = 1
FORM_ROLES_WORTH = 2
FORM_SPANS = 8


class NativeScript:
    def __init__(self, contents, filename="script.txt", packages=DEFAULT_PACKAGES):
        self.lib = abi.load()
        h = C.c_void_p()
        err = C.create_string_buffer(1 << 14)
        rc = self.lib.zh_zscript_compile(contents.encode(), filename.encode(), _package_bits(packages), C.byref(h), err, len(err))
        if rc != 0:
            raise NativeScriptError(err.value.decode(errors="replace"))
        self.handle = h

    def _text(self, fn, *args):
        p = C.c_void_p()
        abi.check(fn(self.handle, *args, C.byref(p)), fn.__name__)
        try:
            return C.string_at(p).decode()
        finally:
            self.lib.zh_zscript_free_text(p)

    def generate_zig(self):
        return self._text(self.lib.zh_zscript_generate_zig)

    def generate_hip(self, only=None, unroll=0, forms=0):
        text = self._text(self.lib.zh_zscript_generate_hip_forms, None if only is None else ",".join(only).encode(), int(unroll), int(forms))
        meta = {}
        name, err = C.create_string_buffer(256), C.create_string_buffer(1024)
        kind, en = C.create_string_buffer(64), C.create_string_buffer(64)
        for i in range(self.lib.zh_zscript_module_count(self.handle)):
            words, noise, npar = C.c_uint32(), C.c_uint32(), C.c_uint32()
            abi.check(self.lib.zh_zscript_module_info(self.handle, i, name, len(name), C.byref(words), C.byref(noise), C.byref(npar), err, len(err)),
                      "zh_zscript_module_info")
            if err.value:
                meta[name.value.decode()] = {"error": err.value.decode()}
                continue
            params = []
            pname = C.create_string_buffer(256)
            for p in range(npar.value):
                abi.check(self.lib.zh_zscript_module_param(self.handle, i, p, pname, len(pname), kind, len(kind), en, len(en)), "zh_zscript_module_param")
                params.append((pname.value.decode(), kind.value.decode(), en.value.decode() or None))
            nt = C.c_uint32()
            abi.check(self.lib.zh_zscript_module_num_temps(self.handle, i, C.byref(nt)), "zh_zscript_module_num_temps")
            meta[name.value.decode()] = {"state_words": words.value, "params": params, "noise_fields": noise.value, "num_temps": nt.value}
        return text, meta

    def close(self):
        if self.handle:
            self.lib.zh_zscript_destroy(self.handle)
            self.handle = None

    def __del__(self):
        try:
            self.close()
        except Exception:
            pass
```

Measured before the change: 1714 billion.

## Drop sign-of-zero adds in generated script kernels via zero-fact analysis

Adds a dataflow pass over script instructions that finds temporaries whose zero-initialised add, and Filter mix terms multiplied by zero, only affect the sign of a zero that no output can observe. Generated HIP then assigns directly, or picks per ZERO_FIRST flag through a compile-time ZS_Z template parameter, and uses type-specialised Filter mixes. The goal is fewer ALU ops per frame in script kernels. The cost is more kernel template instantiations and longer codegen, and correctness rests on the zero-sign analysis.

```diff
diff --git a/bindings/zang_hip.zig b/bindings/zang_hip.zig
--- a/bindings/zang_hip.zig
+++ b/bindings/zang_hip.zig
@@ -118,6 +118,7 @@
 pub const ZSCRIPT_FORM_SPANS: u32 = 8;
 pub const ZSCRIPT_FORM_ROLES: u32 = 1;
 pub const ZSCRIPT_FORM_ROLES_WORTH: u32 = 2;
+pub const ZSCRIPT_FORM_SIGNED_ZERO: u32 = 16;
 
 pub const Ctx = opaque {};
 pub const Graph = opaque {};
diff --git a/include/zang_hip.h b/include/zang_hip.h
--- a/include/zang_hip.h
+++ b/include/zang_hip.h
@@ -564,6 +564,7 @@
 ZH_API int zh_zscript_generate_hip(zh_zscript *z, const char *only_csv, int unroll, char **text_out);
 #define ZH_ZSCRIPT_FORM_ROLES 1
 #define ZH_ZSCRIPT_FORM_ROLES_WORTH 2
+#define ZH_ZSCRIPT_FORM_SIGNED_ZERO 16
 ZH_API int zh_zscript_generate_hip_forms(zh_zscript *z, const char *only_csv, int unroll, uint32_t forms, char **text_out);
 ZH_API uint32_t zh_zscript_module_count(zh_zscript *z);
 ZH_API int zh_zscript_module_info(zh_zscript *z, uint32_t i, char *name, size_t name_cap, uint32_t *state_words, uint32_t *noise_fields,
diff --git a/zang_amd/csrc/common.hip.h b/zang_amd/csrc/common.hip.h
--- a/zang_amd/csrc/common.hip.h
+++ b/zang_amd/csrc/common.hip.h
@@ -123,7 +123,7 @@
        ZF_NICE_MIX_ROLL, ZF_NICE_MIX_WG_MIN, ZF_NF_PC_MAX, ZF_NF_RING_MAX, ZF_FILTER_PC_MAX, ZF_FILTER_PC16_MAX, ZF_FILTER_PC_CTL_MAX,
        ZF_PINK_PIPE_MAX, ZF_PINK_TAPS, ZF_ECHOES_PC_MAX, ZF_DELAY_FRAMES_MAX, ZF_FILTER_TP_MAX, ZF_NF_TP_MAX, ZF_NICE_TP_MAX,
        ZF_PINK_TP_MAX, ZF_ECHOES_TP_MAX, ZF_NICE_MIX_FMA, ZF_BASICS_ROWS_MIN, ZF_SCRIPT_PC, ZF_SCRIPT_PC_MAXV, ZF_NF_TP_PIPE_FRAMES, ZF_DISTORTION_ROWS_MIN, ZF_DISTORTION_RC, ZF_GRAPH_DIRECT,
-       ZF_STEREO_ECHOES_PC_MAX, ZF_COUNT };
+       ZF_STEREO_ECHOES_PC_MAX, ZF_SCRIPT_SIGNED_ZERO, ZF_COUNT };
 long zh_form(int id);
 bool zh_form_is_set(int id);
 uint32_t zh_range_frames(uint32_t V, uint32_t n, int form, uint32_t target_waves, uint32_t max_voices);
diff --git a/zang_amd/csrc/dispatch.hip b/zang_amd/csrc/dispatch.hip
--- a/zang_amd/csrc/dispatch.hip
+++ b/zang_amd/csrc/dispatch.hip
@@ -52,6 +52,7 @@
      {"distortion_rc", 0, "... rows per wave of that form: 3 (0), 6 or 8"},
      {"graph_direct", 1, "zh_graph_launch of a ZH_CAPTURE_COALESCE capture that recorded nothing but held-back oscillator batches: 1 = their launches enqueued directly, one per batch of up to 32 buffers (20 paints: one launch of 20), 0 = the recorded hipGraph (20 paints: two launches of 10)"},
      {"stereo_echoes_pc_max", 32768, "StereoEchoes: up to here loader / filter / writer waves (k_stereo_echoes_pc); StereoEchoes(15000), 1,024 frames, role waves against the walk: 253 / 318 us at 32,768 voices, 518 / 454 at 65,536 (profiles/r10)"},
+     {"script_signed_zero", 1, "generated script kernels asked for with ZH_ZSCRIPT_FORM_SIGNED_ZERO (zang_amd.script does; lane and sub-span forms): 1 = without the adds of a zeroed temporary and the Filter mix terms that only fix the sign of a zero no output can see (zscript_emit.hip zero_facts; same bits), 0 = the bit is masked off when the text is generated: the kernels as they were (profiles/r15)"},
 };
 
 struct Overrides { bool set[ZF_COUNT]; long val[ZF_COUNT]; };
@@ -143,6 +144,8 @@
 
 int zh_form_count(void) { return ZF_COUNT; }
 
+long zs_dispatch_signed_zero_row(void) { return zh_form(ZF_SCRIPT_SIGNED_ZERO); }
+
 int zh_form_info(int index, const char **name, long *default_value, long *current_value, const char **doc) {
     if (index < 0 || index >= ZF_COUNT) return ZH_ERR_INVALID;
     if (name) *name = kForms[index].name;
diff --git a/zang_amd/csrc/voices.hip.h b/zang_amd/csrc/voices.hip.h
--- a/zang_amd/csrc/voices.hip.h
+++ b/zang_amd/csrc/voices.hip.h
@@ -197,6 +197,20 @@
     __device__ __forceinline__ float mix(float sl, float sb, float sh) const { return sl * l_mul + sb * b_mul + sh * h_mul; }
     __device__ __forceinline__ float post(float x, float sl, float sb, float sh) const { return bypass ? x : mix(sl, sb, sh); }
 
+    template <uint32_t TYPE, bool Z> __device__ __forceinline__ float mix_t(float sl, float sb, float sh) const {
+        static_assert(TYPE >= ZH_FILTER_LOW_PASS && TYPE <= ZH_FILTER_ALL_PASS, "a filter type other than bypass");
+        if (TYPE == ZH_FILTER_LOW_PASS) return Z ? sl + sb * 0.0f : (sl + sb * 0.0f) + sh * 0.0f;
+        if (TYPE == ZH_FILTER_BAND_PASS) return Z ? sb + sh * 0.0f : (sl * 0.0f + sb) + sh * 0.0f;
+        if (TYPE == ZH_FILTER_HIGH_PASS) return Z ? sb * 0.0f + sh : (sl * 0.0f + sb * 0.0f) + sh;
+        if (TYPE == ZH_FILTER_NOTCH) return (sl + sb * 0.0f) + sh;
+        return (sl + sb) + sh;
+    }
+    template <uint32_t TYPE, bool Z, bool CB, bool RB> __device__ __forceinline__ float frame_t(float x, float cutoff_i, float res_i) {
+        if (CB) cut = zclampf(cutoff_i, 0.0f, 1.0f);
+        if (RB) res = 1.0f - zclampf(res_i, 0.0f, 1.0f);
+        const SvfOut s = svf_step(l, b, x, cut, res);
+        return mix_t<TYPE, Z>(s.l, s.b, s.h);
+    }
 };
 
 struct DecimatorLane {
diff --git a/zang_amd/csrc/zscript_emit.hip b/zang_amd/csrc/zscript_emit.hip
--- a/zang_amd/csrc/zscript_emit.hip
+++ b/zang_amd/csrc/zscript_emit.hip
@@ -429,6 +429,8 @@
     Lines *begin_sink, *end_sink;
     std::string rel = "(i - L.start)", length = "SPAN_LEN";
     const std::map<size_t, Val> *track = nullptr;
+    const std::map<const Instr *, bool> *drop = nullptr, *drop_z = nullptr;
+    int out_nn = 0;
     ModuleCtx(Kernel &k_, size_t mi, std::vector<Val> env_, std::string outvar_, std::string nic_, std::string prefix_, const ModuleCtx *parent)
         : k(k_), module_index(mi), env(std::move(env_)), outvar(std::move(outvar_)), nic(std::move(nic_)), prefix(std::move(prefix_)) {
         begin_sink = parent ? parent->begin_sink : &k.pro;
@@ -480,6 +482,8 @@
 public:
     const CompiledScript &s;
     explicit HipEmitter(const CompiledScript &cs) : s(cs) {}
+    bool signed_zero = false;
+    bool zs_z_form = true;
 
     Val val(ModuleCtx &mc, const Res &r) {
         Val v;
@@ -515,23 +519,25 @@
         return v.tag;
     }
     static std::string enum_payload(const Val &v) { return v.payload ? v.payload->expr : "0.0f"; }
-    static Lines put_lines(ModuleCtx &mc, const Dest &d, const std::string &expr, bool zero_first, bool heavy, uint64_t sines) {
+    static Lines put_lines(ModuleCtx &mc, const Dest &d, const std::string &expr, bool zero_first, bool heavy, uint64_t sines, int drop = 0) {
         if (!d.output) {
             mc.heavy[d.index] = heavy;
             mc.srcs[d.index] = sines;
             mc.cobsrc.erase(d.index);
             const std::string t = mc.tname(d.index);
+            if (zero_first && drop == 2) return {t + " = 0.0f;", t + " = " + expr + ";"};
+            if (zero_first && drop == 1) return {t + " = 0.0f;", t + " = ZS_Z ? (" + expr + ") : " + t + " + (" + expr + ");"};
             if (zero_first) return {t + " = 0.0f;", t + " = " + t + " + (" + expr + ");"};
             return {t + " = " + expr + ";"};
         }
         mc.outsines |= sines;
         return {mc.outvar + " = " + mc.outvar + " + (" + expr + ");"};
     }
-    static void put(ModuleCtx &mc, const Dest &d, const std::string &expr, bool zero_first, bool heavy = false, uint64_t sines = 0, int cost = 1) {
+    static void put(ModuleCtx &mc, const Dest &d, const std::string &expr, bool zero_first, bool heavy = false, uint64_t sines = 0, int cost = 1, int drop = 0) {
         Kernel &k = mc.k;
         const Mark mk = k.mark();
         Unit u;
-        u.text = put_lines(mc, d, expr, zero_first, heavy, sines);
+        u.text = put_lines(mc, d, expr, zero_first, heavy, sines, drop);
         u.cost = cost + (zero_first ? 1 : 0);
         if (d.output && mc.outvar == "o") {
             const std::string zo = k.zfresh("zo");
@@ -568,6 +574,130 @@
         if (op == "pow") return "zpowf(" + a + ", " + b + ")";
         if (op == "max") return "zs_max(" + a + ", " + b + ")";
         return "zs_min(" + a + ", " + b + ")";
+    }
+
+    typedef std::map<const Instr *, bool> ZeroFacts;
+    struct ZDef { const Instr *ins = nullptr; bool nn = false, addz = false, inner = false, shown = false; std::vector<size_t> into; };
+    std::map<std::pair<size_t, bool>, ZeroFacts> zero_memo;
+    static bool literal_nn(const Res &r) { return r.kind == RK::literal_number && !(r.num.value == 0.0f && signbit(r.num.value)); }
+    void zero_walk(size_t module_index, const std::vector<Instr> &list, bool out_nn, bool inner, std::vector<ZDef> &defs, std::map<size_t, size_t> &cur) {
+        const Module &module = s.pr.modules[module_index];
+        const ModuleResult &mr = s.module_results[module_index];
+        auto reaching = [&](const Res &r) -> ZDef * {
+            if (r.kind != RK::temp_buffer) return nullptr;
+            auto it = cur.find(r.index);
+            return it == cur.end() ? nullptr : &defs[it->second];
+        };
+        auto nn = [&](const Res &r) { if (literal_nn(r)) return true; ZDef *d = reaching(r); return d && d->nn; };
+        auto shows = [&](const Res &r) { if (ZDef *d = reaching(r)) d->shown = true; };
+        auto hands_on = [&](const Res &r, const Dest &out) {
+            ZDef *d = reaching(r);
+            if (!d) return;
+            if (out.output) { if (!out_nn) d->shown = true; }
+            else d->into.push_back(defs.size());
+        };
+        auto define = [&](size_t temp, const Instr *ins, bool is_nn, bool addz) {
+            ZDef d;
+            d.ins = ins; d.inner = inner; d.nn = is_nn && !inner; d.addz = addz;
+            cur[temp] = defs.size();
+            defs.push_back(d);
+        };
+        auto is_const = [&](const Res &r) {
+            if (r.kind == RK::literal_number || r.kind == RK::temp_float) return true;
+            if (r.kind == RK::self_param) return module.params[r.index].type.kind == PK::constant;
+            if (r.kind == RK::track_param) return s.pr.tracks[r.track_index].params[r.index].type.kind == PK::constant;
+            return false;
+        };
+        for (const Instr &ins : list) {
+            switch (ins.kind) {
+            case IK::copy_buffer: {
+                const bool n = nn(ins.src);
+                hands_on(ins.src, ins.out);
+                if (!ins.out.output) define(ins.out.index, &ins, n, false);
+                break;
+            }
+            case IK::float_to_buffer: if (!ins.out.output) define(ins.out.index, &ins, literal_nn(ins.src), false); break;
+            case IK::cob_to_buffer: if (!ins.out.output) define(ins.out.index, &ins, false, false); break;
+            case IK::arith_float: case IK::arith_float_float: break;
+            case IK::arith_buffer:
+                shows(ins.a);
+                if (!ins.out.output) define(ins.out.index, &ins, false, false);
+                break;
+            case IK::arith_float_buffer: case IK::arith_buffer_float: case IK::arith_buffer_buffer: {
+                if (ins.op == "add" || ins.op == "mul") {
+                    const bool n = ins.op == "add" && (nn(ins.a) || nn(ins.b));
+                    if (ins.out.output) { hands_on(ins.a, ins.out); hands_on(ins.b, ins.out); }
+                    else define(ins.out.index, &ins, n, true);
+                } else if (ins.op == "sub") {
+                    const bool n = nn(ins.a);
+                    hands_on(ins.a, ins.out); hands_on(ins.b, ins.out);
+                    if (!ins.out.output) define(ins.out.index, &ins, n, false);
+                } else {
+                    shows(ins.a); shows(ins.b);
+                    if (!ins.out.output) define(ins.out.index, &ins, false, false);
+                }
+                break;
+            }
+            case IK::call: {
+                const Module &callee = s.pr.modules[mr.fields[ins.field_index]];
+                if (!callee.builtin) {
+                    for (const Res &r : ins.args) shows(r);
+                    if (!ins.out.output) define(ins.out.index, &ins, true, false);
+                    break;
+                }
+                const std::string &name = callee.builtin_name;
+                bool lit_type = false, const_freq = false;
+                for (size_t j = 0; j < callee.params.size() && j < ins.args.size(); j++) {
+                    if (callee.params[j].name == "type") lit_type = ins.args[j].kind == RK::literal_enum_value && ins.args[j].label != "bypass";
+                    if (callee.params[j].name == "freq") const_freq = is_const(ins.args[j]);
+                }
+                for (size_t j = 0; j < callee.params.size() && j < ins.args.size(); j++)
+                    if (!(name == "Filter" && callee.params[j].name == "input" && lit_type)) shows(ins.args[j]);
+                if (!ins.out.output) define(ins.out.index, &ins, name == "PulseOsc" || (name == "TriSawOsc" && const_freq) || name == "Gate", true);
+                break;
+            }
+            case IK::track_call: case IK::delay: {
+                const std::map<size_t, size_t> before = cur;
+                const size_t first = defs.size();
+                if (!ins.out.output) define(ins.out.index, &ins, false, false);
+                if (ins.kind == IK::delay) { define(ins.feedback_temp, &ins, false, false); define(ins.feedback_out_temp, &ins, false, false); }
+                for (size_t i = first; i < defs.size(); i++) defs[i].inner = true, defs[i].nn = false;
+                zero_walk(module_index, ins.instructions, out_nn, true, defs, cur);
+                for (const auto &kv : cur) {
+                    auto b = before.find(kv.first);
+                    if (kv.second >= first && b != before.end()) defs[b->second].shown = true;
+                }
+                break;
+            }
+            }
+        }
+    }
+    const ZeroFacts &zero_facts(size_t module_index, bool out_nn) {
+        const auto key = std::make_pair(module_index, out_nn);
+        auto it = zero_memo.find(key);
+        if (it != zero_memo.end()) return it->second;
+        std::vector<ZDef> defs;
+        std::map<size_t, size_t> cur;
+        zero_walk(module_index, s.module_results[module_index].instructions, out_nn, false, defs, cur);
+        ZeroFacts facts;
+        std::vector<bool> hidden(defs.size(), false);
+        for (size_t i = defs.size(); i-- > 0;) {
+            bool h = !defs[i].shown && !defs[i].inner;
+            for (size_t t : defs[i].into) h = h && t < defs.size() && hidden[t];
+            hidden[i] = h;
+            if (defs[i].addz && !defs[i].inner) facts[defs[i].ins] = defs[i].nn || h;
+        }
+        return zero_memo[key] = facts;
+    }
+    static int zero_drop(const ModuleCtx &mc, const Instr &ins) {
+        auto has = [&](const ZeroFacts *f) { if (!f) return false; auto it = f->find(&ins); return it != f->end() && it->second; };
+        return has(mc.drop) ? 2 : has(mc.drop_z) ? 1 : 0;
+    }
+    static std::string into_nn(const ModuleCtx &mc, const Dest &d) { return (!d.output || mc.out_nn == 2) ? "true" : mc.out_nn == 1 ? "ZS_Z" : "false"; }
+    void zero_setup(ModuleCtx &mc) {
+        if (!signed_zero) return;
+        mc.drop = &zero_facts(mc.module_index, mc.out_nn == 2);
+        mc.drop_z = &zero_facts(mc.module_index, mc.out_nn >= 1);
     }
 
     void call_builtin(ModuleCtx &mc, const Instr &ins, const Module &callee, const std::vector<Res> &args) {
@@ -700,7 +830,9 @@
             ld_f("l", w);
             ld_f("b", w + 1);
             pro.push_back(o + ".begin((uint32_t)(" + enum_tag(a["type"], *callee.params[1].type.en) + "), " + c.c + ", " + r.c + ");");
-            value = o + ".frame<" + tf(c.is_buf) + ", " + tf(r.is_buf) + ">(" + a["input"].expr + ", " + (c.is_buf ? c.i : "0.0f") + ", " + (r.is_buf ? r.i : "0.0f") + ")";
+            const bool named = signed_zero && a["type"].tag_literal && a["type"].tag != "bypass";
+            const std::string fn = named ? ".frame_t<" + enum_tag(a["type"], *callee.params[1].type.en) + "u, " + into_nn(mc, ins.out) + ", " : ".frame<";
+            value = o + fn + tf(c.is_buf) + ", " + tf(r.is_buf) + ">(" + a["input"].expr + ", " + (c.is_buf ? c.i : "0.0f") + ", " + (r.is_buf ? r.i : "0.0f") + ")";
         } else if (name == "Decimator") {
             decl.push_back("DecimatorLane " + o + ";");
             ld_f("dval", w);
@@ -751,7 +883,13 @@
             mc.outsines |= out_sines;
             target = mc.outvar;
         }
-        const std::string addl = target + " = " + target + " + (" + value + ");";
+        const int drop = ins.out.output ? 0 : zero_drop(mc, ins);
+        auto add_line = [&](const std::string &val) {
+            if (drop == 2) return target + " = " + val + ";";
+            if (drop == 1) return target + " = ZS_Z ? (" + val + ") : " + target + " + (" + val + ");";
+            return target + " = " + target + " + (" + val + ");";
+        };
+        const std::string addl = add_line(value);
         Unit u;
         u.stateful = state_words(name) > 0;
         u.cost = builtin_cost(name, a, u.walk);
@@ -780,7 +918,9 @@
                         "    " + fl + " = zs_s.l;", "    " + fb + " = zs_s.b;", "    " + fh + " = zs_s.h;", "}"};
             pb.cost = pb.walk = u.cost - 6; pb.stateful = pb.owner = true;
             const bool never_bypass = a["type"].tag_literal && a["type"].tag != "bypass";
-            const std::string mix = never_bypass ? o + ".mix(" + fl + ", " + fb + ", " + fh + ")" : o + ".post(" + a["input"].expr + ", " + fl + ", " + fb + ", " + fh + ")";
+            const bool named = signed_zero && never_bypass;
+            const std::string mix = named ? o + ".mix_t<" + enum_tag(a["type"], *callee.params[1].type.en) + "u, " + into_nn(mc, ins.out) + ">(" + fl + ", " + fb + ", " + fh + ")"
+                                    : never_bypass ? o + ".mix(" + fl + ", " + fb + ", " + fh + ")" : o + ".post(" + a["input"].expr + ", " + fl + ", " + fb + ", " + fh + ")";
             pc.cost = 5;
             if (target == "o") {
                 auto gw = writer_add(mix, "");
@@ -788,7 +928,7 @@
                 u.parts = {pa, pb, pc, gw.second};
             } else {
                 if (!ins.out.output) pc.lines.push_back(target + " = 0.0f;");
-                pc.lines.push_back(target + " = " + target + " + (" + mix + ");");
+                pc.lines.push_back(add_line(mix));
                 u.parts = {pa, pb, pc};
             }
         } else if (target == "o") {
@@ -882,7 +1022,7 @@
             else if (ins.op == "div") { k.sink(vb); sines = sa; }
             if (ins.op == "add" || ins.op == "mul") {
                 if (ins.kind == IK::arith_float_buffer) std::swap(a, b);
-                put(mc, ins.out, bin(ins.op, a, b), true, heavy, sines, op_cost(ins.op));
+                put(mc, ins.out, bin(ins.op, a, b), true, heavy, sines, op_cost(ins.op), zero_drop(mc, ins));
             } else {
                 put(mc, ins.out, bin(ins.op, a, b), false, heavy, sines, op_cost(ins.op));
             }
@@ -904,6 +1044,7 @@
                 k.unit_done(mk, std::move(u));
             } else outvar = mc.outvar;
             ModuleCtx sub(k, callee_index, env, outvar, mc.nic, k.fresh(mc.prefix + "c") + "_", &mc);
+            sub.out_nn = ins.out.output ? mc.out_nn : 2;
             module_body(sub);
             if (!ins.out.output) mc.srcs[ins.out.index] = sub.outsines;
             else mc.outsines |= sub.outsines;
@@ -1095,6 +1236,7 @@
 
     void module_body(ModuleCtx &mc) {
         const ModuleResult &mr = s.module_results[mc.module_index];
+        zero_setup(mc);
         for (const Instr &ins : mr.instructions) instruction(mc, mr, ins);
     }
 
@@ -1156,6 +1298,7 @@
             k.params.push_back(HipParam{p.name, kind, p.type.en ? p.type.en->name : ""});
         }
         ModuleCtx mc(k, module_index, env, "o", "NIC", "", nullptr);
+        mc.out_nn = signed_zero && zs_z_form ? 1 : 0;
         module_body(mc);
     }
 
@@ -1526,6 +1669,7 @@
             out.push_back(I + I + strf("auto zs_body = [&](auto zs_q, uint32_t i, const float (&zs_in)[%zu], float (&zs_out)[%zu], float &o) ZH_INLINE_LAMBDA {", NIN ? NIN : 1, NOUT ? NOUT : 1));
             const std::string B = I + I + I;
             out.push_back(B + "constexpr bool ZS_Q = decltype(zs_q)::value; (void)ZS_Q;");
+            if (signed_zero) out.push_back(B + "constexpr bool ZS_Z = false; (void)ZS_Z;     // (the writer's `o` may be the live output row)");
             out.push_back(B + "(void)i; (void)zs_in; (void)zs_out; (void)o;");
             out.push_back(B + strf("float x[%zu]; (void)x;", ni));
             {
@@ -1616,6 +1760,7 @@
         for (const std::string &t : k.quiet_terms) all += (all.empty() ? "" : " && ") + t;
         out.push_back(I + strf("auto zs_body = [&](auto zs_q, uint32_t i, const float (&x)[%zu], float &o) ZH_INLINE_LAMBDA {", ni));
         out.push_back(II + "constexpr bool ZS_Q = decltype(zs_q)::value; (void)ZS_Q;");
+        if (signed_zero) out.push_back(II + "constexpr bool ZS_Z = false; (void)ZS_Z;     // (one walk for zeroed and live rows)");
         out.push_back(II + "(void)i; (void)x;");
         if (!k.temps.empty()) {
             std::string decl = "float ";
@@ -1639,6 +1784,7 @@
     }
 
     std::string generate(const std::set<std::string> *only, std::vector<HipModuleMeta> &meta, int unroll_override, unsigned forms) {
+        signed_zero = (forms & ZH_ZSCRIPT_FORM_SIGNED_ZERO) != 0;
         Lines out = {"// generated by zang_amd.zangscript (HIP backend) -- compile with zh_script_load / zh_script_compile",
                      "#include \"script_rt.hip.h\"", ""};
         for (size_t ci = 0; ci < s.pr.curves.size(); ci++) {
@@ -1660,7 +1806,22 @@
             m.name = name;
             m.num_temps = s.module_results[em.second].num_temps;
             try {
+                zs_z_form = true;
                 kernel(k, em.second);
+                if (signed_zero) {
+                    size_t saved = 0, cost = 0;
+                    for (const Unit &u : k.units) cost += (size_t)u.cost;
+                    for (const std::string &l : k.frame) {
+                        for (size_t at = l.find("ZS_Z ?"); at != std::string::npos; at = l.find("ZS_Z ?", at + 1)) saved += 1;
+                        for (size_t at = l.find("ZS_Z,"); at != std::string::npos; at = l.find("ZS_Z,", at + 1)) saved += 2;
+                    }
+                    if (saved > 0 && saved * 40 < cost) {
+                        zs_z_form = false;
+                        k = Kernel();
+                        k.name = name;
+                        kernel(k, em.second);
+                    }
+                }
             } catch (const HipBackendError &e) {
                 m.error = e.message;
                 meta.push_back(m);
@@ -1722,6 +1883,7 @@
             preamble.push_back(I + strf("size_t istr[%zu] = {", ni) + zeros + "};");
             preamble.push_back(I + strf("uint32_t ivo[%zu] = {", ni) + zeros + "};");
             for (size_t j = 0; j < k.rows.size(); j++) preamble.push_back(I + strf("ins[%zu] = zs_row(L.p[%zu], v, istr[%zu], ivo[%zu]);", j, k.rows[j], j, j));
+            const size_t preamble_head = preamble.size();
             append(preamble, indent(k.pro));
             append(out, preamble);
             out.push_back(I + "bool zs_walk = false; (void)zs_walk;");
@@ -1735,7 +1897,15 @@
             const std::string lam = I + strf("                     [&](uint32_t i, const float (&x)[%zu], float &o) ZH_INLINE_LAMBDA ", ni);
             std::string all;
             for (const std::string &t : k.quiet_terms) all += (all.empty() ? "" : " && ") + t;
-            if (tolerant) {
+            bool uses_z = false;
+            for (const std::string &l : frame_lines) uses_z = uses_z || l.find("ZS_Z") != std::string::npos;
+            if (uses_z) {
+                if (two_bodies) out.push_back(I + "auto zs_quiet = [&](int zs_n) ZH_INLINE_LAMBDA -> bool { return " + all + "; };");
+                out.push_back(I + strf("auto zs_body = [&](auto zs_q, auto zs_t, auto zs_z, uint32_t i, const float (&x)[%zu], float &o) ZH_INLINE_LAMBDA {", ni));
+                out.push_back(I + I + "constexpr bool ZS_Q = decltype(zs_q)::value; (void)ZS_Q;");
+                out.push_back(I + I + "constexpr bool ZS_T = decltype(zs_t)::value; (void)ZS_T;");
+                out.push_back(I + I + "constexpr bool ZS_Z = decltype(zs_z)::value; (void)ZS_Z;");
+            } else if (tolerant) {
                 if (two_bodies) out.push_back(I + "auto zs_quiet = [&](int zs_n) ZH_INLINE_LAMBDA -> bool { return " + all + "; };");
                 out.push_back(I + strf("auto zs_body = [&](auto zs_q, auto zs_t, uint32_t i, const float (&x)[%zu], float &o) ZH_INLINE_LAMBDA {", ni));
                 out.push_back(I + I + "constexpr bool ZS_Q = decltype(zs_q)::value; (void)ZS_Q;");
@@ -1755,7 +1925,29 @@
                 out.push_back(I + I + decl + ";");
             }
             append(out, indent(indent(frame_lines)));
-            if (tolerant) {
+            if (uses_z) {
+                out.push_back(I + "};");
+                out.push_back(I + "auto zs_run = [&](auto zs_t, auto zs_z) ZH_INLINE_LAMBDA {");
+                out.push_back(I + I + strf("zs_frame_loop<%d, %zu>(L.out, v, L.ostride, ins, istr, ivo, L.start, L.end, decltype(zs_z)::value, zs_walk,", unroll, nin));
+                if (two_bodies) {
+                    out.push_back(I + lam + "{ zs_body(zs_tag<false>{}, zs_t, zs_z, i, x, o); }, zs_quiet,");
+                    out.push_back(I + lam + "{ zs_body(zs_tag<true>{}, zs_t, zs_z, i, x, o); });");
+                } else {
+                    out.push_back(I + lam + "{ zs_body(zs_tag<false>{}, zs_t, zs_z, i, x, o); });");
+                }
+                out.push_back(I + "};");
+                out.push_back(I + "const bool zs_zf = (L.flags & ZH_PAINT_ZERO_FIRST) != 0;");
+                const std::string run_f = "if (zs_zf) zs_run(zs_tag<false>{}, zs_tag<true>{}); else zs_run(zs_tag<false>{}, zs_tag<false>{});";
+                if (tolerant) {
+                    out.push_back(I + "if (L.flags & ZH_PAINT_TOLERANT) {");
+                    out.push_back(I + I + "if (zs_zf) zs_run(zs_tag<true>{}, zs_tag<true>{}); else zs_run(zs_tag<true>{}, zs_tag<false>{});");
+                    out.push_back(I + "} else {");
+                    out.push_back(I + I + run_f);
+                    out.push_back(I + "}");
+                } else {
+                    out.push_back(I + run_f);
+                }
+            } else if (tolerant) {
                 out.push_back(I + "};");
                 for (const char *t : {"true", "false"}) {
                     out.push_back(I + (std::string(t) == "true" ? "if (L.flags & ZH_PAINT_TOLERANT) {" : "} else {"));
@@ -1782,7 +1974,19 @@
             if (forms & ZH_ZSCRIPT_FORM_SPANS) { out.push_back(""); append(out, spans_kernel(k, nin, ni, unroll)); }
             if (forms & (ZH_ZSCRIPT_FORM_ROLES | ZH_ZSCRIPT_FORM_ROLES_WORTH)) {
                 bool worth = false;
-                const Lines pc = role_kernel(k, nin, ni, preamble, (forms & 4u) ? 131072 : 65536, worth);
+                Kernel kr;
+                Lines preamble_r(preamble.begin(), preamble.begin() + (long)preamble_head);
+                const Kernel *rk = &k;
+                const Lines *rp = &preamble;
+                if (signed_zero) {
+                    signed_zero = false;
+                    kr.name = name;
+                    kernel(kr, em.second);
+                    append(preamble_r, indent(kr.pro));
+                    rk = &kr; rp = &preamble_r;
+                }
+                const Lines pc = role_kernel(*rk, nin, ni, *rp, (forms & 4u) ? 131072 : 65536, worth);
+                signed_zero = (forms & ZH_ZSCRIPT_FORM_SIGNED_ZERO) != 0;
                 if (!pc.empty() && ((forms & ZH_ZSCRIPT_FORM_ROLES) || worth)) { out.push_back(""); append(out, pc); }
             }
         }
@@ -1803,6 +2007,8 @@
 }
 
 }
+
+extern "C" long zs_dispatch_signed_zero_row(void) __attribute__((weak));
 
 struct zh_zscript {
     std::unique_ptr<zs::CompiledScript> cs;
@@ -1857,6 +2063,7 @@
 }
 int zh_zscript_generate_hip_forms(zh_zscript *z, const char *only_csv, int unroll, uint32_t forms, char **text_out) {
     if (!z || !text_out) return ZH_ERR_INVALID;
+    if ((forms & ZH_ZSCRIPT_FORM_SIGNED_ZERO) && zs_dispatch_signed_zero_row && zs_dispatch_signed_zero_row() == 0) forms &= ~(uint32_t)ZH_ZSCRIPT_FORM_SIGNED_ZERO;
     std::set<std::string> only;
     if (only_csv) {
         std::string cur;
diff --git a/zang_amd/script.py b/zang_amd/script.py
--- a/zang_amd/script.py
+++ b/zang_amd/script.py
@@ -40,6 +40,7 @@
         forms = int(os.environ.get("ZH_SCRIPT_FORMS", forms))
         if spans:
             forms |= native.FORM_SPANS
+        forms |= native.FORM_SIGNED_ZERO
         self.hip_source, self.meta = compiled.generate_hip(only=only, unroll=int(os.environ.get("ZH_SCRIPT_UNROLL", "0")), forms=forms)
         if hip_patch is not None:
             self.hip_source = hip_patch(self.hip_source)
diff --git a/zang_amd/zscript_native.py b/zang_amd/zscript_native.py
--- a/zang_amd/zscript_native.py
+++ b/zang_amd/zscript_native.py
@@ -36,6 +36,7 @@
 FORM_ROLES = 1
 FORM_ROLES_WORTH = 2
 FORM_SPANS = 8
+FORM_SIGNED_ZERO = 16
 
 
 class NativeScript:
```

Result: no change. 1697 billion (-1.0%).
